# anenbergb/Co-DETR-TensorRT

Hardware: AMD Instinct MI355X
Metric: images/sec, Co-DINO Swin-L 1920x1280 fp16 (p50 ms/image alongside) (higher is better)
Workload: dtype f16

## Files before the change

co-detr-tensorrt_amd/codetr/_cabi.py:

```python
import ctypes
import os

import torch

_HERE = os.path.dirname(os.path.abspath(__file__))
LIB_PATH = os.path.join(_HERE, "libcodetr_hip.so")
ABI_VERSION = 54

_i64, _i32, _vp, _cp = ctypes.c_int64, ctypes.c_int, ctypes.c_void_p, ctypes.c_char_p

_MSDA_ARGS = [_vp, _vp, _vp, _vp, _vp, _vp, _i64, _i64, _i32, _i32, _i32, _i64, _i32, _i64, _vp]
SIGNATURES = {
    "codetr_hip_abi_version": (_i32, []),
    "codetr_hip_strerror": (_cp, [_i32]),
    "codetr_msda_forward_f16": (_i32, _MSDA_ARGS),
    "codetr_msda_forward_bf16": (_i32, _MSDA_ARGS),
    "codetr_msda_forward_f32": (_i32, _MSDA_ARGS),
    "codetr_msda_forward_f64": (_i32, _MSDA_ARGS),
    "codetr_msda_backward_f16": (_i32, [_vp, _vp, _vp, _vp, _vp, _vp, _vp, _i64, _i64, _i32, _i32, _i32, _i64, _i32, _i64,
                                        _vp, _vp, _vp]),
    "codetr_msda_backward_f32": (_i32, [_vp, _vp, _vp, _vp, _vp, _vp, _vp, _i64, _i64, _i32, _i32, _i32, _i64, _i32, _i64,
                                        _vp, _vp, _vp]),
    "codetr_msda_backward_f64": (_i32, [_vp, _vp, _vp, _vp, _vp, _vp, _vp, _i64, _i64, _i32, _i32, _i32, _i64, _i32, _i64,
                                        _vp, _vp, _vp]),
    "codetr_msda_variant": (_cp, [_i32, _i32, _i32, _i32, _i32]),
    "codetr_msda_fused_forward_f16": (_i32, [_vp, _vp, _vp, _vp, _vp, _i64, _vp, _i64, _vp, _i32, _i32, _i64, _i64,
                                             _i32, _i32, _i32, _i64, _i32, _vp]),
    "codetr_msda_fused_forward_bf16": (_i32, [_vp, _vp, _vp, _vp, _vp, _i64, _vp, _i64, _vp, _i32, _i32, _i64, _i64,
                                              _i32, _i32, _i32, _i64, _i32, _vp]),
    "codetr_msda_fused_forward_ref32_f16": (_i32, [_vp, _vp, _vp, _vp, _vp, _i64, _vp, _i64, _vp, _i32, _i32, _i64, _i64,
                                                   _i32, _i32, _i32, _i64, _i32, _vp]),
    "codetr_msda_fused_forward_ref32_bf16": (_i32, [_vp, _vp, _vp, _vp, _vp, _i64, _vp, _i64, _vp, _i32, _i32, _i64, _i64,
                                                    _i32, _i32, _i32, _i64, _i32, _vp]),
    "codetr_msda_encoder_forward_packed_f16": (_i32, [_vp, _vp, _vp, _vp, _i64, _vp, _i64, _i64, _i32, _i32, _i32, _i32,
                                                      _vp, _i32, _i32, _i32, _i32, _vp]),
    "codetr_msda_encoder_forward_packed_bf16": (_i32, [_vp, _vp, _vp, _vp, _i64, _vp, _i64, _i64, _i32, _i32, _i32, _i32,
                                                       _vp, _i32, _i32, _i32, _i32, _vp]),
    "codetr_linear_bf16_f16out": (_i32, [_vp, _vp, _vp, _vp, _vp, _vp, _i64, _i64, _i64, _i64, _i32]),
    "codetr_encoder_projections_f16": (_i32, [_vp, _vp, _vp, _vp, _vp, _vp, _vp, _vp, _i64, _i64, _i64, _i64, _i64, _i32]),
    "codetr_encoder_projections_bf16": (_i32, [_vp, _vp, _vp, _vp, _vp, _vp, _vp, _vp, _i64, _i64, _i64, _i64, _i64, _i32]),
    "codetr_encoder_projections_posgen_f16": (_i32, [_vp, _vp] + [_vp] * 10 + [_vp, _i32, _vp, ctypes.c_float, ctypes.c_float, ctypes.c_float,
                                                              ctypes.c_float, _i32, _vp, _vp, _vp, _vp, _vp, _i64, _i64, _i64, _i64, _i64, _i64, _i32]),
    "codetr_encoder_projections_posgen_bf16": (_i32, [_vp, _vp] + [_vp] * 10 + [_vp, _i32, _vp, ctypes.c_float, ctypes.c_float, ctypes.c_float,
                                                              ctypes.c_float, _i32, _vp, _vp, _vp, _vp, _vp, _i64, _i64, _i64, _i64, _i64, _i64, _i32]),
    "codetr_msda_encoder_packed_lds_bytes": (_i64, [_vp, _i32, _i32, _i32, _vp, _i32, _i32, _i32]),
    "codetr_msda_pack_projection_index": (_i32, [_i32, _i32, _i32, _vp]),
    "codetr_mx_scale_bytes": (_i64, [_i64, _i64]),
    "codetr_linear_fp8mx": (_i32, [_vp, _vp, _vp, _vp, _vp, _vp, _vp, _vp, _vp, _i64, _i64, _i64, _i32]),
    "codetr_cast_fp8mx_f16": (_i32, [_vp, _vp, _vp, _vp, _i64, _i64]),
    "codetr_layernorm_fp8mx_f16": (_i32, [_vp, _vp, _vp, _vp, _vp, _vp, _i64, _i64, ctypes.c_float]),
    "codetr_window_attention_fp8mx_f16": (_i32, [_vp, _vp, _vp, _vp, _vp, _vp, _i64, _i64, _i64, _i32, _i32, _i32, _i32]),
    "codetr_mha_attention_f16": (_i32, [_vp, _vp, _vp, _vp, _vp, _i64, _i64, _i64, _i32, _i32, _i64, _i64, _i64, _i64]),
    "codetr_mha_attention_bf16": (_i32, [_vp, _vp, _vp, _vp, _vp, _i64, _i64, _i64, _i32, _i32, _i64, _i64, _i64, _i64]),
    "codetr_linear_ln_f16": (_i32, [_vp, _vp, _vp, _vp, ctypes.c_float, _vp, _vp, _vp, _i64, _i64, _i64, _i32]),
    "codetr_linear_ln_bf16": (_i32, [_vp, _vp, _vp, _vp, ctypes.c_float, _vp, _vp, _vp, _i64, _i64, _i64, _i32]),
    "codetr_linear_xadd_f16": (_i32, [_vp, _vp, _vp, _vp, _vp, _vp, _i64, _i64, _i64]),
    "codetr_linear_xadd_bf16": (_i32, [_vp, _vp, _vp, _vp, _vp, _vp, _i64, _i64, _i64]),
    "codetr_im2col_tokens_b16": (_i32, [_vp, _vp, _i64, _i64, _i64, _i64, _i32, _i32, _i32, _vp]),
    "codetr_conv_tokens_f16": (_i32, [_vp, _vp, _vp, _vp, _vp, _vp, _i64, _i64, _i64, _i64, _i64, _i32, _i32, _i32, _i32]),
    "codetr_conv_tokens_bf16": (_i32, [_vp, _vp, _vp, _vp, _vp, _vp, _i64, _i64, _i64, _i64, _i64, _i32, _i32, _i32, _i32]),
    "codetr_conv_im2col_nchw_b16": (_i32, [_vp, _vp, _i64, _i32, _i64, _i64, _i32, _i32, _i32, _i32, _vp]),
    "codetr_maxpool_tokens_b16": (_i32, [_vp, _vp, _i64, _i64, _i64, _i64, _i32, _i32, _i32, _i32, _vp]),
    "codetr_topk_chunks": (_i64, [_i64, _i32, _i64, _vp]),
    "codetr_topk_chunked_f16": (_i32, [_vp, _vp, _i64, _i64, _i32, _i32, _vp, _vp, _vp, _i64]),
    "codetr_topk_chunked_bf16": (_i32, [_vp, _vp, _i64, _i64, _i32, _i32, _vp, _vp, _vp, _i64]),
    "codetr_topk_f16": (_i32, [_vp, _vp, _i64, _i64, _i32, _vp, _vp]),
    "codetr_topk_bf16": (_i32, [_vp, _vp, _i64, _i64, _i32, _vp, _vp]),
    "codetr_patch_im2col_b16": (_i32, [_vp, _vp, _i64, _i32, _i64, _i64, _i32, _i32, _vp]),
    "codetr_linear_variant": (_cp, [_i64, _i64, _i64, _i32, _i32, _i32]),
    "codetr_add_f16": (_i32, [_vp, _vp, _vp, _vp, _i64, _i64]),
    "codetr_add_bf16": (_i32, [_vp, _vp, _vp, _vp, _i64, _i64]),
    "codetr_sigmoid_f16": (_i32, [_vp, _vp, _vp, _i64]),
    "codetr_sigmoid_bf16": (_i32, [_vp, _vp, _vp, _i64]),
    "codetr_gather_rows_b16": (_i32, [_vp, _vp, _vp, _vp, _i64, _i64, _i64, _i64]),
    "codetr_decode_boxes_f16": (_i32, [_vp, _vp, _vp, _vp, _vp, _i64, _i64, _i64, _i32, ctypes.c_float, ctypes.c_float]),
    "codetr_decode_boxes_bf16": (_i32, [_vp, _vp, _vp, _vp, _vp, _i64, _i64, _i64, _i32, ctypes.c_float, ctypes.c_float]),
    "codetr_valid_ratios_f16": (_i32, [_vp, _vp, _vp, _vp, _vp, _i64, _i32]),
    "codetr_valid_ratios_bf16": (_i32, [_vp, _vp, _vp, _vp, _vp, _i64, _i32]),
    "codetr_linear_fp8": (_i32, [_vp, _vp, _vp, _vp, ctypes.c_float, _vp, _vp, _vp, _i32, ctypes.c_float, _i64, _i64, _i64,
                                 _i32]),
    "codetr_cast_fp8_f16": (_i32, [_vp, _vp, _vp, _i64, ctypes.c_float]),
    "codetr_layernorm_fp8_f16": (_i32, [_vp, _vp, _vp, _vp, _vp, _i64, _i64, ctypes.c_float, ctypes.c_float]),
    "codetr_linear_f16": (_i32, [_vp, _vp, _vp, _vp, _vp, _vp, _vp, _i64, _i64, _i64, _i32, _i64, _i32]),
    "codetr_linear_bf16": (_i32, [_vp, _vp, _vp, _vp, _vp, _vp, _vp, _i64, _i64, _i64, _i32, _i64, _i32]),
    "codetr_query_sine_embed_f16": (_i32, [_vp, _vp, _vp, _vp, _i64, _i64, _i32, _i32, _i32, ctypes.c_float, _i32, _vp, _vp,
                                           _vp]),
    "codetr_query_sine_embed_bf16": (_i32, [_vp, _vp, _vp, _vp, _i64, _i64, _i32, _i32, _i32, ctypes.c_float, _i32, _vp, _vp,
                                           _vp]),
    "codetr_encoder_geometry_f16": (_i32, [_vp, _vp, _vp, _i64, _i32, _vp, _vp, _vp, _vp, _vp]),
    "codetr_encoder_geometry_bf16": (_i32, [_vp, _vp, _vp, _i64, _i32, _vp, _vp, _vp, _vp, _vp]),
    "codetr_row_max_f16": (_i32, [_vp, _vp, _vp, _i64, _i64]),
    "codetr_row_max_bf16": (_i32, [_vp, _vp, _vp, _i64, _i64]),
    "codetr_preprocess_u8_f16": (_i32, [_vp, _vp, _i64, _i64, _i64, _i64, _i64, _i64, _vp, _vp, _vp, _vp, _vp]),
    "codetr_preprocess_u8_f32": (_i32, [_vp, _vp, _i64, _i64, _i64, _i64, _i64, _i64, _vp, _vp, _vp, _vp, _vp]),
    "codetr_batched_nms_f32": (_i32, [_vp, _vp, _vp, _i64, ctypes.c_float, _vp]),
    "codetr_preprocess_batch_u8_f16": (_i32, [_vp, _vp, _i64, _i64, _vp, _i64, _i64, _vp, _vp, _vp, ctypes.c_float, _vp, _vp]),
    "codetr_preprocess_batch_u8_bf16": (_i32, [_vp, _vp, _i64, _i64, _vp, _i64, _i64, _vp, _vp, _vp, ctypes.c_float, _vp, _vp]),
    "codetr_preprocess_batch_u8_f32": (_i32, [_vp, _vp, _i64, _i64, _vp, _i64, _i64, _vp, _vp, _vp, ctypes.c_float, _vp, _vp]),
    "codetr_postprocess_detections_f16": (_i32, [_vp, _vp, _vp, _vp, _vp, _i64, _i64, _i32, ctypes.c_float, _i32,
                                                 ctypes.c_float, _vp, _vp, _vp, _vp]),
    "codetr_postprocess_detections_bf16": (_i32, [_vp, _vp, _vp, _vp, _vp, _i64, _i64, _i32, ctypes.c_float, _i32,
                                                  ctypes.c_float, _vp, _vp, _vp, _vp]),
    "codetr_postprocess_detections_f32": (_i32, [_vp, _vp, _vp, _vp, _vp, _i64, _i64, _i32, ctypes.c_float, _i32,
                                                 ctypes.c_float, _vp, _vp, _vp, _vp]),
    "codetr_postprocess_softnms_f16": (_i32, [_vp, _vp, _vp, _vp, _vp, _i64, _i64, _i32, ctypes.c_float, _i32,
                                              ctypes.c_float, ctypes.c_float, _i64, _vp, _vp, _vp, _vp, _vp]),
    "codetr_postprocess_softnms_bf16": (_i32, [_vp, _vp, _vp, _vp, _vp, _i64, _i64, _i32, ctypes.c_float, _i32,
                                               ctypes.c_float, ctypes.c_float, _i64, _vp, _vp, _vp, _vp, _vp]),
    "codetr_postprocess_softnms_f32": (_i32, [_vp, _vp, _vp, _vp, _vp, _i64, _i64, _i32, ctypes.c_float, _i32,
                                              ctypes.c_float, ctypes.c_float, _i64, _vp, _vp, _vp, _vp, _vp]),
    "codetr_preprocess_views_u8_f16": (_i32, [_vp, _vp, _i64, _i64, _vp, _i64, _i64, _vp, _vp, _vp, ctypes.c_float, _vp, _vp]),
    "codetr_preprocess_views_u8_bf16": (_i32, [_vp, _vp, _i64, _i64, _vp, _i64, _i64, _vp, _vp, _vp, ctypes.c_float, _vp, _vp]),
    "codetr_preprocess_views_u8_f32": (_i32, [_vp, _vp, _i64, _i64, _vp, _i64, _i64, _vp, _vp, _vp, ctypes.c_float, _vp, _vp]),
    "codetr_tta_merge_f16": (_i32, [_vp, _vp, _vp, _vp, _vp, _i64, _i64, _i64, ctypes.c_uint32, _vp, _i32, ctypes.c_float,
                                    ctypes.c_float, _i64, _vp, _vp, _vp, _vp, _vp]),
    "codetr_tta_merge_bf16": (_i32, [_vp, _vp, _vp, _vp, _vp, _i64, _i64, _i64, ctypes.c_uint32, _vp, _i32, ctypes.c_float,
                                     ctypes.c_float, _i64, _vp, _vp, _vp, _vp, _vp]),
    "codetr_tta_merge_f32": (_i32, [_vp, _vp, _vp, _vp, _vp, _i64, _i64, _i64, ctypes.c_uint32, _vp, _i32, ctypes.c_float,
                                    ctypes.c_float, _i64, _vp, _vp, _vp, _vp, _vp]),
    "codetr_patch_merge_layernorm_f16": (_i32, [_vp, _vp, _vp, _vp, _vp, _i64, _i64, _i64, _i64, ctypes.c_float]),
    "codetr_patch_merge_layernorm_bf16": (_i32, [_vp, _vp, _vp, _vp, _vp, _i64, _i64, _i64, _i64, ctypes.c_float]),
    "codetr_mask_pyramid": (_i32, [_vp, _vp, _i64, _i64, _i64, _i32, _vp, _vp, _vp, _vp, _vp, _i32]),
    "codetr_linear_splitk_plan": (_i32, [_i64, _i64, _i64, _vp]),
    "codetr_linear_splitk_f16": (_i32, [_vp, _vp, _vp, _vp, _vp, _vp, _vp, _i64, _i64, _i64, _i32, _i32, _vp, _i64]),
    "codetr_linear_splitk_bf16": (_i32, [_vp, _vp, _vp, _vp, _vp, _vp, _vp, _i64, _i64, _i64, _i32, _i32, _vp, _i64]),
    "codetr_linear_sk_workspace_bytes": (_i64, []),
    "codetr_linear_sk_supported": (_i32, [_i64, _i64, _i64]),
    "codetr_linear_sk_preferred": (_i32, [_i64, _i64, _i64, _i32, _i32]),
    "codetr_linear_sk_f16": (_i32, [_vp, _vp, _vp, _vp, _vp, _vp, _i64, _i64, _i64, _i32, _vp, _i64, _i32]),
    "codetr_msda_op4_supported": (_i32, [_i32, _i64, _i64, _i32, _i32, _i32, _i64, _i32]),
    "codetr_msda_op4_forward_f16": (_i32, [_vp, _vp, _vp, _vp, _vp, _vp, _i64, _i64, _i32, _i32, _i32, _i64, _i32, _vp]),
    "codetr_msda_op4_forward_bf16": (_i32, [_vp, _vp, _vp, _vp, _vp, _vp, _i64, _i64, _i32, _i32, _i32, _i64, _i32, _vp]),
    "codetr_swin_mlp_supported": (_i32, [_i64, _i64, _i64]),
    "codetr_swin_mlp_f16": (_i32, [_vp, _vp, _vp, _vp, ctypes.c_float, _vp, _vp, _vp, _vp, _vp, _i64, _i64]),
    "codetr_swin_mlp_bf16": (_i32, [_vp, _vp, _vp, _vp, ctypes.c_float, _vp, _vp, _vp, _vp, _vp, _i64, _i64]),
    "codetr_linear_pp_supported": (_i32, [_i64, _i64, _i64]),
    "codetr_linear_pp_preferred": (_i32, [_i64, _i64, _i64, _i32, _i32]),
    "codetr_linear_pp_f16": (_i32, [_vp, _vp, _vp, _vp, _vp, _vp, _i64, _i64, _i64, _i32, _i32]),
    "codetr_linear_pp_bf16": (_i32, [_vp, _vp, _vp, _vp, _vp, _vp, _i64, _i64, _i64, _i32, _i32]),
    "codetr_linear_sk_bf16": (_i32, [_vp, _vp, _vp, _vp, _vp, _vp, _i64, _i64, _i64, _i32, _vp, _i64, _i32]),
    "codetr_decoder_layer_supported": (_i32, [_i32] * 7),
    "codetr_decoder_layer_blob_halfs": (_i64, [_i32] * 4),
    "codetr_decoder_layer_f16": (_i32, [_vp] * 18 + [_i64, _i64, _i64, _i32, _i32, _i32, ctypes.c_float, ctypes.c_float]),
    "codetr_decoder_layer_bf16": (_i32, [_vp] * 18 + [_i64, _i64, _i64, _i32, _i32, _i32, ctypes.c_float, ctypes.c_float]),
    "codetr_layernorm_f16": (_i32, [_vp, _vp, _vp, _vp, _vp, _i64, _i64, ctypes.c_float]),
    "codetr_layernorm_bf16": (_i32, [_vp, _vp, _vp, _vp, _vp, _i64, _i64, ctypes.c_float]),
    "codetr_groupnorm_tokens_workspace_bytes": (_i64, [_i64, _i64, _i64]),
    "codetr_groupnorm_tokens_f16": (_i32, [_vp, _vp, _vp, _vp, _vp, _i64, _vp, _i64, _i64, _i64, _i32,
                                           ctypes.c_float]),
    "codetr_groupnorm_tokens_bf16": (_i32, [_vp, _vp, _vp, _vp, _vp, _i64, _vp, _i64, _i64, _i64, _i32,
                                           ctypes.c_float]),
    "codetr_sine_pos_tokens_f16": (_i32, [_vp, _vp, _vp, _vp, _vp, _i64, _i64, _i64, _i64, _i32, ctypes.c_float,
                                          ctypes.c_float, ctypes.c_float, ctypes.c_float, _i32]),
    "codetr_sine_pos_tokens_bf16": (_i32, [_vp, _vp, _vp, _vp, _vp, _i64, _i64, _i64, _i64, _i32, ctypes.c_float,
                                          ctypes.c_float, ctypes.c_float, ctypes.c_float, _i32]),
    "codetr_ffn_relu_f16": (_i32, [_vp, _vp, _vp, _vp, _vp, _vp, _vp, _i64, _i64, _i64]),
    "codetr_ffn_relu_ln_f16": (_i32, [_vp, _vp, _vp, _vp, _vp, _vp, _vp, _i64, _i64, _i64, _vp, _vp, ctypes.c_float,
                                      _vp, _vp]),
    "codetr_ffn_relu_ln2_f16": (_i32, [_vp, _vp, _vp, _vp, _vp, _vp, _vp, _i64, _i64, _i64, _vp, _vp, ctypes.c_float,
                                       _vp, _vp, ctypes.c_float, _vp, _vp]),
    "codetr_ffn_relu_ln2_bf16": (_i32, [_vp, _vp, _vp, _vp, _vp, _vp, _vp, _i64, _i64, _i64, _vp, _vp, ctypes.c_float,
                                       _vp, _vp, ctypes.c_float, _vp, _vp]),
    "codetr_ffn_pack_w2_f16": (_i32, [_vp, _vp, _vp, _i64, _i64]),
    "codetr_ffn_oproj_relu_ln2_f16": (_i32, [_vp, _vp, _vp, _vp, _vp, _vp, _vp, _vp, _vp, _vp, _i64, _i64, _i64, _vp, _vp,
                                             ctypes.c_float, _vp, _vp, ctypes.c_float, _vp, _vp]),
    "codetr_ffn_oproj_relu_ln2_bf16": (_i32, [_vp, _vp, _vp, _vp, _vp, _vp, _vp, _vp, _vp, _vp, _i64, _i64, _i64, _vp, _vp,
                                              ctypes.c_float, _vp, _vp, ctypes.c_float, _vp, _vp]),
    "codetr_ffn_oproj_w1_index": (_i32, [_i64, _vp]),
    "codetr_ffn_fp8": (_i32, [_vp, _vp, _vp, _vp, _vp, _vp, _vp, _vp, _vp, _i64, _i64, _i64, ctypes.c_float, ctypes.c_float,
                              _vp, _vp, ctypes.c_float, _vp, _vp, ctypes.c_float, _vp, _vp]),
    "codetr_window_attention_f16": (_i32, [_vp, _vp, _vp, _vp, _vp, _i64, _i64, _i64, _i32, _i32, _i32, _i32]),
    "codetr_window_attention_bf16": (_i32, [_vp, _vp, _vp, _vp, _vp, _i64, _i64, _i64, _i32, _i32, _i32, _i32]),
    "codetr_window_attention_ex": (_i32, [_vp, _vp, _vp, _vp, _vp, _vp, ctypes.c_float, _i64, _i64, _i64, _i32, _i32, _i32, _i32,
                                          _i32, _i32, _i32]),
    "codetr_window_attention_bias_index": (_i32, [_i32, _vp]),
    "codetr_window_attention_fp8out_f16": (_i32, [_vp, _vp, _vp, _vp, _vp, ctypes.c_float, _i64, _i64, _i64, _i32, _i32,
                                                  _i32, _i32]),
}

_lib = None

CALLS = {"encoder_projections_posgen": 0, "msda": 0, "msda_fused": 0, "linear": 0, "layernorm": 0, "window_attention": 0, "groupnorm_tokens": 0,
         "sine_pos_tokens": 0, "ffn_fused": 0, "ffn_oproj_fused": 0, "linear_splitk": 0, "linear_sk": 0, "mask_pyramid": 0,
         "query_sine_embed": 0, "encoder_geometry": 0, "row_max": 0, "preprocess": 0, "batched_nms": 0,
         "preprocess_batch": 0, "postprocess_detections": 0, "postprocess_softnms": 0,
         "preprocess_views": 0, "tta_merge": 0,
         "msda_backward": 0, "patch_merge_layernorm": 0, "msda_encoder": 0, "msda_encoder_packed": 0, "patch_im2col": 0, "mha_attention": 0, "topk": 0,
         "linear_pp": 0, "swin_mlp": 0, "linear_tile128": 0, "linear_tile256": 0, "linear_xs": 0, "linear_ln": 0, "linear_xadd": 0, "encoder_projections": 0,
         "linear_fp8": 0, "cast_fp8": 0, "layernorm_fp8": 0, "small_ops": 0, "ffn_fp8": 0, "decoder_layer": 0,
         "conv_tokens": 0, "conv_im2col_nchw": 0, "maxpool_tokens": 0}


RECORDER = None
_QUERIES = {"codetr_hip_abi_version", "codetr_hip_strerror", "codetr_msda_variant", "codetr_linear_variant",
            "codetr_topk_chunks", "codetr_linear_splitk_plan", "codetr_groupnorm_tokens_workspace_bytes",
            "codetr_linear_sk_workspace_bytes", "codetr_linear_sk_supported", "codetr_linear_sk_preferred",
            "codetr_linear_pp_supported", "codetr_linear_pp_preferred", "codetr_msda_op4_supported", "codetr_swin_mlp_supported",
            "codetr_msda_encoder_packed_lds_bytes", "codetr_msda_pack_projection_index", "codetr_window_attention_bias_index",
            "codetr_mx_scale_bytes", "codetr_decoder_layer_supported",
            "codetr_decoder_layer_blob_halfs"}


class _RecordingLib:
    def __init__(self, lib):
        self._lib = lib

    def __getattr__(self, name):
        fn = getattr(self._lib, name)
        if name in _QUERIES or name not in SIGNATURES:
            return fn

        def launch(*args):
            rc = fn(*args)
            if RECORDER is not None and rc == 0:
                RECORDER.append((name, args))
            return rc

        return launch


_rec_lib = None


def load():
    global _lib, _rec_lib
    if _lib is not None:
        if RECORDER is None:
            return _lib
        if _rec_lib is None:
            _rec_lib = _RecordingLib(_lib)
        return _rec_lib
    if not os.path.isfile(LIB_PATH):
        raise ImportError(
            f"HIP extension not found at {LIB_PATH}; build it with "
            "`python -c 'import __graft_entry__ as g; g.build()'` or `make -C co-detr-tensorrt_amd/csrc`"
        )
    lib = ctypes.CDLL(LIB_PATH)
    for name, (res, args) in SIGNATURES.items():
        try:
            fn = getattr(lib, name)
        except AttributeError as e:
            raise ImportError(f"{LIB_PATH} does not export {name}; rebuild the extension") from e
        fn.restype = res
        fn.argtypes = args
    ver = lib.codetr_hip_abi_version()
    if ver != ABI_VERSION:
        raise ImportError(f"{LIB_PATH} has ABI version {ver}, host expects {ABI_VERSION}; rebuild the extension")
    _lib = lib
    return lib


def strerror(code: int) -> str:
    return load().codetr_hip_strerror(code).decode()


def check(code: int, what: str):
    if code != 0:
        raise RuntimeError(f"{what} failed: {strerror(code)} (code {code})")


def current_stream_ptr(device) -> int:
    return torch.cuda.current_stream(device).cuda_stream


_MSDA_BY_DTYPE = {
    torch.float16: ("codetr_msda_forward_f16", 2),
    torch.bfloat16: ("codetr_msda_forward_bf16", 2),
    torch.float32: ("codetr_msda_forward_f32", 4),
    torch.float64: ("codetr_msda_forward_f64", 8),
}


def msda_variant(dtype, M, D, L, P) -> str:
    return load().codetr_msda_variant(_MSDA_BY_DTYPE[dtype][1], M, D, L, P).decode()


def msda_forward(value, spatial_shapes, level_start_index, sampling_loc, attn_weight, im2col_step, out):
    lib = load()
    CALLS["msda"] += 1
    name, _ = _MSDA_BY_DTYPE[value.dtype]
    B, S, M, D = value.shape
    Nq, L, P = sampling_loc.shape[1], sampling_loc.shape[3], sampling_loc.shape[4]
    rc = getattr(lib, name)(
        current_stream_ptr(value.device),
        value.data_ptr(), spatial_shapes.data_ptr(), level_start_index.data_ptr(),
        sampling_loc.data_ptr(), attn_weight.data_ptr(),
        B, S, M, D, L, Nq, P, int(im2col_step), out.data_ptr(),
    )
    if rc == -2:
        raise RuntimeError(f"batch({B}) must divide im2col_step({min(B, int(im2col_step))})")
    check(rc, name)
    return out


_ACT = {None: 0, "relu": 1, "gelu": 2, "relu_res": 3}
_LINEAR_BY_DTYPE = {torch.float16: "codetr_linear_f16", torch.bfloat16: "codetr_linear_bf16"}


def linear_supported(x, weight) -> bool:
    return x.dtype in _LINEAR_BY_DTYPE and weight.dtype == x.dtype and weight.shape[1] % 64 == 0


_VARIANTS = {}


def linear_variant(M, N, K, act=None, has_residual=False, hm_head_dim=0) -> str:
    key = (M, N, K, act, bool(has_residual), hm_head_dim)
    v = _VARIANTS.get(key)
    if v is None:
        v = _VARIANTS[key] = load().codetr_linear_variant(M, N, K, _ACT[act], 1 if has_residual else 0,
                                                          hm_head_dim).decode()
    return v


def linear(x2d, weight, bias, residual2d, act, out2d, row_mask=None, hm_rows=0, hm_head_dim=0):
    lib = load()
    CALLS["linear"] += 1
    M, K = x2d.shape
    N = weight.shape[0]
    variant = linear_variant(M, N, K, act, residual2d is not None, hm_head_dim)
    if variant != "unsupported":
        CALLS["linear_" + variant] += 1
    rc = getattr(lib, _LINEAR_BY_DTYPE[x2d.dtype])(
        current_stream_ptr(x2d.device), x2d.data_ptr(), weight.data_ptr(),
        bias.data_ptr() if bias is not None else None,
        residual2d.data_ptr() if residual2d is not None else None,
        row_mask.data_ptr() if row_mask is not None else None,
        out2d.data_ptr(), M, N, K, _ACT[act], hm_rows, hm_head_dim)
    check(rc, "codetr_linear")
    return out2d


_SK_PREFERRED = {}


def linear_sk_preferred(M, N, K, act=None, has_residual=False) -> bool:
    key = (M, N, K, act, bool(has_residual))
    v = _SK_PREFERRED.get(key)
    if v is None:
        v = _SK_PREFERRED[key] = bool(load().codetr_linear_sk_preferred(M, N, K, _ACT[act], 1 if has_residual else 0))
    return v


_SK_WORKSPACE = {}


def linear_sk_workspace(device):
    key = (device.index, torch.cuda.current_stream(device).cuda_stream)
    ws = _SK_WORKSPACE.get(key)
    if ws is None:
        with torch.cuda.device(device):
            ws = _SK_WORKSPACE[key] = torch.zeros(load().codetr_linear_sk_workspace_bytes(), dtype=torch.uint8, device=device)
    return ws


def linear_sk(x2d, weight, bias, residual2d, act, out2d, flags=0):
    lib = load()
    CALLS["linear"] += 1
    CALLS["linear_sk"] += 1
    M, K = x2d.shape
    N = weight.shape[0]
    ws = linear_sk_workspace(x2d.device) if flags & 0x40 else None
    fn = lib.codetr_linear_sk_f16 if x2d.dtype == torch.float16 else lib.codetr_linear_sk_bf16
    rc = fn(current_stream_ptr(x2d.device), x2d.data_ptr(), weight.data_ptr(),
            bias.data_ptr() if bias is not None else None,
            residual2d.data_ptr() if residual2d is not None else None, out2d.data_ptr(), M, N, K, _ACT[act],
            ws.data_ptr() if ws is not None else None, ws.numel() if ws is not None else 0, flags)
    check(rc, "codetr_linear_sk")
    return out2d


def swin_mlp(x2d, ln_w, ln_b, eps, w1, b1, w2_packed, b2, out2d):
    CALLS["swin_mlp"] += 1
    lib = load()
    fn = lib.codetr_swin_mlp_bf16 if x2d.dtype == torch.bfloat16 else lib.codetr_swin_mlp_f16
    rc = fn(current_stream_ptr(x2d.device), x2d.data_ptr(), ln_w.data_ptr(), ln_b.data_ptr(), float(eps), w1.data_ptr(),
            b1.data_ptr(), w2_packed.data_ptr(), b2.data_ptr(), out2d.data_ptr(), x2d.shape[0], x2d.shape[1])
    check(rc, "codetr_swin_mlp")
    return out2d


_PP_PREFERRED = {}


def linear_pp_preferred(M, N, K, act=None, has_residual=False) -> bool:
    key = (M, N, K, act, bool(has_residual))
    v = _PP_PREFERRED.get(key)
    if v is None:
        v = _PP_PREFERRED[key] = bool(load().codetr_linear_pp_preferred(M, N, K, _ACT[act], 1 if has_residual else 0))
    return v


def linear_pp(x2d, weight, bias, residual2d, act, out2d, flags=0):
    lib = load()
    CALLS["linear"] += 1
    CALLS["linear_pp"] += 1
    M, K = x2d.shape
    N = weight.shape[0]
    fn = lib.codetr_linear_pp_f16 if x2d.dtype == torch.float16 else lib.codetr_linear_pp_bf16
    rc = fn(current_stream_ptr(x2d.device), x2d.data_ptr(), weight.data_ptr(),
            bias.data_ptr() if bias is not None else None,
            residual2d.data_ptr() if residual2d is not None else None, out2d.data_ptr(), M, N, K, _ACT[act], flags)
    check(rc, "codetr_linear_pp")
    return out2d


def query_sine_embed(ref, valid_ratios, pos_feat, temperature=10000.0, apply_sigmoid=True, valid_ratios32=None):
    CALLS["query_sine_embed"] += 1
    B, Nq, d = ref.shape
    L = valid_ratios.shape[1]
    ref_in = torch.empty((B, Nq, L, d), dtype=ref.dtype, device=ref.device)
    ref_in32 = torch.empty((B, Nq, L, d), dtype=torch.float32, device=ref.device) if valid_ratios32 is not None else None
    embed = torch.empty((B, Nq, d * pos_feat), dtype=ref.dtype, device=ref.device)
    fn = load().codetr_query_sine_embed_bf16 if ref.dtype == torch.bfloat16 else load().codetr_query_sine_embed_f16
    rc = fn(current_stream_ptr(ref.device), ref.data_ptr(), valid_ratios.data_ptr(),
                                            valid_ratios32.data_ptr() if valid_ratios32 is not None else None, B, Nq,
                                            d, L, pos_feat, float(temperature), 1 if apply_sigmoid else 0,
                                            ref_in.data_ptr(), ref_in32.data_ptr() if ref_in32 is not None else None,
                                            embed.data_ptr())
    check(rc, "codetr_query_sine_embed_f16")
    return ref_in, embed, ref_in32


_MSDA_BWD = {torch.float16: "codetr_msda_backward_f16", torch.float32: "codetr_msda_backward_f32",
             torch.float64: "codetr_msda_backward_f64"}


def msda_backward(value, spatial_shapes, level_start_index, sampling_loc, attn_weight, grad_output, grad_value,
                  grad_sampling_loc, grad_attn_weight, im2col_step):
    if value.dtype not in _MSDA_BWD:
        raise RuntimeError(f"multi_scale_deformable_attention_backward: unsupported dtype {value.dtype} (f16 / f32 / f64)")
    CALLS["msda_backward"] += 1
    B, S, M, D = value.shape
    Nq, L, P = sampling_loc.shape[1], sampling_loc.shape[3], sampling_loc.shape[4]
    rc = getattr(load(), _MSDA_BWD[value.dtype])(
        current_stream_ptr(value.device), value.data_ptr(), spatial_shapes.data_ptr(), level_start_index.data_ptr(),
        sampling_loc.data_ptr(), attn_weight.data_ptr(), grad_output.data_ptr(), B, S, M, D, L, Nq, P, int(im2col_step),
        grad_value.data_ptr(), grad_sampling_loc.data_ptr(), grad_attn_weight.data_ptr())
    if rc == -2:
        step = min(B, int(im2col_step))
        raise RuntimeError(f"batch({B}) must divide im2col_step({step})")
    check(rc, "codetr_msda_backward")


def encoder_geometry(valid_ratios, mask_flat, shapes):
    CALLS["encoder_geometry"] += 1
    B, S = mask_flat.shape
    L = len(shapes)
    dev = mask_flat.device
    dt = valid_ratios.dtype
    ref = torch.empty((B, S, 2), dtype=dt, device=dev)
    ref_lvl = torch.empty((B, S, L, 2), dtype=dt, device=dev)
    prop = torch.empty((B, S, 4), dtype=dt, device=dev)
    state = torch.empty((B, S), dtype=torch.uint8, device=dev)
    hw = (ctypes.c_int64 * (2 * L))(*[int(v) for s in shapes for v in s])
    fn = load().codetr_encoder_geometry_bf16 if valid_ratios.dtype == torch.bfloat16 else load().codetr_encoder_geometry_f16
    rc = fn(current_stream_ptr(dev), valid_ratios.data_ptr(), mask_flat.data_ptr(), B, L, hw,
                                            ref.data_ptr(), ref_lvl.data_ptr(), prop.data_ptr(), state.data_ptr())
    check(rc, "codetr_encoder_geometry_f16")
    return ref, ref_lvl, prop, state


def row_max(x2d):
    CALLS["row_max"] += 1
    rows, C = x2d.shape
    out = torch.empty((rows,), dtype=x2d.dtype, device=x2d.device)
    fn = load().codetr_row_max_bf16 if x2d.dtype == torch.bfloat16 else load().codetr_row_max_f16
    rc = fn(current_stream_ptr(x2d.device), x2d.data_ptr(), out.data_ptr(), rows, C)
    check(rc, "codetr_row_max_f16")
    return out


def preprocess_u8(src, resized_hw, pad_hw, mean, std, pad_value, dtype, with_mask=True):
    CALLS["preprocess"] += 1
    if dtype not in (torch.float16, torch.float32):
        raise RuntimeError("preprocess_u8 writes f16 or f32")
    Hs, Ws, _ = src.shape
    (Hr, Wr), (Hp, Wp) = resized_hw, pad_hw
    dst = torch.empty((3, Hp, Wp), dtype=dtype, device=src.device)
    mask = torch.empty((Hp, Wp), dtype=dtype, device=src.device) if with_mask else None
    f3 = ctypes.c_float * 3
    fn = load().codetr_preprocess_u8_f16 if dtype == torch.float16 else load().codetr_preprocess_u8_f32
    rc = fn(current_stream_ptr(src.device), src.data_ptr(), Hs, Ws, Hr, Wr, Hp, Wp, f3(*[float(v) for v in mean]),
            f3(*[float(v) for v in std]), (ctypes.c_int * 3)(*[int(v) for v in pad_value]), dst.data_ptr(),
            mask.data_ptr() if mask is not None else None)
    check(rc, "codetr_preprocess_u8")
    return dst, mask


def batched_nms_sorted(boxes_sorted, labels_sorted, iou_threshold):
    CALLS["batched_nms"] += 1
    N = boxes_sorted.shape[0]
    keep = torch.empty((N,), dtype=torch.bool, device=boxes_sorted.device)
    rc = load().codetr_batched_nms_f32(current_stream_ptr(boxes_sorted.device), boxes_sorted.data_ptr(),
                                       labels_sorted.data_ptr(), N, float(iou_threshold), keep.data_ptr())
    check(rc, "codetr_batched_nms_f32")
    return keep


PREPROCESS_BATCH_MAX = 32
POSTPROCESS_MAX_Q = 1024
_PRE_BATCH_BY_DTYPE = {torch.float16: "codetr_preprocess_batch_u8_f16", torch.bfloat16: "codetr_preprocess_batch_u8_bf16",
                       torch.float32: "codetr_preprocess_batch_u8_f32"}
_POST_BY_DTYPE = {torch.float16: "codetr_postprocess_detections_f16", torch.bfloat16: "codetr_postprocess_detections_bf16",
                  torch.float32: "codetr_postprocess_detections_f32"}


def preprocess_batch_u8(src, images, batch_hw, mean, std, pad_value, pad_fill, dst, mask):
    CALLS["preprocess_batch"] += 1
    N = len(images)
    H, W = batch_hw
    table = (ctypes.c_int64 * (7 * N))(*[int(v) for row in images for v in row])
    f3 = ctypes.c_float * 3
    rc = getattr(load(), _PRE_BATCH_BY_DTYPE[dst.dtype])(
        current_stream_ptr(src.device), src.data_ptr(), src.numel(), N, table, H, W, f3(*[float(v) for v in mean]),
        f3(*[float(v) for v in std]), (ctypes.c_int * 3)(*[int(v) for v in pad_value]), float(pad_fill), dst.data_ptr(),
        mask.data_ptr() if mask is not None else None)
    check(rc, "codetr_preprocess_batch_u8")


def postprocess_detections(boxes, scores, labels, divisors, score_threshold, iou_threshold, boxes_out, scores_out,
                           labels_out, count):
    CALLS["postprocess_detections"] += 1
    N, Q = scores.shape
    rc = getattr(load(), _POST_BY_DTYPE[scores.dtype])(
        current_stream_ptr(scores.device), boxes.data_ptr(), scores.data_ptr(), labels.data_ptr(), divisors.data_ptr(),
        N, Q, 0 if score_threshold is None else 1, 0.0 if score_threshold is None else float(score_threshold),
        0 if iou_threshold is None else 1, 0.0 if iou_threshold is None else float(iou_threshold), boxes_out.data_ptr(),
        scores_out.data_ptr(), labels_out.data_ptr(), count.data_ptr())
    check(rc, "codetr_postprocess_detections")


_SOFTNMS_BY_DTYPE = {torch.float16: "codetr_postprocess_softnms_f16", torch.bfloat16: "codetr_postprocess_softnms_bf16",
                     torch.float32: "codetr_postprocess_softnms_f32"}
SOFTNMS_METHODS = {"naive": 0, "linear": 1}


def postprocess_softnms(boxes, scores, labels, divisors, score_threshold, method, iou_threshold, min_score, max_keep,
                        boxes_out, scores_out, labels_out, index_out, count):
    CALLS["postprocess_softnms"] += 1
    N, Q = scores.shape
    rc = getattr(load(), _SOFTNMS_BY_DTYPE[scores.dtype])(
        current_stream_ptr(scores.device), boxes.data_ptr(), scores.data_ptr(), labels.data_ptr(), divisors.data_ptr(),
        N, Q, 0 if score_threshold is None else 1, 0.0 if score_threshold is None else float(score_threshold),
        int(method), float(iou_threshold), float(min_score), int(max_keep), boxes_out.data_ptr(), scores_out.data_ptr(),
        labels_out.data_ptr(), index_out.data_ptr(), count.data_ptr())
    check(rc, "codetr_postprocess_softnms")


TTA_MAX_VIEWS = 16
TTA_MAX_CANDIDATES = 4096
TTA_NMS_MODES = {"nms": 0, "naive": 1, "linear": 2}
_PRE_VIEWS_BY_DTYPE = {torch.float16: "codetr_preprocess_views_u8_f16", torch.bfloat16: "codetr_preprocess_views_u8_bf16",
                       torch.float32: "codetr_preprocess_views_u8_f32"}
_TTA_MERGE_BY_DTYPE = {torch.float16: "codetr_tta_merge_f16", torch.bfloat16: "codetr_tta_merge_bf16",
                       torch.float32: "codetr_tta_merge_f32"}


def preprocess_views_u8(src, rows, batch_hw, mean, std, pad_value, pad_fill, dst, mask):
    CALLS["preprocess_views"] += 1
    N = len(rows)
    H, W = batch_hw
    table = (ctypes.c_int64 * (8 * N))(*[int(v) for row in rows for v in row])
    f3 = ctypes.c_float * 3
    rc = getattr(load(), _PRE_VIEWS_BY_DTYPE[dst.dtype])(
        current_stream_ptr(src.device), src.data_ptr(), src.numel(), N, table, H, W, f3(*[float(v) for v in mean]),
        f3(*[float(v) for v in std]), (ctypes.c_int * 3)(*[int(v) for v in pad_value]), float(pad_fill), dst.data_ptr(),
        mask.data_ptr() if mask is not None else None)
    check(rc, "codetr_preprocess_views_u8")


def tta_merge(boxes, scores, labels, count, flip_mask, width, mode, iou_threshold, min_score, max_keep, boxes_out,
              scores_out, labels_out, index_out, count_out):
    CALLS["tta_merge"] += 1
    V, N, Q = scores.shape
    rc = getattr(load(), _TTA_MERGE_BY_DTYPE[scores.dtype])(
        current_stream_ptr(scores.device), boxes.data_ptr(), scores.data_ptr(), labels.data_ptr(), count.data_ptr(),
        V, N, Q, int(flip_mask), width.data_ptr(), int(mode), float(iou_threshold), float(min_score), int(max_keep),
        boxes_out.data_ptr(), scores_out.data_ptr(), labels_out.data_ptr(), index_out.data_ptr(), count_out.data_ptr())
    check(rc, "codetr_tta_merge")


def mask_pyramid(img_masks, shapes):
    CALLS["mask_pyramid"] += 1
    B, Hi, Wi = img_masks.shape
    L = len(shapes)
    S = sum(int(h) * int(w) for h, w in shapes)
    dev = img_masks.device
    mask_flat = torch.empty((B, S), dtype=torch.bool, device=dev)
    cums = torch.empty((2, B * S), dtype=torch.float32, device=dev)
    counts = torch.empty((B, L, 2), dtype=torch.float32, device=dev)
    hw = (ctypes.c_int64 * (2 * L))(*[int(v) for s in shapes for v in s])
    rc = load().codetr_mask_pyramid(current_stream_ptr(dev), img_masks.data_ptr(), B, Hi, Wi, L, hw,
                                    mask_flat.data_ptr(), cums[0].data_ptr(), cums[1].data_ptr(), counts.data_ptr(),
                                    img_masks.element_size())
    check(rc, "codetr_mask_pyramid")
    return mask_flat, cums[0], cums[1], counts


_SPLITK_PLANS = {}


def linear_splitk_plan(M, N, K):
    key = (M, N, K)
    if key not in _SPLITK_PLANS:
        nbytes = ctypes.c_int64(0)
        splits = load().codetr_linear_splitk_plan(M, N, K, ctypes.byref(nbytes))
        _SPLITK_PLANS[key] = (int(splits), int(nbytes.value))
    return _SPLITK_PLANS[key]


def linear_splitk(x2d, weight, bias, residual2d, act, out2d, splits, workspace, row_mask=None):
    lib = load()
    CALLS["linear"] += 1
    CALLS["linear_splitk"] += 1
    M, K = x2d.shape
    N = weight.shape[0]
    fn = lib.codetr_linear_splitk_f16 if x2d.dtype == torch.float16 else lib.codetr_linear_splitk_bf16
    rc = fn(current_stream_ptr(x2d.device), x2d.data_ptr(), weight.data_ptr(),
            bias.data_ptr() if bias is not None else None,
            residual2d.data_ptr() if residual2d is not None else None,
            row_mask.data_ptr() if row_mask is not None else None,
            out2d.data_ptr(), M, N, K, _ACT[act], splits, workspace.data_ptr(), workspace.numel())
# ... 586 lines not shown
```

co-detr-tensorrt_amd/codetr/_kernel_names.py:

```python
KERNEL_NAMES = (
    "add_kernel",
    "batched_nms_kernel",
    "cast_fp8_kernel",
    "cast_fp8mx_kernel",
    "conv_im2col_nchw_kernel",
    "conv_tokens_kernel",
    "decode_boxes_kernel",
    "decoder_layer_kernel",
    "encoder_geometry_kernel",
    "ffn_fp8_kernel",
    "ffn_fused_kernel",
    "gather_rows_kernel",
    "gn_apply_kernel",
    "gn_finalize_kernel",
    "gn_partial_kernel",
    "im2col_tokens_kernel",
    "layernorm_fp8_kernel",
    "layernorm_fp8mx_kernel",
    "layernorm_kernel",
    "level_cums_kernel",
    "level_mask_kernel",
    "linear_256_fp8_kernel",
    "linear_256_kernel",
    "linear_kernel",
    "linear_pp_kernel",
    "linear_sk_kernel",
    "linear_xs_kernel",
    "maxpool_tokens_kernel",
    "mha_attention_kernel",
    "msda_backward_generic_kernel",
    "msda_backward_kernel",
    "msda_encoder_v4_kernel",
    "msda_fused_headmajor_kernel",
    "msda_op4_kernel",
    "msda_scalar_kernel",
    "msda_tiled_kernel",
    "pack_w2_kernel",
    "patch_im2col_k4_kernel",
    "postprocess_kernel",
    "postprocess_softnms_kernel",
    "preprocess_batch_kernel",
    "preprocess_kernel",
    "preprocess_views_kernel",
    "query_sine_embed_kernel",
    "row_max_kernel",
    "sigmoid_kernel",
    "sine_pos_kernel",
    "splitk_reduce_kernel",
    "swin_mlp_kernel",
    "topk_kernel",
    "topk_reg_kernel",
    "tta_merge_kernel",
    "valid_ratios_kernel",
    "window_attention_kernel",
)
```

co-detr-tensorrt_amd/codetr/hip_ops.py:

```python

import collections

import torch
import torch.nn.functional as F

from . import _cabi

NATIVE = {"msda", "linear(f16/bf16, K%64==0)", "layer_norm(f16/bf16)", "swin_window_attention(f16, head_dim 32)",
          "msda_fused(softmax + sampling locations in-kernel)", "groupnorm_tokens(f16, 8 ch/group)",
          "sine_pos_tokens(f16, + level_embed)", "ffn_fused(f16, 256 -> hidden -> 256, ReLU, + identity)",
          "mask_pyramid(level masks + running valid counts + valid ratios)",
          "query_sine_embed(f16: sigmoid x valid ratios + sine embedding of the decoder reference boxes)",
          "encoder_geometry(f16: reference points, proposals, keep/drop state)", "row_max(f16)",
          "preprocess_image(u8 -> f16/f32, cv2-exact resize + pad + normalise + mask)", "batched_nms(f32)",
          "preprocess_batch(u8 -> f16/bf16/f32, <= 32 images of any size per launch, stacked + padded)",
          "postprocess_detections(f16/bf16/f32: threshold + sort + per-class NMS + rescale, one workgroup per image)",
          "postprocess_detections_soft(f16/bf16/f32: threshold + per-class soft-NMS (linear / naive) + max_per_img + rescale)",
          "patch_merge_layernorm(f16: Swin 2x2 gather + LayerNorm)",
          "msda_encoder_packed(f16/bf16: LDS-staged gather for the encoder's self-attention, csrc/msda_encoder4.hip)",
          "patch_embed(f16/bf16: 4x4 patch gather + GEMM)",
          "mha_attention(f16/bf16: dense softmax attention, head_dim 32, <= 1024 keys)",
          "topk(f16/bf16 rows, k <= 1024: radix select + bitonic sort)",
          "im2col_tokens(16-bit token-major maps)",
          "resnet50(f16/bf16: implicit-GEMM conv_tokens, stem window gather + GEMM, maxpool_tokens, BN folded)",
          "small_ops(f16: add, sigmoid, gather_rows, decode_boxes, valid_ratios)",
          "linear_fp8(e4m3 x e4m3, K%128==0) + layer_norm_fp8 + cast_fp8", "ffn_fp8(fused FFN, both products e4m3)"}


LINEAR_PROFILE = None
KERNEL_PROFILE = None


def _timed(name, meta, launch, device):
    if KERNEL_PROFILE is None:
        return launch()
    st = torch.cuda.current_stream(device)
    e0, e1 = torch.cuda.Event(enable_timing=True), torch.cuda.Event(enable_timing=True)
    e0.record(st)
    r = launch()
    e1.record(st)
    KERNEL_PROFILE.setdefault(name, []).append((e0, e1, meta))
    return r


def _gpu(x, what):
    if not x.is_cuda:
        raise RuntimeError(
            f"codetr.hip_ops.{what}: got a {x.device.type} tensor; this package computes on MI355X only "
            "(the CPU formulation is the oracle in oracle/, not a fallback)"
        )


LINEAR_PP = True


def _persistent_ok(mk, head_major, out, x2, w, r2, bias):
    return (mk is None and not head_major and out.data_ptr() % 16 == 0 and x2.data_ptr() % 16 == 0
            and w.data_ptr() % 16 == 0 and (r2 is None or r2.data_ptr() % 16 == 0)
            and (bias is None or bias.data_ptr() % 16 == 0))


def linear(x, weight, bias=None, act=None, residual=None, row_mask=None, head_major=None):
    _gpu(x, "linear")
    if _cabi.linear_supported(x, weight):
        K = x.shape[-1]
        N = weight.shape[0]
        x2 = x.reshape(-1, K)
        if not x2.is_contiguous():
            x2 = x2.contiguous()
        w = weight if weight.is_contiguous() else weight.contiguous()
        r2 = None
        if residual is not None:
            r2 = residual.reshape(-1, N)
            if not r2.is_contiguous():
                r2 = r2.contiguous()
        mk = None
        if row_mask is not None:
            mk = row_mask.reshape(-1)
            if mk.dtype != torch.bool and mk.dtype != torch.uint8:
                mk = mk != 0
            mk = mk.contiguous()
        hm_rows = hm_hd = 0
        if head_major:
            if x.dim() != 3 or residual is not None:
                raise ValueError("head_major needs a [B, S, K] input and no residual")
            hm_rows, hm_hd = x.shape[1], int(head_major)
        out = torch.empty((x2.shape[0], N), dtype=x.dtype, device=x.device)
        if x2.shape[0] > 0:
            with torch.cuda.device(x.device):
                res_act = act == "relu_res"
                splits, ws_bytes = (1, 0) if (head_major or res_act) else _cabi.linear_splitk_plan(x2.shape[0], N, K)
                if res_act:
                    launch = lambda: _cabi.linear(x2, w, bias, r2, act, out, mk, hm_rows, hm_hd)
                elif splits > 1:
                    ws = torch.empty(ws_bytes, dtype=torch.uint8, device=x.device)
                    launch = lambda: _cabi.linear_splitk(x2, w, bias, r2, act, out, splits, ws, mk)
                elif (LINEAR_PP and _persistent_ok(mk, head_major, out, x2, w, r2, bias)
                      and _cabi.linear_pp_preferred(x2.shape[0], N, K, act, r2 is not None)):
                    launch = lambda: _cabi.linear_pp(x2, w, bias, r2, act, out)
                elif (_persistent_ok(mk, head_major, out, x2, w, r2, bias)
                      and _cabi.linear_sk_preferred(x2.shape[0], N, K, act, r2 is not None)):
                    launch = lambda: _cabi.linear_sk(x2, w, bias, r2, act, out)
                else:
                    launch = lambda: _cabi.linear(x2, w, bias, r2, act, out, mk, hm_rows, hm_hd)
                if LINEAR_PROFILE is None:
                    launch()
                else:
                    st = torch.cuda.current_stream(x.device)
                    e0, e1 = torch.cuda.Event(enable_timing=True), torch.cuda.Event(enable_timing=True)
                    e0.record(st)
                    launch()
                    e1.record(st)
                    LINEAR_PROFILE.append((e0, e1, 2.0 * x2.shape[0] * N * K, x2.shape[0], N, K))
        if head_major:
            return out.view(x.shape[0], N // hm_hd, hm_rows, hm_hd)
        return out.view(*x.shape[:-1], N)
    if head_major:
        raise RuntimeError("head_major output exists only on the native linear (f16/bf16, K % 64 == 0)")
    y = F.linear(x, weight, bias)
    if act == "relu_res":
        if row_mask is not None:
            y = y.masked_fill(row_mask[..., None], 0.0)
        return F.relu(y + residual if residual is not None else y)
    if act == "relu":
        y = F.relu(y, inplace=True)
    elif act == "gelu":
        y = F.gelu(y)
    elif act is not None:
        raise ValueError(act)
    if row_mask is not None:
        y = y.masked_fill(row_mask[..., None], 0.0)
    if residual is not None:
        y = y + residual
    return y


LN_GEMM = True


def linear_ln_supported(x, norm_weight, weight):
    return (LN_GEMM and x.is_cuda and norm_weight is not None and norm_weight.dtype == x.dtype and weight.dtype == x.dtype
            and not torch.is_grad_enabled() and norm_weight.shape[0] == x.shape[-1]
            and _cabi.linear_xadd_supported(x.numel() // max(x.shape[-1], 1), weight.shape[0], x.shape[-1], x.dtype))


def linear_ln(x, norm_weight, norm_bias, eps, weight, bias=None, act=None):
    _gpu(x, "linear_ln")
    if linear_ln_supported(x, norm_weight, weight):
        K, N = x.shape[-1], weight.shape[0]
        x2 = x.reshape(-1, K)
        x2 = x2 if x2.is_contiguous() else x2.contiguous()
        w = weight if weight.is_contiguous() else weight.contiguous()
        out = torch.empty((x2.shape[0], N), dtype=x.dtype, device=x.device)
        ok = [False]

        def launch():
            ok[0] = _cabi.linear_ln(x2, norm_weight, norm_bias, eps, w, bias, act, out)

        with torch.cuda.device(x.device):
            if LINEAR_PROFILE is None:
                launch()
            else:
                st = torch.cuda.current_stream(x.device)
                e0, e1 = torch.cuda.Event(enable_timing=True), torch.cuda.Event(enable_timing=True)
                e0.record(st)
                launch()
# ... 94 lines not shown
        x2 = x2.contiguous()
    out = torch.empty_like(x2)
    w1c = w1 if w1.is_contiguous() else w1.contiguous()
    with torch.cuda.device(x.device):
        w2p = _packed_w2(w2)
        _timed("swin_mlp", {"M": x2.shape[0], "C": C},
               lambda: _cabi.swin_mlp(x2, ln_weight, ln_bias, eps, w1c, b1, w2p, b2, out), x.device)
    return out.view(x.shape)


def ffn_fused(x, w1, b1, w2, b2, ln=None, pos=None, ln_in=None):
    _gpu(x, "ffn_fused")
    x2 = x.reshape(-1, x.shape[-1])
    if not x2.is_contiguous():
        x2 = x2.contiguous()
    out = torch.empty_like(x2)
    p2 = out2 = None
    if pos is not None:
        p2 = pos.reshape(-1, pos.shape[-1])
        if p2.shape != x2.shape or p2.dtype != x2.dtype:
            raise ValueError("pos must match x in shape and dtype")
        if not p2.is_contiguous():
            p2 = p2.contiguous()
        out2 = torch.empty_like(x2)
    if x2.shape[0] > 0:
        with torch.cuda.device(x.device):
            _timed("ffn_fused", {"M": x2.shape[0], "C": x2.shape[1], "hidden": w1.shape[0]},
                   lambda: _cabi.ffn_fused(x2, w1.contiguous(), b1, _packed_w2(w2), b2, out, ln, p2, out2, ln_in), x.device)
    if pos is not None:
        return out.view(x.shape), out2.view(x.shape)
    return out.view(x.shape)


FFN_OPROJ = True


def ffn_oproj_fused(attn, wo, bo, identity, w1, b1, w2, b2, ln, pos=None, ln_in=None):
    _gpu(attn, "ffn_oproj_fused")
    C = attn.shape[-1]
    a2, i2 = attn.reshape(-1, C), identity.reshape(-1, C)
    a2 = a2 if a2.is_contiguous() else a2.contiguous()
    i2 = i2 if i2.is_contiguous() else i2.contiguous()
    if i2.shape != a2.shape or i2.dtype != a2.dtype:
        raise ValueError("identity must match the attention output in shape and dtype")
    out = torch.empty_like(a2)
    p2 = out2 = None
    if pos is not None:
        p2 = pos.reshape(-1, C)
        if p2.shape != a2.shape or p2.dtype != a2.dtype:
            raise ValueError("pos must match x in shape and dtype")
        p2 = p2 if p2.is_contiguous() else p2.contiguous()
        out2 = torch.empty_like(a2)
    w1p = derived((w1,), "_codetr_w1_oproj", lambda: w1.detach()[:, torch.tensor(
        _cabi.ffn_oproj_w1_index(C), dtype=torch.long, device=w1.device)].contiguous())
    woc = wo if wo.is_contiguous() else wo.contiguous()
    if a2.shape[0] > 0:
        with torch.cuda.device(attn.device):
            _timed("ffn_fused", {"M": a2.shape[0], "C": C, "hidden": w1.shape[0], "oproj": True},
                   lambda: _cabi.ffn_oproj_fused(a2, woc, bo, i2, w1p, b1, _packed_w2(w2), b2, out, ln_in, ln, p2, out2),
                   attn.device)
    if pos is not None:
        return out.view(attn.shape), out2.view(attn.shape)
    return out.view(attn.shape)


def layer_norm(x, weight, bias, eps=1e-5):
    _gpu(x, "layer_norm")
    if _cabi.layernorm_supported(x, weight):
        C = x.shape[-1]
        x2 = x.reshape(-1, C)
        if not x2.is_contiguous():
            x2 = x2.contiguous()
        out = torch.empty_like(x2)
        if x2.shape[0] > 0:
            with torch.cuda.device(x.device):
                _cabi.layernorm(x2, weight, bias, eps, out)
        return out.view(x.shape)
    return F.layer_norm(x, (x.shape[-1],), weight, bias, eps)


MERGE_LN = True


def patch_merge_layernorm_supported(x, C):
    return (x.is_cuda and x.dtype in (torch.float16, torch.bfloat16) and C % 8 == 0 and 4 * C <= 4096
            and MERGE_LN)


def patch_merge_layernorm(x, hw, weight_kkc, bias_kkc, eps=1e-5):
    _gpu(x, "patch_merge_layernorm")
    B, L, C = x.shape
    H, W = hw
    x4 = x.view(B, H, W, C)
    if not x4.is_contiguous():
        x4 = x4.contiguous()
    with torch.cuda.device(x.device):
        return _cabi.patch_merge_layernorm(x4, weight_kkc, bias_kkc, eps)


def group_norm(x, groups, weight, bias, eps=1e-5):
    _gpu(x, "group_norm")
    return F.group_norm(x, groups, weight, bias, eps)


def groupnorm_tokens_supported(x, groups):
    return x.is_cuda and _cabi.groupnorm_tokens_supported(x, groups)


def groupnorm_tokens_into(x, gamma, beta, groups, eps, dest, row_start):
    _gpu(x, "groupnorm_tokens_into")
    B, HW, C = x.shape
    if not x.is_contiguous():
        x = x.contiguous()
    if not dest.is_contiguous() or dest.shape[0] != B or dest.shape[2] != C:
        raise AssertionError("destination must be a contiguous [B, S, C] tensor")
    with torch.cuda.device(x.device):
        _cabi.groupnorm_tokens(x, gamma, beta, groups, eps, dest[0, row_start:], dest.shape[1] * C)
    return dest


def query_sine_embed_supported(ref, valid_ratios, pos_feat):
    return (ref.is_cuda and ref.dtype in (torch.float16, torch.bfloat16) and valid_ratios.dtype == ref.dtype
            and ref.shape[-1] in (2, 4) and pos_feat % 8 == 0 and valid_ratios.shape[1] <= ref.shape[-1] * pos_feat // 8)


def query_sine_embed(ref, valid_ratios, pos_feat, temperature=10000.0):
    _gpu(ref, "query_sine_embed")
    vr32 = getattr(valid_ratios, "_codetr_f32", None) if MSDA_FP32_REF else None
    with torch.cuda.device(ref.device):
        ref_in, embed, ref32 = _cabi.query_sine_embed(ref.contiguous(), valid_ratios.contiguous(), pos_feat, temperature,
                                                      valid_ratios32=vr32)
    if ref32 is not None:
        ref_in._codetr_ref32 = ref32
    return ref_in, embed


def encoder_geometry(valid_ratios, mask_flat, shapes):
    _gpu(mask_flat, "encoder_geometry")
    if valid_ratios.dtype not in (torch.float16, torch.bfloat16):
        raise RuntimeError("encoder_geometry is the 16-bit inference path; fp32 parity runs use the ATen formulation")
    with torch.cuda.device(mask_flat.device):
        return _cabi.encoder_geometry(valid_ratios.contiguous(), mask_flat.contiguous(),
                                      [tuple(int(v) for v in s) for s in shapes])


def row_max(x):
    _gpu(x, "row_max")
    if x.dtype not in (torch.float16, torch.bfloat16) or not x.is_contiguous():
        return x.max(-1)[0]
    with torch.cuda.device(x.device):
        return _cabi.row_max(x.view(-1, x.shape[-1])).view(x.shape[:-1])


def preprocess_image(src_u8, resized_hw, pad_hw, mean, std, pad_value=(0, 0, 0), dtype=torch.float16):
    _gpu(src_u8, "preprocess_image")
    if src_u8.dtype != torch.uint8 or src_u8.dim() != 3 or src_u8.shape[2] != 3:
        raise ValueError("expected a uint8 [H, W, 3] image")
    with torch.cuda.device(src_u8.device):
        return _cabi.preprocess_u8(src_u8.contiguous(), resized_hw, pad_hw, mean, std, pad_value, dtype)


def batched_nms(boxes, scores, labels, iou_threshold):
    _gpu(boxes, "batched_nms")
    if boxes.shape[0] == 0:
        return torch.empty((0,), dtype=torch.int64, device=boxes.device)
    order = torch.sort(scores.float(), descending=True, stable=True)[1]
    with torch.cuda.device(boxes.device):
        keep = _cabi.batched_nms_sorted(boxes.float()[order].contiguous(), labels.to(torch.int64)[order].contiguous(),
                                        iou_threshold)
    return order[keep]


PREPROCESS_BATCH_MAX = _cabi.PREPROCESS_BATCH_MAX


def preprocess_batch(src_u8, images, batch_hw, mean, std, pad_val=(0, 0, 0), pad_value=0.0, dtype=torch.float16,
                     with_mask=True):
    _gpu(src_u8, "preprocess_batch")
    if src_u8.dtype != torch.uint8 or src_u8.dim() != 1 or not src_u8.is_contiguous():
        raise ValueError("expected one contiguous flat uint8 buffer")
    if dtype not in (torch.float16, torch.bfloat16, torch.float32):
        raise ValueError(f"preprocess_batch writes f16, bf16 or f32, not {dtype}")
    N = len(images)
    H, W = (int(v) for v in batch_hw)
    x = torch.empty((N, 3, H, W), dtype=dtype, device=src_u8.device)
    m = torch.empty((N, H, W), dtype=dtype, device=src_u8.device) if with_mask else None
    with torch.cuda.device(src_u8.device):
        for i in range(0, N, PREPROCESS_BATCH_MAX):
            j = min(N, i + PREPROCESS_BATCH_MAX)
            _cabi.preprocess_batch_u8(src_u8, images[i:j], (H, W), mean, std, pad_val, pad_value, x[i:j],
                                      m[i:j] if m is not None else None)
    return x, m


Detections = collections.namedtuple("Detections", "boxes scores labels count packed")


def _detection_views(packed, N, Q, dtype):
    es = torch.empty((), dtype=dtype).element_size()
    o1 = N * Q * 8
    o2 = o1 + N * 4
    o3 = o2 + N * Q * 4 * es
    o4 = o3 + N * Q * es
    return Detections(packed[o2:o3].view(dtype).view(N, Q, 4), packed[o3:o4].view(dtype).view(N, Q),
                      packed[:o1].view(torch.int64).view(N, Q), packed[o1:o2].view(torch.int32), packed)


def postprocess_detections(boxes, scores, labels, divisors, score_threshold=None, iou_threshold=None):
    _gpu(scores, "postprocess_detections")
    dtype = scores.dtype
    if dtype not in (torch.float16, torch.bfloat16, torch.float32) or boxes.dtype != dtype or divisors.dtype != dtype:
        raise ValueError("postprocess_detections: boxes, scores and divisors in one dtype of f16 / bf16 / f32")
    N, Q = scores.shape
    if tuple(boxes.shape) != (N, Q, 4) or tuple(labels.shape) != (N, Q) or tuple(divisors.shape) != (N, 4):
        raise ValueError("postprocess_detections: boxes [N,Q,4], scores [N,Q], labels [N,Q], divisors [N,4]")
    nbytes = N * Q * 8 + N * 4 + N * Q * 5 * scores.element_size()
    if N == 0 or Q == 0:
        return _detection_views(torch.zeros((nbytes,), dtype=torch.uint8, device=scores.device), N, Q, dtype)
    out = _detection_views(torch.empty((nbytes,), dtype=torch.uint8, device=scores.device), N, Q, dtype)
    with torch.cuda.device(scores.device):
        _cabi.postprocess_detections(boxes.contiguous(), scores.contiguous(), labels.to(torch.int64).contiguous(),
                                     divisors.contiguous(), score_threshold, iou_threshold, out.boxes, out.scores,
                                     out.labels, out.count)
    return out


def detections_to_host(dets):
    N, Q = dets.scores.shape
    views = _soft_detection_views if isinstance(dets, SoftDetections) else _detection_views
    return views(dets.packed.cpu(), N, Q, dets.scores.dtype)


SoftDetections = collections.namedtuple("SoftDetections", "boxes scores labels count index packed")


def _soft_detection_views(packed, N, Q, dtype):
    es = torch.empty((), dtype=dtype).element_size()
    o1 = N * Q * 8
    o2 = o1 + N * 4
    o3 = o2 + N * Q * 4
    o4 = o3 + N * Q * 4 * es
    o5 = o4 + N * Q * es
    return SoftDetections(packed[o3:o4].view(dtype).view(N, Q, 4), packed[o4:o5].view(dtype).view(N, Q),
                          packed[:o1].view(torch.int64).view(N, Q), packed[o1:o2].view(torch.int32),
                          packed[o2:o3].view(torch.int32).view(N, Q), packed)


def _soft_method(method):
    if method == "gaussian":
        raise NotImplementedError("soft-NMS method 'gaussian' is not provided (exp() cannot be held bit-exact against "
                                  "the CPU reference and no shipped config uses it): 'linear' or 'naive'")
    if method not in _cabi.SOFTNMS_METHODS:
        raise ValueError(f"soft-NMS method must be 'linear' or 'naive', got {method!r}")
    return _cabi.SOFTNMS_METHODS[method]


def postprocess_detections_soft(boxes, scores, labels, divisors, score_threshold=None, iou_threshold=0.3,
                                method="linear", min_score=1e-3, max_per_img=None):
    _gpu(scores, "postprocess_detections_soft")
    m = _soft_method(method)
    dtype = scores.dtype
    if dtype not in (torch.float16, torch.bfloat16, torch.float32) or boxes.dtype != dtype or divisors.dtype != dtype:
        raise ValueError("postprocess_detections_soft: boxes, scores and divisors in one dtype of f16 / bf16 / f32")
    if scores.dim() != 2:
        raise ValueError("postprocess_detections_soft: boxes [N,Q,4], scores [N,Q], labels [N,Q], divisors [N,4]")
    N, Q = scores.shape
    if tuple(boxes.shape) != (N, Q, 4) or tuple(labels.shape) != (N, Q) or tuple(divisors.shape) != (N, 4):
        raise ValueError("postprocess_detections_soft: boxes [N,Q,4], scores [N,Q], labels [N,Q], divisors [N,4]")
    nbytes = N * Q * 12 + N * 4 + N * Q * 5 * scores.element_size()
    if N == 0 or Q == 0:
        return _soft_detection_views(torch.zeros((nbytes,), dtype=torch.uint8, device=scores.device), N, Q, dtype)
    out = _soft_detection_views(torch.empty((nbytes,), dtype=torch.uint8, device=scores.device), N, Q, dtype)
    with torch.cuda.device(scores.device):
        _cabi.postprocess_softnms(boxes.contiguous(), scores.contiguous(), labels.to(torch.int64).contiguous(),
                                  divisors.contiguous(), score_threshold, m, iou_threshold, min_score,
                                  0 if max_per_img is None else int(max_per_img), out.boxes, out.scores, out.labels,
                                  out.index, out.count)
    return out


def soft_nms(boxes, scores, labels, iou_threshold, method="linear", min_score=1e-3):
    _gpu(boxes, "soft_nms")
    _soft_method(method)
    n = boxes.shape[0]
    if n == 0:
        return scores.new_empty((0,)), torch.empty((0,), dtype=torch.int64, device=boxes.device)
    if n > _cabi.POSTPROCESS_MAX_Q:
        raise ValueError(f"soft_nms: at most {_cabi.POSTPROCESS_MAX_Q} boxes per call, got {n}")
    dtype = scores.dtype if scores.dtype in (torch.float16, torch.bfloat16, torch.float32) else torch.float32
    dets = postprocess_detections_soft(boxes.to(dtype)[None], scores.to(dtype)[None], labels[None],
                                       torch.ones((1, 4), dtype=dtype, device=boxes.device), None, iou_threshold, method,
                                       min_score, None)
    c = int(dets.count[0])
    return dets.scores[0, :c].to(scores.dtype), dets.index[0, :c].to(torch.int64)


TTA_MAX_VIEWS = _cabi.TTA_MAX_VIEWS
TTA_MAX_CANDIDATES = _cabi.TTA_MAX_CANDIDATES


def preprocess_views(src_u8, rows8, batch_hw, mean, std, pad_val=(0, 0, 0), pad_value=0.0, dtype=torch.float16,
                     with_mask=True):
    _gpu(src_u8, "preprocess_views")
    if src_u8.dtype != torch.uint8 or src_u8.dim() != 1 or not src_u8.is_contiguous():
        raise ValueError("expected one contiguous flat uint8 buffer")
    if dtype not in (torch.float16, torch.bfloat16, torch.float32):
# ... 157 lines not shown
                                    "out_bytes": out.element_size()},
               lambda: _cabi.window_attention(qkv, qkv_bias, rel_bias if lane is None else lane, out, B, H, W, num_heads,
                                              window_size, shift, out_scale, scales, 0 if lane is None else 1), qkv.device)
    return (out, scales) if out_mx else out


def mha_self_attention(q, k, v, num_heads):
    _gpu(q, "mha_self_attention")
    B, N, C = q.shape
    if _cabi.mha_attention_supported(q, k, v, num_heads):
        out = torch.empty((B, N, C), dtype=q.dtype, device=q.device)
        with torch.cuda.device(q.device):
            _cabi.mha_attention(q, k, v, num_heads, out)
        return out
    hd = C // num_heads
    sp = lambda t: t.reshape(B, -1, num_heads, hd).transpose(1, 2)
    o = F.scaled_dot_product_attention(sp(q), sp(k), sp(v))
    return o.transpose(1, 2).reshape(B, N, C)


def msda_fused_supported(value_dtype, head_dim, num_levels, num_points):
    return _cabi.msda_fused_supported(value_dtype, head_dim, num_levels, num_points)


def msda_head_major_supported(value_dtype, head_dim, num_levels, num_points):
    return _cabi.msda_head_major_supported(value_dtype, head_dim, num_levels, num_points)


def msda_fused(value, spatial_shapes, level_start_index, proj, off_col, logit_col, reference_points, num_levels,
               num_points, head_major=False):
    _gpu(value, "msda_fused")
    if head_major:
        B, M, S, D = value.shape
    else:
        B, S, M, D = value.shape
    out = torch.empty((B, proj.shape[1], M * D), dtype=value.dtype, device=value.device)
    ref32 = getattr(reference_points, "_codetr_ref32", None) if MSDA_FP32_REF else None
    ref = ref32 if ref32 is not None else reference_points.to(value.dtype).contiguous()
    if out.numel():
        with torch.cuda.device(value.device):
            _timed("msda_fused", {"B": B, "S": S, "Nq": proj.shape[1], "M": M, "D": D, "L": num_levels, "P": num_points},
                   lambda: _cabi.msda_fused(value.contiguous(), spatial_shapes, level_start_index, proj.contiguous(),
                                            off_col, logit_col, ref, num_levels, num_points, out,
                                            head_major=head_major), value.device)
    return out


def patch_embed_supported(x, weight, stride):
    kh, kw = weight.shape[-2:]
    return (x.is_cuda and x.dtype in (torch.float16, torch.bfloat16) and weight.dtype == x.dtype
            and kh == kw == 4 and tuple(stride) == (4, 4) and x.shape[1] * 16 <= 64 and not torch.is_grad_enabled())


def patch_embed(x, weight, bias):
    _gpu(x, "patch_embed")
    B, C, H, W = x.shape
    E = weight.shape[0]
    Hp, Wp = -(-H // 4), -(-W // 4)
    cache = getattr(weight, "_codetr_w64", None)
    if cache is None or cache[0] != weight._version or cache[1].device != weight.device:
        w64 = torch.zeros((E, 64), dtype=weight.dtype, device=weight.device)
        w64[:, :C * 16] = weight.detach().reshape(E, C * 16)
        cache = weight._codetr_w64 = (weight._version, w64)
    cols = torch.empty((B * Hp * Wp, 64), dtype=x.dtype, device=x.device)
    with torch.cuda.device(x.device):
        _cabi.patch_im2col(x.contiguous(), 4, 64, cols)
    return linear(cols, cache[1], bias).view(B, Hp * Wp, E), (Hp, Wp)


def im2col_tokens(x4d, k, stride, pad):
    _gpu(x4d, "im2col_tokens")
    B, H, W, C = x4d.shape
    Ho, Wo = (H + 2 * pad - k) // stride + 1, (W + 2 * pad - k) // stride + 1
    if x4d.dtype in (torch.float16, torch.bfloat16) and C % 8 == 0:
        out = torch.empty((B, Ho * Wo, k * k * C), dtype=x4d.dtype, device=x4d.device)
        with torch.cuda.device(x4d.device):
            _cabi.im2col_tokens(x4d.contiguous(), k, stride, pad, out)
        return out
    xp = F.pad(x4d, (0, 0, pad, pad, pad, pad))
    return torch.cat([xp[:, ky:ky + stride * (Ho - 1) + 1:stride, kx:kx + stride * (Wo - 1) + 1:stride, :]
                      for ky in range(k) for kx in range(k)], dim=-1).reshape(B, Ho * Wo, -1)


R50_NATIVE = True
R50_CONV_IM2COL = False


def conv_tokens(x4d, weight_kkc, bias, k, stride, pad, act=None, residual=None):
    _gpu(x4d, "conv_tokens")
    B, H, W, C = x4d.shape
    Cout = weight_kkc.shape[0]
    Ho, Wo = (H + 2 * pad - k) // stride + 1, (W + 2 * pad - k) // stride + 1
    if not _cabi.conv_tokens_supported(x4d, weight_kkc, k, stride, pad):
        raise RuntimeError(f"conv_tokens: no native kernel for x {tuple(x4d.shape)} {x4d.dtype}, k={k}, stride={stride}, "
                           f"pad={pad}, Cout={Cout} (C % 64 == 0, Cout % 8 == 0, k in (1, 3), stride in (1, 2))")
    if R50_CONV_IM2COL:
        cols = im2col_tokens(x4d, k, stride, pad)
        r = residual.reshape(B, Ho * Wo, Cout) if residual is not None else None
        return linear(cols, weight_kkc, bias, act=act, residual=r).view(B, Ho, Wo, Cout)
    x4d = x4d if x4d.is_contiguous() else x4d.contiguous()
    if residual is not None and not residual.is_contiguous():
        residual = residual.contiguous()
    out = torch.empty((B, Ho, Wo, Cout), dtype=x4d.dtype, device=x4d.device)
    with torch.cuda.device(x4d.device):
        _timed("conv_tokens", {"M": B * Ho * Wo, "N": Cout, "K": k * k * C},
               lambda: _cabi.conv_tokens(x4d, weight_kkc, bias, residual, k, stride, pad, act, out), x4d.device)
    return out


def stem_conv_tokens(x, weight_pad, bias, k, stride, pad):
    _gpu(x, "stem_conv_tokens")
    B, C, H, W = x.shape
    Cout, kpad = weight_pad.shape
    Ho, Wo = (H + 2 * pad - k) // stride + 1, (W + 2 * pad - k) // stride + 1
    cols = torch.empty((B * Ho * Wo, kpad), dtype=x.dtype, device=x.device)
    with torch.cuda.device(x.device):
        _cabi.conv_im2col_nchw(x if x.is_contiguous() else x.contiguous(), k, stride, pad, kpad, cols)
    return linear(cols, weight_pad, bias, act="relu").view(B, Ho, Wo, Cout)


def maxpool_tokens(x4d):
    _gpu(x4d, "maxpool_tokens")
    B, H, W, C = x4d.shape
    out = torch.empty((B, (H - 1) // 2 + 1, (W - 1) // 2 + 1, C), dtype=x4d.dtype, device=x4d.device)
    with torch.cuda.device(x4d.device):
        _cabi.maxpool_tokens(x4d if x4d.is_contiguous() else x4d.contiguous(), out)
    return out




def topk(x, k, want_values=True):
    _gpu(x, "topk")
    x2 = x.reshape(-1, x.shape[-1])
    if not torch.is_grad_enabled():
        x2 = x2 if x2.is_contiguous() else x2.contiguous()
        if _cabi.topk_supported(x2, k):
            idx = torch.empty((x2.shape[0], k), dtype=torch.int64, device=x.device)
            val = torch.empty((x2.shape[0], k), dtype=x.dtype, device=x.device) if want_values else None
            with torch.cuda.device(x.device):
                _cabi.topk(x2, k, val, idx)
            shape = (*x.shape[:-1], k)
            return (val.view(shape) if val is not None else None), idx.view(shape)
    v, i = torch.topk(x, k, dim=-1)
    return v, i


MSDA_ENCODER = True
MSDA_FP32_REF = True


_SWITCH_DEFAULTS = {"ENC_POSGEN": True, "WINDOW_BIAS_LANE": True, "LINEAR_PP": True, "SWIN_MLP": True, "SWIN_MLP_MIN_ROWS": 32768, "LN_GEMM": True, "XADD": True, "XADD_MIN_ROWS": 0, "MERGE_LN": True, "MSDA_ENCODER": True,
                    "MSDA_FP32_REF": True, "FP8_MIN_TILES": 96,
                    "R50_NATIVE": True, "R50_CONV_IM2COL": False}


def nondefault_switches():
    import sys

    from . import multi_scale_deformable_attention as msda_mod
    from . import transformer as tr_mod

    me = sys.modules[__name__]
    out = [k for k, v in _SWITCH_DEFAULTS.items() if getattr(me, k) != v]
    if msda_mod.HEAD_MAJOR_VALUE:
        out.append("HEAD_MAJOR_VALUE")
    out += [k for k in ("DEC_FUSED", "DEC_VPROJ") if not getattr(tr_mod, k)]
    return sorted(out)


MSDA_V4 = True
MSDA_V4_THREADS = 512
MSDA_V4_REGION = (16, 16)
MSDA_V4_LDS_BUDGET = 64 * 1024
MSDA_V4_MARGIN_CAP = 40.0
MSDA_V4_HEAD_MAJOR = True
ENC_PROJ_FUSED = True
_SWITCH_DEFAULTS.update({"MSDA_V4": True, "MSDA_V4_THREADS": 512, "MSDA_V4_REGION": (16, 16),
                         "MSDA_V4_LDS_BUDGET": 64 * 1024, "MSDA_V4_MARGIN_CAP": 40.0,
                         "MSDA_V4_HEAD_MAJOR": True, "ENC_PROJ_FUSED": True, "FFN_OPROJ": True})


def msda_encoder_packed_supported(dtype, head_dim, num_levels, num_points):
    return (MSDA_V4 and MSDA_ENCODER and dtype in (torch.float16, torch.bfloat16) and head_dim == 32 and num_levels == 5
            and num_points == 4)


def value_projection_f16(x, weight, bias, row_mask, head_dim):
    _gpu(x, "value_projection_f16")
    if not (x.dtype == torch.bfloat16 and weight.dtype == torch.bfloat16 and x.dim() == 3):
        return None
    B, S, K = x.shape
    N = weight.shape[0]
    x2 = x.reshape(-1, K)
    x2 = x2 if x2.is_contiguous() else x2.contiguous()
    w = weight if weight.is_contiguous() else weight.contiguous()
    mk = None
    if row_mask is not None:
        mk = row_mask.reshape(-1)
        if mk.dtype != torch.bool and mk.dtype != torch.uint8:
            mk = mk != 0
        mk = mk.contiguous()
    out = torch.empty((B * S, N), dtype=torch.float16, device=x.device)
    with torch.cuda.device(x.device):
        ok = _cabi.linear_bf16_f16out(x2, w, bias, out, mk, S, int(head_dim))
    return out.view(B, N // head_dim, S, head_dim) if ok else None


ENC_POSGEN = True


def encoder_projections(x, pos, w_cat, b_cat, row_mask, n_value, head_dim):
    _gpu(x, "encoder_projections")
    if not (ENC_PROJ_FUSED and x.dim() == 3 and x.dtype in (torch.float16, torch.bfloat16) and pos is not None
            and pos.shape == x.shape and pos.dtype == x.dtype and w_cat.dtype == x.dtype and not torch.is_grad_enabled()):
        return None
    B, S, K = x.shape
    n_packed = w_cat.shape[0] - n_value
    x2, p2 = x.reshape(-1, K), pos.reshape(-1, K)
    x2 = x2 if x2.is_contiguous() else x2.contiguous()
    p2 = p2 if p2.is_contiguous() else p2.contiguous()
    mk = None
    if row_mask is not None:
        mk = row_mask.reshape(-1)
        if mk.dtype != torch.bool and mk.dtype != torch.uint8:
            mk = mk != 0
        mk = mk.contiguous()
    value = torch.empty((B * S, n_value), dtype=torch.float16, device=x.device)
    packed = torch.empty((B * S, n_packed), dtype=x.dtype, device=x.device)
    ok = [False]
    gen = getattr(pos, "_codetr_posgen", None) if ENC_POSGEN else None

    def launch():
        if gen is not None and gen["S"] == S and gen["B"] == B:
            ok[0] = _cabi.encoder_projections_posgen(x2, S, gen["cums"], gen["shapes"], gen["level_embed"], gen["temperature"],
                                                     gen["scale"], gen["eps"], gen["offset"], gen["normalize"], w_cat, b_cat,
                                                     mk, value, packed, S, int(head_dim))
            if ok[0]:
                return
        ok[0] = _cabi.encoder_projections(x2, p2, w_cat, b_cat, mk, value, packed, S, int(head_dim))

    with torch.cuda.device(x.device):
        if LINEAR_PROFILE is None:
            launch()
        else:
            st = torch.cuda.current_stream(x.device)
            e0, e1 = torch.cuda.Event(enable_timing=True), torch.cuda.Event(enable_timing=True)
            e0.record(st)
            launch()
            e1.record(st)
            if ok[0]:
                LINEAR_PROFILE.append((e0, e1, 2.0 * B * S * (n_value + n_packed) * K, B * S, n_value + n_packed, K))
    if not ok[0]:
        return None
    return value.view(B, n_value // head_dim, S, head_dim), packed.view(B, S, n_packed)


def msda_packed_projection(w_off, b_off, w_aw, b_aw, num_heads, num_levels, num_points):
    idx = _cabi.msda_pack_projection_index(num_heads, num_levels, num_points)
    if idx is None:
        return None
    ii = torch.tensor(idx, dtype=torch.long, device=w_off.device)
    wcat = torch.cat((w_off, w_aw), 0)
    bcat = torch.cat((b_off, b_aw), 0)
    pad = ii < 0
    wp = wcat[ii.clamp_min(0)].clone()
    bp = bcat[ii.clamp_min(0)].clone()
    wp[pad] = 0
    bp[pad] = 0
    return wp.contiguous(), bp.contiguous()


def msda_encoder_windows_packed(bias, level_shapes, num_heads, num_levels, num_points):
    import math

    b = bias.detach().float().cpu().view(num_heads, num_levels, num_points, 2)
    b = torch.round(b * 1024) / 1024
    lo, hi = b.amin(2).tolist(), b.amax(2).tolist()
    groups = [[0], [1, 2], [3, 4]]
    steps = int(2 * MSDA_V4_MARGIN_CAP)

    def window(m, l, mg):
        return (max(-127, math.floor(lo[m][l][0] - mg)), min(127, math.ceil(hi[m][l][0] + mg)),
                max(-127, math.floor(lo[m][l][1] - mg)), min(127, math.ceil(hi[m][l][1] + mg)))

    def need(trial):
        return _cabi.msda_encoder_packed_lds_bytes(level_shapes, num_heads, num_points, [trial] * num_heads,
                                                   MSDA_V4_REGION, MSDA_V4_THREADS)

    out = []
    for m in range(num_heads):
        win = [window(m, l, 0.0) for l in range(num_levels)]
        for grp in groups:
            a, z = 0, steps
            while a < z:
                mid = (a + z + 1) // 2
                trial = list(win)
                for l in grp:
                    trial[l] = window(m, l, 0.5 * mid)
                n = need(trial)
                if 0 < n <= MSDA_V4_LDS_BUDGET:
                    a = mid
                else:
                    z = mid - 1
            for l in grp:
                win[l] = window(m, l, 0.5 * a)
        out.append(win)
# ... 264 lines not shown
```

co-detr-tensorrt_amd/codetr/transformer.py:

```python
import math

import torch
import torch.nn as nn

from . import hip_ops
from .multi_scale_deformable_attention import MultiScaleDeformableAttention
from .transformer_layers import BaseTransformerLayer, DetrTransformerDecoderLayer, build_norm


DEC_FUSED = True
DEC_VPROJ = True


class DetrTransformerEncoder(nn.Module):
    def __init__(self, post_norm_cfg=dict(type="LN"), with_cp=-1, transformerlayers=None, num_layers=None,
                 init_cfg=None):
        super().__init__()
        if not isinstance(transformerlayers, dict):
            raise AssertionError("transformerlayers must be a dict")
        layer_cfg = dict(transformerlayers)
        if layer_cfg.pop("type") != "BaseTransformerLayer":
            raise AssertionError("encoder layers must be BaseTransformerLayer")
        self.num_layers = num_layers
        self.layers = nn.ModuleList(BaseTransformerLayer(**layer_cfg) for _ in range(num_layers))
# ... 306 lines not shown
def get_reference_points(mlvl_feats, valid_ratios, device):
    out = []
    for lvl, feat in enumerate(mlvl_feats):
        if isinstance(feat, tuple):
            (H, W), B, dt = feat, valid_ratios.shape[0], valid_ratios.dtype
        else:
            (B, _, H, W), dt = feat.shape, feat.dtype
        ys, xs = _pixel_centres(H, W, dt, device)
        y = ys / (valid_ratios[:, lvl, 1].reshape(B, 1) * H)
        x = xs / (valid_ratios[:, lvl, 0].reshape(B, 1) * W)
        out.append(torch.stack((x, y), -1))
    return torch.cat(out, 1)


_LVL_REPEATED = {}


def get_lvl_repeated(mlvl_masks, dtype=torch.float32):
    key = (tuple(m.shape[-2] * m.shape[-1] for m in mlvl_masks), dtype, str(mlvl_masks[0].device))
    hit = _LVL_REPEATED.get(key)
    if hit is None:
        hit = _LVL_REPEATED[key] = torch.cat([torch.full((n,), float(lvl), dtype=dtype, device=mlvl_masks[0].device)
                                              for lvl, n in enumerate(key[0])], 0)
    return hit


def make_encoder_output_proposals_export(reference_points, mlvl_masks):
    B, S = reference_points.shape[:2]
    wh = (0.05 * (2.0 ** get_lvl_repeated(mlvl_masks, dtype=reference_points.dtype))).expand(B, S).reshape(B, S, 1)
    prop = torch.cat((reference_points, wh, wh), dim=-1)
    return torch.log(prop / (1 - prop))


def make_encoder_output_proposals(reference_points, level_counts):
    B, S = reference_points.shape[:2]
    lvl = torch.repeat_interleave(
        torch.arange(level_counts.shape[0], dtype=reference_points.dtype, device=reference_points.device), level_counts)
    wh = (0.05 * (2.0 ** lvl)).expand(B, S).reshape(B, S, 1)
    prop = torch.cat((reference_points, wh, wh), dim=-1)
    return torch.log(prop / (1 - prop))


def apply_mask_to_proposal_and_memory(output_proposals, memory, memory_padding_mask):
    dt = output_proposals.dtype
    inside = ((output_proposals > -4.6) & (output_proposals < 4.6)).to(dt).prod(-1, keepdim=True)
    keep = inside * (~memory_padding_mask).to(dt).unsqueeze(-1)
    output_proposals = output_proposals * keep + (1.0 - keep) * torch.finfo(dt).max
    return output_proposals, memory * keep + (1.0 - keep) * 0.0


_SHAPE_TENSORS = {}
_LEVEL_WH = {}


def _level_wh(shapes, dtype, device):
    key = (tuple(tuple(s) for s in shapes), dtype, str(device))
    hit = _LEVEL_WH.get(key)
    if hit is None:
        hit = _LEVEL_WH[key] = torch.tensor([[float(w), float(h)] for h, w in shapes], dtype=dtype, device=device)
    return hit


def _shape_tensors(shapes, device):
    key = (tuple(shapes), str(device))
    hit = _SHAPE_TENSORS.get(key)
    if hit is None:
        ss = torch.as_tensor(shapes, dtype=torch.long, device=device)
        counts = ss.prod(1)
        ss._codetr_host = tuple((int(h), int(w)) for h, w in shapes)
        hit = (ss, torch.cat((ss.new_zeros((1,)), counts.cumsum(0)[:-1])))
        _SHAPE_TENSORS[key] = hit
    return hit


class CoDinoTransformer(nn.Module):
    def __init__(self, with_pos_coord=True, with_coord_feat=True, num_co_heads=1, as_two_stage=False,
                 num_feature_levels=4, two_stage_num_proposals=300, encoder=None, decoder=None, init_cfg=None):
        super().__init__()
        enc, dec = dict(encoder), dict(decoder)
        if enc.pop("type") != "DetrTransformerEncoder":
            raise AssertionError("encoder must be DetrTransformerEncoder")
        if dec.pop("type") != "DinoTransformerDecoder":
            raise AssertionError("decoder must be DinoTransformerDecoder")
        self.encoder = DetrTransformerEncoder(**enc)
        self.decoder = DinoTransformerDecoder(**dec)
        self.embed_dims = self.encoder.embed_dims
        self.with_pos_coord, self.with_coord_feat, self.num_co_heads = with_pos_coord, with_coord_feat, num_co_heads
        self.as_two_stage = as_two_stage
        self.num_feature_levels = num_feature_levels
        self.two_stage_num_proposals = two_stage_num_proposals
        self.init_layers()

    def init_layers(self):
        C = self.embed_dims
        self.level_embeds = nn.Parameter(torch.zeros(self.num_feature_levels, C))
        self.enc_output = nn.Linear(C, C)
        self.enc_output_norm = nn.LayerNorm(C)
        self.query_embed = nn.Embedding(self.two_stage_num_proposals, C)
        if self.with_pos_coord and self.num_co_heads > 0:
            self.aux_pos_trans = nn.ModuleList(nn.Linear(C * 2, C) for _ in range(self.num_co_heads))
            self.aux_pos_trans_norm = nn.ModuleList(nn.LayerNorm(C) for _ in range(self.num_co_heads))
            self.pos_feats_trans = nn.ModuleList()
            self.pos_feats_norm = nn.ModuleList()
            if self.with_coord_feat:
                self.pos_feats_trans.extend(nn.Linear(C, C) for _ in range(self.num_co_heads))
                self.pos_feats_norm.extend(nn.LayerNorm(C) for _ in range(self.num_co_heads))

    def init_weights(self):
        for p in self.parameters():
            if p.dim() > 1:
                nn.init.xavier_uniform_(p)
        for m in self.modules():
            if isinstance(m, MultiScaleDeformableAttention):
                m.init_weights()
        nn.init.normal_(self.level_embeds)
        nn.init.normal_(self.query_embed.weight)

    def forward(self, mlvl_feats, mlvl_masks, mlvl_pos_embeds, reg_branches=None, cls_branches=None,
                forced_topk_indices=None, capture=None, **kwargs):
        shapes = [tuple(f.shape[-2:]) for f in mlvl_feats]
        feat = torch.cat([f.flatten(2).transpose(1, 2) for f in mlvl_feats], 1)
        pos_tokens = [p.flatten(2).transpose(1, 2) for p in mlvl_pos_embeds]
        return self.forward_flat(feat, shapes, mlvl_masks, pos_tokens, reg_branches, cls_branches, forced_topk_indices,
                                 capture)

    def forward_flat(self, feat, shapes, mlvl_masks, mlvl_pos_tokens, reg_branches=None, cls_branches=None,
                     forced_topk_indices=None, capture=None, lvl_pos_embed_flat=None, mask_flat=None,
                     valid_counts=None):
        if not self.as_two_stage:
            raise AssertionError("as_two_stage must be True for DINO")
        dev = feat.device
        mask = mask_flat if mask_flat is not None else torch.cat([m.flatten(1) for m in mlvl_masks], 1)
        if lvl_pos_embed_flat is not None:
            pos = lvl_pos_embed_flat
        else:
            pos = torch.cat([p + self.level_embeds[l].view(1, 1, -1) for l, p in enumerate(mlvl_pos_tokens)], 1)
        spatial_shapes, level_start_index = _shape_tensors(shapes, dev)
        if valid_counts is not None:
            valid_ratios = hip_ops.valid_ratios(valid_counts, _level_wh(shapes, feat.dtype, dev))
        else:
            valid_ratios = torch.stack([get_valid_ratio(m, dtype=feat.dtype) for m in mlvl_masks], 1)
        native_geom = feat.is_cuda and feat.dtype in (torch.float16, torch.bfloat16) and mask.dtype == torch.bool
        if native_geom:
            reference_points, ref_by_level, proposals, row_state = hip_ops.encoder_geometry(valid_ratios, mask, shapes)
            if valid_counts is not None:
                ref_by_level._codetr_valid_counts = valid_counts
        else:
            reference_points = get_reference_points([tuple(s) for s in shapes], valid_ratios, device=dev)
            ref_by_level = reference_points[:, :, None] * valid_ratios[:, None]

        memory = self.encoder.forward_bf(feat, pos, mask, reference_points=ref_by_level, spatial_shapes=spatial_shapes,
                                         level_start_index=level_start_index)
        B = memory.shape[0]
        if native_geom:
            out_mem = hip_ops.linear(memory, self.enc_output.weight, self.enc_output.bias, row_mask=row_state)
        else:
            proposals = make_encoder_output_proposals_export(reference_points, mlvl_masks)
            proposals, out_mem = apply_mask_to_proposal_and_memory(proposals, memory, mask)
            out_mem = hip_ops.linear(out_mem, self.enc_output.weight, self.enc_output.bias)
        out_mem = hip_ops.layer_norm(out_mem, self.enc_output_norm.weight, self.enc_output_norm.bias,
                                     self.enc_output_norm.eps)
        last = self.decoder.num_layers
        cls_head = cls_branches[last]
        enc_cls = hip_ops.linear(out_mem, cls_head.weight, cls_head.bias)
        if forced_topk_indices is None:
            topk = hip_ops.topk(hip_ops.row_max(enc_cls), self.two_stage_num_proposals, want_values=False)[1]
        else:
            topk = forced_topk_indices
        sel = hip_ops.gather_rows(out_mem, topk)
        topk_coords = run_mlp(reg_branches[last], sel, residual=hip_ops.gather_rows(proposals, topk))
        qw = self.query_embed.weight
        if B == 1 or not qw.is_cuda or torch.is_grad_enabled():
            query = qw[None].expand(B, -1, -1)
        else:
            query = hip_ops.derived((qw,), f"_codetr_query_b{B}", lambda: qw.detach()[None].expand(B, -1, -1).contiguous())
        if capture is not None:
            enc_coord = run_mlp(reg_branches[last], out_mem) + proposals
            capture["topk_coords_unact"] = topk_coords
            capture.update(memory=memory, enc_outputs_class=enc_cls, enc_outputs_coord_unact=enc_coord,
                           topk_indices=topk, spatial_shapes=spatial_shapes, level_start_index=level_start_index,
                           valid_ratios=valid_ratios)
        return self.decoder.forward_bf(query, memory, mask, topk_coords, valid_ratios, reg_branches,
                                       spatial_shapes=spatial_shapes, level_start_index=level_start_index)
```

include/codetr_hip.h:

```cpp
#ifndef CODETR_HIP_H_
#define CODETR_HIP_H_

#include <stdint.h>

#ifdef __cplusplus
extern "C" {
#endif

#define CODETR_E_BADARG (-1)
#define CODETR_E_IM2COL_STEP (-2)
#define CODETR_E_TOO_LARGE (-3)
#define CODETR_E_UNSUPPORTED (-4)

#define CODETR_HIP_ABI_VERSION 54
int codetr_hip_abi_version(void);
const char *codetr_hip_strerror(int code);

int codetr_msda_forward_f16(void *stream, const void *value_dev, const int64_t *spatial_shapes_dev,
                            const int64_t *level_start_dev, const void *loc_dev, const void *weight_dev,
                            int64_t B, int64_t S, int M, int D, int L, int64_t Nq, int P, int64_t im2col_step,
                            void *out_dev);
int codetr_msda_forward_bf16(void *stream, const void *value_dev, const int64_t *spatial_shapes_dev,
                             const int64_t *level_start_dev, const void *loc_dev, const void *weight_dev,
                             int64_t B, int64_t S, int M, int D, int L, int64_t Nq, int P, int64_t im2col_step,
// ... 70 lines not shown
                              int stride, int pad, int is_bf16, void *y_dev);

int codetr_topk_f16(void *stream, const void *x_dev, int64_t rows, int64_t n, int k, void *values_dev,
                    int64_t *indices_dev);
int codetr_topk_bf16(void *stream, const void *x_dev, int64_t rows, int64_t n, int k, void *values_dev,
                     int64_t *indices_dev);

int64_t codetr_topk_chunks(int64_t n, int k, int64_t rows, int64_t *workspace_bytes);
int codetr_topk_chunked_f16(void *stream, const void *x_dev, int64_t rows, int64_t n, int k, int chunks,
                            void *values_dev, int64_t *indices_dev, void *workspace_dev, int64_t workspace_bytes);
int codetr_topk_chunked_bf16(void *stream, const void *x_dev, int64_t rows, int64_t n, int k, int chunks,
                             void *values_dev, int64_t *indices_dev, void *workspace_dev, int64_t workspace_bytes);

const char *codetr_msda_variant(int elem_bytes, int M, int D, int L, int P);

int codetr_linear_f16(void *stream, const void *x_dev, const void *w_dev, const void *bias_dev,
                      const void *residual_dev, const void *row_mask_dev, void *y_dev, int64_t M, int64_t N,
                      int64_t K, int act, int64_t hm_rows, int hm_head_dim);
int codetr_linear_bf16(void *stream, const void *x_dev, const void *w_dev, const void *bias_dev,
                       const void *residual_dev, const void *row_mask_dev, void *y_dev, int64_t M, int64_t N,
                       int64_t K, int act, int64_t hm_rows, int hm_head_dim);
int codetr_linear_bf16_f16out(void *stream, const void *x_dev, const void *w_dev, const void *bias_dev,
                              const void *row_mask_dev, void *y_dev, int64_t M, int64_t N, int64_t K,
                              int64_t hm_rows, int hm_head_dim);
int codetr_encoder_projections_f16(void *stream, const void *x_dev, const void *pos_dev, const void *w_dev,
                                   const void *bias_dev, const void *row_mask_dev, void *value_dev, void *packed_dev,
                                   int64_t M, int64_t N_value, int64_t N_packed, int64_t K, int64_t hm_rows,
                                   int hm_head_dim);
int codetr_encoder_projections_bf16(void *stream, const void *x_dev, const void *pos_dev, const void *w_dev,
                                    const void *bias_dev, const void *row_mask_dev, void *value_f16_dev,
                                    void *packed_dev, int64_t M, int64_t N_value, int64_t N_packed, int64_t K,
                                    int64_t hm_rows, int hm_head_dim);
int codetr_encoder_projections_posgen_f16(void *stream, const void *x_dev, const float *ycum0, const float *ycum1,
                                          const float *ycum2, const float *ycum3, const float *ycum4, const float *xcum0,
                                          const float *xcum1, const float *xcum2, const float *xcum3, const float *xcum4,
                                          const int64_t *level_shapes_host, int num_levels, const void *level_embed_dev,
                                          float temperature, float scale, float eps, float offset, int normalize,
                                          const void *w_dev, const void *bias_dev, const void *row_mask_dev, void *value_dev,
                                          void *packed_dev, int64_t M, int64_t S, int64_t N_value, int64_t N_packed, int64_t K,
                                          int64_t hm_rows, int hm_head_dim);
int codetr_encoder_projections_posgen_bf16(void *stream, const void *x_dev, const float *ycum0, const float *ycum1,
                                           const float *ycum2, const float *ycum3, const float *ycum4, const float *xcum0,
                                           const float *xcum1, const float *xcum2, const float *xcum3, const float *xcum4,
                                           const int64_t *level_shapes_host, int num_levels, const void *level_embed_dev,
                                           float temperature, float scale, float eps, float offset, int normalize,
                                           const void *w_dev, const void *bias_dev, const void *row_mask_dev,
                                           void *value_f16_dev, void *packed_dev, int64_t M, int64_t S, int64_t N_value,
                                           int64_t N_packed, int64_t K, int64_t hm_rows, int hm_head_dim);

const char *codetr_linear_variant(int64_t M, int64_t N, int64_t K, int act, int has_residual, int hm_head_dim);

int codetr_linear_xadd_f16(void *stream, const void *x_dev, const void *x_add_dev, const void *w_dev,
                           const void *bias_dev, void *y_dev, int64_t M, int64_t N, int64_t K);
int codetr_linear_xadd_bf16(void *stream, const void *x_dev, const void *x_add_dev, const void *w_dev,
                            const void *bias_dev, void *y_dev, int64_t M, int64_t N, int64_t K);

int codetr_linear_ln_f16(void *stream, const void *x_dev, const void *ln_gamma_dev, const void *ln_beta_dev,
                         float ln_eps, const void *w_dev, const void *bias_dev, void *y_dev, int64_t M, int64_t N,
                         int64_t K, int act);
int codetr_linear_ln_bf16(void *stream, const void *x_dev, const void *ln_gamma_dev, const void *ln_beta_dev,
                          float ln_eps, const void *w_dev, const void *bias_dev, void *y_dev, int64_t M, int64_t N,
                          int64_t K, int act);

int codetr_linear_fp8(void *stream, const void *x8_dev, const void *w8_dev, const float *w_scale_dev, float x_scale,
                      const void *bias_f16_dev, const void *residual_f16_dev, void *y_dev, int out_is_fp8,
                      float out_scale, int64_t M, int64_t N, int64_t K, int act);
int codetr_cast_fp8_f16(void *stream, const void *x_f16_dev, void *y8_dev, int64_t n, float scale);
int codetr_layernorm_fp8_f16(void *stream, const void *x_f16_dev, const void *gamma_f16_dev, const void *beta_f16_dev,
                             void *y8_dev, int64_t rows, int64_t C, float eps, float scale);

int64_t codetr_mx_scale_bytes(int64_t M, int64_t K);
int codetr_linear_fp8mx(void *stream, const void *x8_dev, const void *x_scales_dev, const void *w8_dev,
                        const float *w_scale_dev, const void *bias_f16_dev, const void *residual_f16_dev, void *y_dev,
                        void *y_scales_dev, int64_t M, int64_t N, int64_t K, int act);
int codetr_cast_fp8mx_f16(void *stream, const void *x_f16_dev, void *y8_dev, void *y_scales_dev, int64_t rows, int64_t C);
int codetr_layernorm_fp8mx_f16(void *stream, const void *x_f16_dev, const void *gamma_f16_dev, const void *beta_f16_dev,
                               void *y8_dev, void *y_scales_dev, int64_t rows, int64_t C, float eps);
int codetr_window_attention_fp8mx_f16(void *stream, const void *qkv_dev, const void *qkv_bias_dev,
                                      const void *rel_bias_dev, void *out8_dev, void *out_scales_dev, int64_t B, int64_t H,
                                      int64_t W, int num_heads, int head_dim, int window_size, int shift);

int codetr_add_f16(void *stream, const void *a_dev, const void *b_dev, void *out_dev, int64_t n, int64_t a_period);
int codetr_add_bf16(void *stream, const void *a_dev, const void *b_dev, void *out_dev, int64_t n, int64_t a_period);
int codetr_sigmoid_f16(void *stream, const void *x_dev, void *out_dev, int64_t n);
int codetr_sigmoid_bf16(void *stream, const void *x_dev, void *out_dev, int64_t n);
int codetr_gather_rows_b16(void *stream, const void *src_dev, const int64_t *idx_dev, void *out_dev, int64_t B, int64_t S,
                           int64_t K, int64_t C);
int codetr_decode_boxes_f16(void *stream, const void *coords_unact_dev, const int64_t *idx_dev, void *boxes_dev,
                            int64_t *labels_dev, int64_t B, int64_t Nq, int64_t K, int num_classes, float img_w,
                            float img_h);
int codetr_decode_boxes_bf16(void *stream, const void *coords_unact_dev, const int64_t *idx_dev, void *boxes_dev,
                            int64_t *labels_dev, int64_t B, int64_t Nq, int64_t K, int num_classes, float img_w,
                            float img_h);
int codetr_valid_ratios_f16(void *stream, const float *counts_dev, const void *level_wh_f16_dev, void *out_dev,
                            float *out32_dev, int64_t B, int L);
int codetr_valid_ratios_bf16(void *stream, const float *counts_dev, const void *level_wh_bf16_dev, void *out_dev,
                            float *out32_dev, int64_t B, int L);

int codetr_linear_splitk_plan(int64_t M, int64_t N, int64_t K, int64_t *workspace_bytes);
int codetr_linear_splitk_f16(void *stream, const void *x_dev, const void *w_dev, const void *bias_dev,
                             const void *residual_dev, const void *row_mask_dev, void *y_dev, int64_t M, int64_t N,
                             int64_t K, int act, int splits, void *workspace_dev, int64_t workspace_bytes);
int codetr_linear_splitk_bf16(void *stream, const void *x_dev, const void *w_dev, const void *bias_dev,
                              const void *residual_dev, const void *row_mask_dev, void *y_dev, int64_t M, int64_t N,
                              int64_t K, int act, int splits, void *workspace_dev, int64_t workspace_bytes);

int64_t codetr_linear_sk_workspace_bytes(void);
int codetr_linear_sk_supported(int64_t M, int64_t N, int64_t K);
int codetr_linear_sk_preferred(int64_t M, int64_t N, int64_t K, int act, int has_residual);
int codetr_linear_sk_f16(void *stream, const void *x_dev, const void *w_dev, const void *bias_dev,
                         const void *residual_dev, void *y_dev, int64_t M, int64_t N, int64_t K, int act,
                         void *workspace_dev, int64_t workspace_bytes, int flags);
int codetr_linear_sk_bf16(void *stream, const void *x_dev, const void *w_dev, const void *bias_dev,
                          const void *residual_dev, void *y_dev, int64_t M, int64_t N, int64_t K, int act,
                          void *workspace_dev, int64_t workspace_bytes, int flags);

int codetr_swin_mlp_supported(int64_t M, int64_t C, int64_t hidden);
int codetr_swin_mlp_f16(void *stream, const void *x_dev, const void *ln_gamma_dev, const void *ln_beta_dev, float ln_eps,
                        const void *w1_dev, const void *b1_dev, const void *w2_packed_dev, const void *b2_dev, void *y_dev,
                        int64_t M, int64_t C);
int codetr_swin_mlp_bf16(void *stream, const void *x_dev, const void *ln_gamma_dev, const void *ln_beta_dev, float ln_eps,
                         const void *w1_dev, const void *b1_dev, const void *w2_packed_dev, const void *b2_dev, void *y_dev,
                         int64_t M, int64_t C);

int codetr_linear_pp_supported(int64_t M, int64_t N, int64_t K);
int codetr_linear_pp_preferred(int64_t M, int64_t N, int64_t K, int act, int has_residual);
int codetr_linear_pp_f16(void *stream, const void *x_dev, const void *w_dev, const void *bias_dev,
                         const void *residual_dev, void *y_dev, int64_t M, int64_t N, int64_t K, int act, int flags);
int codetr_linear_pp_bf16(void *stream, const void *x_dev, const void *w_dev, const void *bias_dev,
                          const void *residual_dev, void *y_dev, int64_t M, int64_t N, int64_t K, int act, int flags);

int codetr_mask_pyramid(void *stream, const void *img_mask_dev, int64_t B, int64_t H_img, int64_t W_img,
                        int num_levels, const int64_t *level_shapes_host, void *mask_flat_dev, float *ycum_dev,
                        float *xcum_dev, float *valid_counts_dev, int mask_elem_bytes);

int codetr_query_sine_embed_f16(void *stream, const void *ref_dev, const void *valid_ratios_dev,
                                const float *valid_ratios32_dev, int64_t B, int64_t Nq, int ref_dim, int num_levels,
                                int pos_feat, float temperature, int apply_sigmoid, void *ref_in_dev,
                                float *ref_in32_dev, void *embed_dev);
int codetr_query_sine_embed_bf16(void *stream, const void *ref_dev, const void *valid_ratios_dev,
                                const float *valid_ratios32_dev, int64_t B, int64_t Nq, int ref_dim, int num_levels,
                                int pos_feat, float temperature, int apply_sigmoid, void *ref_in_dev,
                                float *ref_in32_dev, void *embed_dev);

int codetr_encoder_geometry_f16(void *stream, const void *valid_ratios_dev, const void *mask_flat_dev, int64_t B,
                                int num_levels, const int64_t *level_shapes_host, void *reference_points_dev,
                                void *reference_by_level_dev, void *proposals_dev, void *row_state_dev);
int codetr_encoder_geometry_bf16(void *stream, const void *valid_ratios_dev, const void *mask_flat_dev, int64_t B,
                                int num_levels, const int64_t *level_shapes_host, void *reference_points_dev,
                                void *reference_by_level_dev, void *proposals_dev, void *row_state_dev);

int codetr_row_max_f16(void *stream, const void *x_dev, void *out_dev, int64_t rows, int64_t C);
int codetr_row_max_bf16(void *stream, const void *x_dev, void *out_dev, int64_t rows, int64_t C);

int codetr_preprocess_u8_f16(void *stream, const void *src_dev, int64_t H_src, int64_t W_src, int64_t H_resized,
                             int64_t W_resized, int64_t H_pad, int64_t W_pad, const float *mean_host,
                             const float *std_host, const int *pad_value_host, void *dst_dev, void *mask_dev);
int codetr_preprocess_u8_f32(void *stream, const void *src_dev, int64_t H_src, int64_t W_src, int64_t H_resized,
                             int64_t W_resized, int64_t H_pad, int64_t W_pad, const float *mean_host,
                             const float *std_host, const int *pad_value_host, void *dst_dev, void *mask_dev);
int codetr_batched_nms_f32(void *stream, const float *boxes_sorted_dev, const int64_t *labels_sorted_dev, int64_t N,
                           float iou_threshold, void *keep_dev);

#define CODETR_PREPROCESS_BATCH_MAX 32
#define CODETR_POSTPROCESS_MAX_Q 1024
int codetr_preprocess_batch_u8_f16(void *stream, const void *src_dev, int64_t src_bytes, int64_t N,
                                   const int64_t *images_host, int64_t H, int64_t W, const float *mean_host,
                                   const float *std_host, const int *pad_value_host, float pad_fill, void *dst_dev,
                                   void *mask_dev);
int codetr_preprocess_batch_u8_bf16(void *stream, const void *src_dev, int64_t src_bytes, int64_t N,
                                    const int64_t *images_host, int64_t H, int64_t W, const float *mean_host,
                                    const float *std_host, const int *pad_value_host, float pad_fill, void *dst_dev,
                                    void *mask_dev);
int codetr_preprocess_batch_u8_f32(void *stream, const void *src_dev, int64_t src_bytes, int64_t N,
                                   const int64_t *images_host, int64_t H, int64_t W, const float *mean_host,
                                   const float *std_host, const int *pad_value_host, float pad_fill, void *dst_dev,
                                   void *mask_dev);
int codetr_postprocess_detections_f16(void *stream, const void *boxes_dev, const void *scores_dev,
                                      const int64_t *labels_dev, const void *divisor_dev, int64_t N, int64_t Q,
                                      int apply_threshold, float score_threshold, int apply_nms, float iou_threshold,
                                      void *boxes_out_dev, void *scores_out_dev, int64_t *labels_out_dev,
                                      int *count_dev);
int codetr_postprocess_detections_bf16(void *stream, const void *boxes_dev, const void *scores_dev,
                                       const int64_t *labels_dev, const void *divisor_dev, int64_t N, int64_t Q,
                                       int apply_threshold, float score_threshold, int apply_nms, float iou_threshold,
                                       void *boxes_out_dev, void *scores_out_dev, int64_t *labels_out_dev,
                                       int *count_dev);
int codetr_postprocess_detections_f32(void *stream, const void *boxes_dev, const void *scores_dev,
                                      const int64_t *labels_dev, const void *divisor_dev, int64_t N, int64_t Q,
                                      int apply_threshold, float score_threshold, int apply_nms, float iou_threshold,
                                      void *boxes_out_dev, void *scores_out_dev, int64_t *labels_out_dev,
                                      int *count_dev);
#define CODETR_SOFTNMS_NAIVE 0
#define CODETR_SOFTNMS_LINEAR 1
int codetr_postprocess_softnms_f16(void *stream, const void *boxes_dev, const void *scores_dev,
                                   const int64_t *labels_dev, const void *divisor_dev, int64_t N, int64_t Q,
                                   int apply_threshold, float score_threshold, int method, float iou_threshold,
                                   float min_score, int64_t max_keep, void *boxes_out_dev, void *scores_out_dev,
                                   int64_t *labels_out_dev, int *index_out_dev, int *count_dev);
int codetr_postprocess_softnms_bf16(void *stream, const void *boxes_dev, const void *scores_dev,
                                    const int64_t *labels_dev, const void *divisor_dev, int64_t N, int64_t Q,
                                    int apply_threshold, float score_threshold, int method, float iou_threshold,
                                    float min_score, int64_t max_keep, void *boxes_out_dev, void *scores_out_dev,
                                    int64_t *labels_out_dev, int *index_out_dev, int *count_dev);
int codetr_postprocess_softnms_f32(void *stream, const void *boxes_dev, const void *scores_dev,
                                   const int64_t *labels_dev, const void *divisor_dev, int64_t N, int64_t Q,
                                   int apply_threshold, float score_threshold, int method, float iou_threshold,
                                   float min_score, int64_t max_keep, void *boxes_out_dev, void *scores_out_dev,
                                   int64_t *labels_out_dev, int *index_out_dev, int *count_dev);

#define CODETR_TTA_MAX_VIEWS 16
#define CODETR_TTA_MAX_CANDIDATES 4096
#define CODETR_TTA_NMS_HARD 0
#define CODETR_TTA_NMS_SOFT_NAIVE 1
#define CODETR_TTA_NMS_SOFT_LINEAR 2
int codetr_preprocess_views_u8_f16(void *stream, const void *src_dev, int64_t src_bytes, int64_t N,
                                   const int64_t *images_host, int64_t H, int64_t W, const float *mean_host,
                                   const float *std_host, const int *pad_value_host, float pad_fill, void *dst_dev,
                                   void *mask_dev);
int codetr_preprocess_views_u8_bf16(void *stream, const void *src_dev, int64_t src_bytes, int64_t N,
                                    const int64_t *images_host, int64_t H, int64_t W, const float *mean_host,
                                    const float *std_host, const int *pad_value_host, float pad_fill, void *dst_dev,
                                    void *mask_dev);
int codetr_preprocess_views_u8_f32(void *stream, const void *src_dev, int64_t src_bytes, int64_t N,
                                   const int64_t *images_host, int64_t H, int64_t W, const float *mean_host,
                                   const float *std_host, const int *pad_value_host, float pad_fill, void *dst_dev,
                                   void *mask_dev);
int codetr_tta_merge_f16(void *stream, const void *boxes_dev, const void *scores_dev, const int64_t *labels_dev,
                         const int *count_dev, int64_t V, int64_t N, int64_t Q, uint32_t flip_mask,
                         const float *width_dev, int mode, float iou_threshold, float min_score, int64_t max_keep,
                         void *boxes_out_dev, void *scores_out_dev, int64_t *labels_out_dev, int *index_out_dev,
                         int *count_out_dev);
int codetr_tta_merge_bf16(void *stream, const void *boxes_dev, const void *scores_dev, const int64_t *labels_dev,
                          const int *count_dev, int64_t V, int64_t N, int64_t Q, uint32_t flip_mask,
                          const float *width_dev, int mode, float iou_threshold, float min_score, int64_t max_keep,
                          void *boxes_out_dev, void *scores_out_dev, int64_t *labels_out_dev, int *index_out_dev,
                          int *count_out_dev);
int codetr_tta_merge_f32(void *stream, const void *boxes_dev, const void *scores_dev, const int64_t *labels_dev,
                         const int *count_dev, int64_t V, int64_t N, int64_t Q, uint32_t flip_mask,
                         const float *width_dev, int mode, float iou_threshold, float min_score, int64_t max_keep,
                         void *boxes_out_dev, void *scores_out_dev, int64_t *labels_out_dev, int *index_out_dev,
                         int *count_out_dev);

int codetr_msda_backward_f16(void *stream, const void *value_dev, const int64_t *spatial_shapes_dev,
                             const int64_t *level_start_dev, const void *sampling_loc_dev, const void *attn_weight_dev,
                             const void *grad_output_dev, int64_t B, int64_t S, int M, int D, int L, int64_t Nq, int P,
                             int64_t im2col_step, void *grad_value_dev, void *grad_sampling_loc_dev,
                             void *grad_attn_weight_dev);
int codetr_msda_backward_f32(void *stream, const void *value_dev, const int64_t *spatial_shapes_dev,
                             const int64_t *level_start_dev, const void *sampling_loc_dev, const void *attn_weight_dev,
                             const void *grad_output_dev, int64_t B, int64_t S, int M, int D, int L, int64_t Nq, int P,
                             int64_t im2col_step, void *grad_value_dev, void *grad_sampling_loc_dev,
                             void *grad_attn_weight_dev);
int codetr_msda_backward_f64(void *stream, const void *value_dev, const int64_t *spatial_shapes_dev,
                             const int64_t *level_start_dev, const void *sampling_loc_dev, const void *attn_weight_dev,
                             const void *grad_output_dev, int64_t B, int64_t S, int M, int D, int L, int64_t Nq, int P,
                             int64_t im2col_step, void *grad_value_dev, void *grad_sampling_loc_dev,
                             void *grad_attn_weight_dev);

int codetr_layernorm_f16(void *stream, const void *x_dev, const void *gamma_dev, const void *beta_dev, void *y_dev,
                         int64_t rows, int64_t C, float eps);
int codetr_layernorm_bf16(void *stream, const void *x_dev, const void *gamma_dev, const void *beta_dev, void *y_dev,
                          int64_t rows, int64_t C, float eps);

int codetr_patch_merge_layernorm_f16(void *stream, const void *x_dev, const void *gamma_dev, const void *beta_dev,
                                     void *y_dev, int64_t B, int64_t H, int64_t W, int64_t C, float eps);
int codetr_patch_merge_layernorm_bf16(void *stream, const void *x_dev, const void *gamma_dev, const void *beta_dev,
                                     void *y_dev, int64_t B, int64_t H, int64_t W, int64_t C, float eps);

int codetr_window_attention_f16(void *stream, const void *qkv_dev, const void *qkv_bias_dev,
                                const void *rel_bias_dev, void *out_dev, int64_t B, int64_t H, int64_t W,
                                int num_heads, int head_dim, int window_size, int shift);
int codetr_window_attention_bf16(void *stream, const void *qkv_dev, const void *qkv_bias_dev,
                                 const void *rel_bias_dev, void *out_dev, int64_t B, int64_t H, int64_t W,
                                 int num_heads, int head_dim, int window_size, int shift);
int codetr_window_attention_fp8out_f16(void *stream, const void *qkv_dev, const void *qkv_bias_dev,
                                       const void *rel_bias_dev, void *out8_dev, float out_scale, int64_t B,
                                       int64_t H, int64_t W, int num_heads, int head_dim, int window_size, int shift);
int codetr_window_attention_ex(void *stream, const void *qkv_dev, const void *qkv_bias_dev, const void *rel_bias_dev,
                               void *out_dev, void *out_scales_dev, float out_scale, int64_t B, int64_t H, int64_t W,
                               int num_heads, int head_dim, int window_size, int shift, int elem, int out_mode,
                               int bias_layout);
int codetr_window_attention_bias_index(int window_size, int32_t *idx_host);

int codetr_mha_attention_f16(void *stream, const void *q_dev, const void *k_dev, const void *v_dev, void *out_dev,
                             int64_t B, int64_t Nq, int64_t Nk, int num_heads, int head_dim, int64_t q_row_stride,
                             int64_t k_row_stride, int64_t v_row_stride, int64_t out_row_stride);
int codetr_mha_attention_bf16(void *stream, const void *q_dev, const void *k_dev, const void *v_dev, void *out_dev,
                              int64_t B, int64_t Nq, int64_t Nk, int num_heads, int head_dim, int64_t q_row_stride,
                              int64_t k_row_stride, int64_t v_row_stride, int64_t out_row_stride);

int codetr_decoder_layer_supported(int embed_dims, int num_heads, int num_levels, int num_points, int hidden, int ref_dim,
                                   int pos_feat);
int64_t codetr_decoder_layer_blob_halfs(int which, int num_levels, int num_points, int hidden);
int codetr_decoder_layer_f16(void *stream, const void *x_dev, const void *attn_dev, const void *qpos_dev,
                             const void *ref_dev, const float *valid_ratios32_dev, const void *value_dev,
                             const int64_t *spatial_shapes_dev, const int64_t *level_start_dev, const void *tail_w_dev,
                             const void *pos_w_dev, const void *head_w_dev, const void *final_norm_dev, void *x_out_dev,
                             void *ref_out_dev, void *qpos_out_dev, void *qk_out_dev, void *v_out_dev, int64_t B,
                             int64_t Nq, int64_t S, int num_levels, int num_points, int hidden, float ln_eps,
                             float temperature);
int codetr_decoder_layer_bf16(void *stream, const void *x_dev, const void *attn_dev, const void *qpos_dev,
                             const void *ref_dev, const float *valid_ratios32_dev, const void *value_dev,
                             const int64_t *spatial_shapes_dev, const int64_t *level_start_dev, const void *tail_w_dev,
                             const void *pos_w_dev, const void *head_w_dev, const void *final_norm_dev, void *x_out_dev,
                             void *ref_out_dev, void *qpos_out_dev, void *qk_out_dev, void *v_out_dev, int64_t B,
// ... 64 lines not shown
```

runner/dispatch_gen.inc:

```
static const int kPlanAbi = 54;
static int call_codetr_msda_forward_f16(void* fn, const Arg* a) { typedef int (*F)(const void*, const void*, const void*, const void*, const void*, const void*, long long, long long, int, int, int, long long, int, long long, const void*); return ((F)fn)((const void*)a[0].p, (const void*)a[1].p, (const void*)a[2].p, (const void*)a[3].p, (const void*)a[4].p, (const void*)a[5].p, (long long)a[6].i, (long long)a[7].i, (int)a[8].i, (int)a[9].i, (int)a[10].i, (long long)a[11].i, (int)a[12].i, (long long)a[13].i, (const void*)a[14].p); }
static int call_codetr_msda_forward_bf16(void* fn, const Arg* a) { typedef int (*F)(const void*, const void*, const void*, const void*, const void*, const void*, long long, long long, int, int, int, long long, int, long long, const void*); return ((F)fn)((const void*)a[0].p, (const void*)a[1].p, (const void*)a[2].p, (const void*)a[3].p, (const void*)a[4].p, (const void*)a[5].p, (long long)a[6].i, (long long)a[7].i, (int)a[8].i, (int)a[9].i, (int)a[10].i, (long long)a[11].i, (int)a[12].i, (long long)a[13].i, (const void*)a[14].p); }
static int call_codetr_msda_forward_f32(void* fn, const Arg* a) { typedef int (*F)(const void*, const void*, const void*, const void*, const void*, const void*, long long, long long, int, int, int, long long, int, long long, const void*); return ((F)fn)((const void*)a[0].p, (const void*)a[1].p, (const void*)a[2].p, (const void*)a[3].p, (const void*)a[4].p, (const void*)a[5].p, (long long)a[6].i, (long long)a[7].i, (int)a[8].i, (int)a[9].i, (int)a[10].i, (long long)a[11].i, (int)a[12].i, (long long)a[13].i, (const void*)a[14].p); }
static int call_codetr_msda_forward_f64(void* fn, const Arg* a) { typedef int (*F)(const void*, const void*, const void*, const void*, const void*, const void*, long long, long long, int, int, int, long long, int, long long, const void*); return ((F)fn)((const void*)a[0].p, (const void*)a[1].p, (const void*)a[2].p, (const void*)a[3].p, (const void*)a[4].p, (const void*)a[5].p, (long long)a[6].i, (long long)a[7].i, (int)a[8].i, (int)a[9].i, (int)a[10].i, (long long)a[11].i, (int)a[12].i, (long long)a[13].i, (const void*)a[14].p); }
static int call_codetr_msda_backward_f16(void* fn, const Arg* a) { typedef int (*F)(const void*, const void*, const void*, const void*, const void*, const void*, const void*, long long, long long, int, int, int, long long, int, long long, const void*, const void*, const void*); return ((F)fn)((const void*)a[0].p, (const void*)a[1].p, (const void*)a[2].p, (const void*)a[3].p, (const void*)a[4].p, (const void*)a[5].p, (const void*)a[6].p, (long long)a[7].i, (long long)a[8].i, (int)a[9].i, (int)a[10].i, (int)a[11].i, (long long)a[12].i, (int)a[13].i, (long long)a[14].i, (const void*)a[15].p, (const void*)a[16].p, (const void*)a[17].p); }
static int call_codetr_msda_backward_f32(void* fn, const Arg* a) { typedef int (*F)(const void*, const void*, const void*, const void*, const void*, const void*, const void*, long long, long long, int, int, int, long long, int, long long, const void*, const void*, const void*); return ((F)fn)((const void*)a[0].p, (const void*)a[1].p, (const void*)a[2].p, (const void*)a[3].p, (const void*)a[4].p, (const void*)a[5].p, (const void*)a[6].p, (long long)a[7].i, (long long)a[8].i, (int)a[9].i, (int)a[10].i, (int)a[11].i, (long long)a[12].i, (int)a[13].i, (long long)a[14].i, (const void*)a[15].p, (const void*)a[16].p, (const void*)a[17].p); }
static int call_codetr_msda_backward_f64(void* fn, const Arg* a) { typedef int (*F)(const void*, const void*, const void*, const void*, const void*, const void*, const void*, long long, long long, int, int, int, long long, int, long long, const void*, const void*, const void*); return ((F)fn)((const void*)a[0].p, (const void*)a[1].p, (const void*)a[2].p, (const void*)a[3].p, (const void*)a[4].p, (const void*)a[5].p, (const void*)a[6].p, (long long)a[7].i, (long long)a[8].i, (int)a[9].i, (int)a[10].i, (int)a[11].i, (long long)a[12].i, (int)a[13].i, (long long)a[14].i, (const void*)a[15].p, (const void*)a[16].p, (const void*)a[17].p); }
static int call_codetr_msda_fused_forward_f16(void* fn, const Arg* a) { typedef int (*F)(const void*, const void*, const void*, const void*, const void*, long long, const void*, long long, const void*, int, int, long long, long long, int, int, int, long long, int, const void*); return ((F)fn)((const void*)a[0].p, (const void*)a[1].p, (const void*)a[2].p, (const void*)a[3].p, (const void*)a[4].p, (long long)a[5].i, (const void*)a[6].p, (long long)a[7].i, (const void*)a[8].p, (int)a[9].i, (int)a[10].i, (long long)a[11].i, (long long)a[12].i, (int)a[13].i, (int)a[14].i, (int)a[15].i, (long long)a[16].i, (int)a[17].i, (const void*)a[18].p); }
static int call_codetr_msda_fused_forward_bf16(void* fn, const Arg* a) { typedef int (*F)(const void*, const void*, const void*, const void*, const void*, long long, const void*, long long, const void*, int, int, long long, long long, int, int, int, long long, int, const void*); return ((F)fn)((const void*)a[0].p, (const void*)a[1].p, (const void*)a[2].p, (const void*)a[3].p, (const void*)a[4].p, (long long)a[5].i, (const void*)a[6].p, (long long)a[7].i, (const void*)a[8].p, (int)a[9].i, (int)a[10].i, (long long)a[11].i, (long long)a[12].i, (int)a[13].i, (int)a[14].i, (int)a[15].i, (long long)a[16].i, (int)a[17].i, (const void*)a[18].p); }
static int call_codetr_msda_fused_forward_ref32_f16(void* fn, const Arg* a) { typedef int (*F)(const void*, const void*, const void*, const void*, const void*, long long, const void*, long long, const void*, int, int, long long, long long, int, int, int, long long, int, const void*); return ((F)fn)((const void*)a[0].p, (const void*)a[1].p, (const void*)a[2].p, (const void*)a[3].p, (const void*)a[4].p, (long long)a[5].i, (const void*)a[6].p, (long long)a[7].i, (const void*)a[8].p, (int)a[9].i, (int)a[10].i, (long long)a[11].i, (long long)a[12].i, (int)a[13].i, (int)a[14].i, (int)a[15].i, (long long)a[16].i, (int)a[17].i, (const void*)a[18].p); }
static int call_codetr_msda_fused_forward_ref32_bf16(void* fn, const Arg* a) { typedef int (*F)(const void*, const void*, const void*, const void*, const void*, long long, const void*, long long, const void*, int, int, long long, long long, int, int, int, long long, int, const void*); return ((F)fn)((const void*)a[0].p, (const void*)a[1].p, (const void*)a[2].p, (const void*)a[3].p, (const void*)a[4].p, (long long)a[5].i, (const void*)a[6].p, (long long)a[7].i, (const void*)a[8].p, (int)a[9].i, (int)a[10].i, (long long)a[11].i, (long long)a[12].i, (int)a[13].i, (int)a[14].i, (int)a[15].i, (long long)a[16].i, (int)a[17].i, (const void*)a[18].p); }
static int call_codetr_msda_encoder_forward_packed_f16(void* fn, const Arg* a) { typedef int (*F)(const void*, const void*, const void*, const void*, long long, const void*, long long, long long, int, int, int, int, const void*, int, int, int, int, const void*); return ((F)fn)((const void*)a[0].p, (const void*)a[1].p, (const void*)a[2].p, (const void*)a[3].p, (long long)a[4].i, (const void*)a[5].p, (long long)a[6].i, (long long)a[7].i, (int)a[8].i, (int)a[9].i, (int)a[10].i, (int)a[11].i, (const void*)a[12].p, (int)a[13].i, (int)a[14].i, (int)a[15].i, (int)a[16].i, (const void*)a[17].p); }
static int call_codetr_msda_encoder_forward_packed_bf16(void* fn, const Arg* a) { typedef int (*F)(const void*, const void*, const void*, const void*, long long, const void*, long long, long long, int, int, int, int, const void*, int, int, int, int, const void*); return ((F)fn)((const void*)a[0].p, (const void*)a[1].p, (const void*)a[2].p, (const void*)a[3].p, (long long)a[4].i, (const void*)a[5].p, (long long)a[6].i, (long long)a[7].i, (int)a[8].i, (int)a[9].i, (int)a[10].i, (int)a[11].i, (const void*)a[12].p, (int)a[13].i, (int)a[14].i, (int)a[15].i, (int)a[16].i, (const void*)a[17].p); }
static int call_codetr_linear_bf16_f16out(void* fn, const Arg* a) { typedef int (*F)(const void*, const void*, const void*, const void*, const void*, const void*, long long, long long, long long, long long, int); return ((F)fn)((const void*)a[0].p, (const void*)a[1].p, (const void*)a[2].p, (const void*)a[3].p, (const void*)a[4].p, (const void*)a[5].p, (long long)a[6].i, (long long)a[7].i, (long long)a[8].i, (long long)a[9].i, (int)a[10].i); }
static int call_codetr_encoder_projections_f16(void* fn, const Arg* a) { typedef int (*F)(const void*, const void*, const void*, const void*, const void*, const void*, const void*, const void*, long long, long long, long long, long long, long long, int); return ((F)fn)((const void*)a[0].p, (const void*)a[1].p, (const void*)a[2].p, (const void*)a[3].p, (const void*)a[4].p, (const void*)a[5].p, (const void*)a[6].p, (const void*)a[7].p, (long long)a[8].i, (long long)a[9].i, (long long)a[10].i, (long long)a[11].i, (long long)a[12].i, (int)a[13].i); }
static int call_codetr_encoder_projections_bf16(void* fn, const Arg* a) { typedef int (*F)(const void*, const void*, const void*, const void*, const void*, const void*, const void*, const void*, long long, long long, long long, long long, long long, int); return ((F)fn)((const void*)a[0].p, (const void*)a[1].p, (const void*)a[2].p, (const void*)a[3].p, (const void*)a[4].p, (const void*)a[5].p, (const void*)a[6].p, (const void*)a[7].p, (long long)a[8].i, (long long)a[9].i, (long long)a[10].i, (long long)a[11].i, (long long)a[12].i, (int)a[13].i); }
static int call_codetr_encoder_projections_posgen_f16(void* fn, const Arg* a) { typedef int (*F)(const void*, const void*, const void*, const void*, const void*, const void*, const void*, const void*, const void*, const void*, const void*, const void*, const void*, int, const void*, float, float, float, float, int, const void*, const void*, const void*, const void*, const void*, long long, long long, long long, long long, long long, long long, int); return ((F)fn)((const void*)a[0].p, (const void*)a[1].p, (const void*)a[2].p, (const void*)a[3].p, (const void*)a[4].p, (const void*)a[5].p, (const void*)a[6].p, (const void*)a[7].p, (const void*)a[8].p, (const void*)a[9].p, (const void*)a[10].p, (const void*)a[11].p, (const void*)a[12].p, (int)a[13].i, (const void*)a[14].p, (float)a[15].f, (float)a[16].f, (float)a[17].f, (float)a[18].f, (int)a[19].i, (const void*)a[20].p, (const void*)a[21].p, (const void*)a[22].p, (const void*)a[23].p, (const void*)a[24].p, (long long)a[25].i, (long long)a[26].i, (long long)a[27].i, (long long)a[28].i, (long long)a[29].i, (long long)a[30].i, (int)a[31].i); }
static int call_codetr_encoder_projections_posgen_bf16(void* fn, const Arg* a) { typedef int (*F)(const void*, const void*, const void*, const void*, const void*, const void*, const void*, const void*, const void*, const void*, const void*, const void*, const void*, int, const void*, float, float, float, float, int, const void*, const void*, const void*, const void*, const void*, long long, long long, long long, long long, long long, long long, int); return ((F)fn)((const void*)a[0].p, (const void*)a[1].p, (const void*)a[2].p, (const void*)a[3].p, (const void*)a[4].p, (const void*)a[5].p, (const void*)a[6].p, (const void*)a[7].p, (const void*)a[8].p, (const void*)a[9].p, (const void*)a[10].p, (const void*)a[11].p, (const void*)a[12].p, (int)a[13].i, (const void*)a[14].p, (float)a[15].f, (float)a[16].f, (float)a[17].f, (float)a[18].f, (int)a[19].i, (const void*)a[20].p, (const void*)a[21].p, (const void*)a[22].p, (const void*)a[23].p, (const void*)a[24].p, (long long)a[25].i, (long long)a[26].i, (long long)a[27].i, (long long)a[28].i, (long long)a[29].i, (long long)a[30].i, (int)a[31].i); }
static int call_codetr_linear_fp8mx(void* fn, const Arg* a) { typedef int (*F)(const void*, const void*, const void*, const void*, const void*, const void*, const void*, const void*, const void*, long long, long long, long long, int); return ((F)fn)((const void*)a[0].p, (const void*)a[1].p, (const void*)a[2].p, (const void*)a[3].p, (const void*)a[4].p, (const void*)a[5].p, (const void*)a[6].p, (const void*)a[7].p, (const void*)a[8].p, (long long)a[9].i, (long long)a[10].i, (long long)a[11].i, (int)a[12].i); }
static int call_codetr_cast_fp8mx_f16(void* fn, const Arg* a) { typedef int (*F)(const void*, const void*, const void*, const void*, long long, long long); return ((F)fn)((const void*)a[0].p, (const void*)a[1].p, (const void*)a[2].p, (const void*)a[3].p, (long long)a[4].i, (long long)a[5].i); }
static int call_codetr_layernorm_fp8mx_f16(void* fn, const Arg* a) { typedef int (*F)(const void*, const void*, const void*, const void*, const void*, const void*, long long, long long, float); return ((F)fn)((const void*)a[0].p, (const void*)a[1].p, (const void*)a[2].p, (const void*)a[3].p, (const void*)a[4].p, (const void*)a[5].p, (long long)a[6].i, (long long)a[7].i, (float)a[8].f); }
static int call_codetr_window_attention_fp8mx_f16(void* fn, const Arg* a) { typedef int (*F)(const void*, const void*, const void*, const void*, const void*, const void*, long long, long long, long long, int, int, int, int); return ((F)fn)((const void*)a[0].p, (const void*)a[1].p, (const void*)a[2].p, (const void*)a[3].p, (const void*)a[4].p, (const void*)a[5].p, (long long)a[6].i, (long long)a[7].i, (long long)a[8].i, (int)a[9].i, (int)a[10].i, (int)a[11].i, (int)a[12].i); }
static int call_codetr_mha_attention_f16(void* fn, const Arg* a) { typedef int (*F)(const void*, const void*, const void*, const void*, const void*, long long, long long, long long, int, int, long long, long long, long long, long long); return ((F)fn)((const void*)a[0].p, (const void*)a[1].p, (const void*)a[2].p, (const void*)a[3].p, (const void*)a[4].p, (long long)a[5].i, (long long)a[6].i, (long long)a[7].i, (int)a[8].i, (int)a[9].i, (long long)a[10].i, (long long)a[11].i, (long long)a[12].i, (long long)a[13].i); }
static int call_codetr_mha_attention_bf16(void* fn, const Arg* a) { typedef int (*F)(const void*, const void*, const void*, const void*, const void*, long long, long long, long long, int, int, long long, long long, long long, long long); return ((F)fn)((const void*)a[0].p, (const void*)a[1].p, (const void*)a[2].p, (const void*)a[3].p, (const void*)a[4].p, (long long)a[5].i, (long long)a[6].i, (long long)a[7].i, (int)a[8].i, (int)a[9].i, (long long)a[10].i, (long long)a[11].i, (long long)a[12].i, (long long)a[13].i); }
static int call_codetr_linear_ln_f16(void* fn, const Arg* a) { typedef int (*F)(const void*, const void*, const void*, const void*, float, const void*, const void*, const void*, long long, long long, long long, int); return ((F)fn)((const void*)a[0].p, (const void*)a[1].p, (const void*)a[2].p, (const void*)a[3].p, (float)a[4].f, (const void*)a[5].p, (const void*)a[6].p, (const void*)a[7].p, (long long)a[8].i, (long long)a[9].i, (long long)a[10].i, (int)a[11].i); }
static int call_codetr_linear_ln_bf16(void* fn, const Arg* a) { typedef int (*F)(const void*, const void*, const void*, const void*, float, const void*, const void*, const void*, long long, long long, long long, int); return ((F)fn)((const void*)a[0].p, (const void*)a[1].p, (const void*)a[2].p, (const void*)a[3].p, (float)a[4].f, (const void*)a[5].p, (const void*)a[6].p, (const void*)a[7].p, (long long)a[8].i, (long long)a[9].i, (long long)a[10].i, (int)a[11].i); }
static int call_codetr_linear_xadd_f16(void* fn, const Arg* a) { typedef int (*F)(const void*, const void*, const void*, const void*, const void*, const void*, long long, long long, long long); return ((F)fn)((const void*)a[0].p, (const void*)a[1].p, (const void*)a[2].p, (const void*)a[3].p, (const void*)a[4].p, (const void*)a[5].p, (long long)a[6].i, (long long)a[7].i, (long long)a[8].i); }
static int call_codetr_linear_xadd_bf16(void* fn, const Arg* a) { typedef int (*F)(const void*, const void*, const void*, const void*, const void*, const void*, long long, long long, long long); return ((F)fn)((const void*)a[0].p, (const void*)a[1].p, (const void*)a[2].p, (const void*)a[3].p, (const void*)a[4].p, (const void*)a[5].p, (long long)a[6].i, (long long)a[7].i, (long long)a[8].i); }
static int call_codetr_im2col_tokens_b16(void* fn, const Arg* a) { typedef int (*F)(const void*, const void*, long long, long long, long long, long long, int, int, int, const void*); return ((F)fn)((const void*)a[0].p, (const void*)a[1].p, (long long)a[2].i, (long long)a[3].i, (long long)a[4].i, (long long)a[5].i, (int)a[6].i, (int)a[7].i, (int)a[8].i, (const void*)a[9].p); }
static int call_codetr_conv_tokens_f16(void* fn, const Arg* a) { typedef int (*F)(const void*, const void*, const void*, const void*, const void*, const void*, long long, long long, long long, long long, long long, int, int, int, int); return ((F)fn)((const void*)a[0].p, (const void*)a[1].p, (const void*)a[2].p, (const void*)a[3].p, (const void*)a[4].p, (const void*)a[5].p, (long long)a[6].i, (long long)a[7].i, (long long)a[8].i, (long long)a[9].i, (long long)a[10].i, (int)a[11].i, (int)a[12].i, (int)a[13].i, (int)a[14].i); }
static int call_codetr_conv_tokens_bf16(void* fn, const Arg* a) { typedef int (*F)(const void*, const void*, const void*, const void*, const void*, const void*, long long, long long, long long, long long, long long, int, int, int, int); return ((F)fn)((const void*)a[0].p, (const void*)a[1].p, (const void*)a[2].p, (const void*)a[3].p, (const void*)a[4].p, (const void*)a[5].p, (long long)a[6].i, (long long)a[7].i, (long long)a[8].i, (long long)a[9].i, (long long)a[10].i, (int)a[11].i, (int)a[12].i, (int)a[13].i, (int)a[14].i); }
static int call_codetr_conv_im2col_nchw_b16(void* fn, const Arg* a) { typedef int (*F)(const void*, const void*, long long, int, long long, long long, int, int, int, int, const void*); return ((F)fn)((const void*)a[0].p, (const void*)a[1].p, (long long)a[2].i, (int)a[3].i, (long long)a[4].i, (long long)a[5].i, (int)a[6].i, (int)a[7].i, (int)a[8].i, (int)a[9].i, (const void*)a[10].p); }
static int call_codetr_maxpool_tokens_b16(void* fn, const Arg* a) { typedef int (*F)(const void*, const void*, long long, long long, long long, long long, int, int, int, int, const void*); return ((F)fn)((const void*)a[0].p, (const void*)a[1].p, (long long)a[2].i, (long long)a[3].i, (long long)a[4].i, (long long)a[5].i, (int)a[6].i, (int)a[7].i, (int)a[8].i, (int)a[9].i, (const void*)a[10].p); }
static int call_codetr_topk_chunked_f16(void* fn, const Arg* a) { typedef int (*F)(const void*, const void*, long long, long long, int, int, const void*, const void*, const void*, long long); return ((F)fn)((const void*)a[0].p, (const void*)a[1].p, (long long)a[2].i, (long long)a[3].i, (int)a[4].i, (int)a[5].i, (const void*)a[6].p, (const void*)a[7].p, (const void*)a[8].p, (long long)a[9].i); }
static int call_codetr_topk_chunked_bf16(void* fn, const Arg* a) { typedef int (*F)(const void*, const void*, long long, long long, int, int, const void*, const void*, const void*, long long); return ((F)fn)((const void*)a[0].p, (const void*)a[1].p, (long long)a[2].i, (long long)a[3].i, (int)a[4].i, (int)a[5].i, (const void*)a[6].p, (const void*)a[7].p, (const void*)a[8].p, (long long)a[9].i); }
static int call_codetr_topk_f16(void* fn, const Arg* a) { typedef int (*F)(const void*, const void*, long long, long long, int, const void*, const void*); return ((F)fn)((const void*)a[0].p, (const void*)a[1].p, (long long)a[2].i, (long long)a[3].i, (int)a[4].i, (const void*)a[5].p, (const void*)a[6].p); }
static int call_codetr_topk_bf16(void* fn, const Arg* a) { typedef int (*F)(const void*, const void*, long long, long long, int, const void*, const void*); return ((F)fn)((const void*)a[0].p, (const void*)a[1].p, (long long)a[2].i, (long long)a[3].i, (int)a[4].i, (const void*)a[5].p, (const void*)a[6].p); }
static int call_codetr_patch_im2col_b16(void* fn, const Arg* a) { typedef int (*F)(const void*, const void*, long long, int, long long, long long, int, int, const void*); return ((F)fn)((const void*)a[0].p, (const void*)a[1].p, (long long)a[2].i, (int)a[3].i, (long long)a[4].i, (long long)a[5].i, (int)a[6].i, (int)a[7].i, (const void*)a[8].p); }
static int call_codetr_add_f16(void* fn, const Arg* a) { typedef int (*F)(const void*, const void*, const void*, const void*, long long, long long); return ((F)fn)((const void*)a[0].p, (const void*)a[1].p, (const void*)a[2].p, (const void*)a[3].p, (long long)a[4].i, (long long)a[5].i); }
static int call_codetr_add_bf16(void* fn, const Arg* a) { typedef int (*F)(const void*, const void*, const void*, const void*, long long, long long); return ((F)fn)((const void*)a[0].p, (const void*)a[1].p, (const void*)a[2].p, (const void*)a[3].p, (long long)a[4].i, (long long)a[5].i); }
static int call_codetr_sigmoid_f16(void* fn, const Arg* a) { typedef int (*F)(const void*, const void*, const void*, long long); return ((F)fn)((const void*)a[0].p, (const void*)a[1].p, (const void*)a[2].p, (long long)a[3].i); }
static int call_codetr_sigmoid_bf16(void* fn, const Arg* a) { typedef int (*F)(const void*, const void*, const void*, long long); return ((F)fn)((const void*)a[0].p, (const void*)a[1].p, (const void*)a[2].p, (long long)a[3].i); }
static int call_codetr_gather_rows_b16(void* fn, const Arg* a) { typedef int (*F)(const void*, const void*, const void*, const void*, long long, long long, long long, long long); return ((F)fn)((const void*)a[0].p, (const void*)a[1].p, (const void*)a[2].p, (const void*)a[3].p, (long long)a[4].i, (long long)a[5].i, (long long)a[6].i, (long long)a[7].i); }
static int call_codetr_decode_boxes_f16(void* fn, const Arg* a) { typedef int (*F)(const void*, const void*, const void*, const void*, const void*, long long, long long, long long, int, float, float); return ((F)fn)((const void*)a[0].p, (const void*)a[1].p, (const void*)a[2].p, (const void*)a[3].p, (const void*)a[4].p, (long long)a[5].i, (long long)a[6].i, (long long)a[7].i, (int)a[8].i, (float)a[9].f, (float)a[10].f); }
static int call_codetr_decode_boxes_bf16(void* fn, const Arg* a) { typedef int (*F)(const void*, const void*, const void*, const void*, const void*, long long, long long, long long, int, float, float); return ((F)fn)((const void*)a[0].p, (const void*)a[1].p, (const void*)a[2].p, (const void*)a[3].p, (const void*)a[4].p, (long long)a[5].i, (long long)a[6].i, (long long)a[7].i, (int)a[8].i, (float)a[9].f, (float)a[10].f); }
static int call_codetr_valid_ratios_f16(void* fn, const Arg* a) { typedef int (*F)(const void*, const void*, const void*, const void*, const void*, long long, int); return ((F)fn)((const void*)a[0].p, (const void*)a[1].p, (const void*)a[2].p, (const void*)a[3].p, (const void*)a[4].p, (long long)a[5].i, (int)a[6].i); }
static int call_codetr_valid_ratios_bf16(void* fn, const Arg* a) { typedef int (*F)(const void*, const void*, const void*, const void*, const void*, long long, int); return ((F)fn)((const void*)a[0].p, (const void*)a[1].p, (const void*)a[2].p, (const void*)a[3].p, (const void*)a[4].p, (long long)a[5].i, (int)a[6].i); }
static int call_codetr_linear_fp8(void* fn, const Arg* a) { typedef int (*F)(const void*, const void*, const void*, const void*, float, const void*, const void*, const void*, int, float, long long, long long, long long, int); return ((F)fn)((const void*)a[0].p, (const void*)a[1].p, (const void*)a[2].p, (const void*)a[3].p, (float)a[4].f, (const void*)a[5].p, (const void*)a[6].p, (const void*)a[7].p, (int)a[8].i, (float)a[9].f, (long long)a[10].i, (long long)a[11].i, (long long)a[12].i, (int)a[13].i); }
static int call_codetr_cast_fp8_f16(void* fn, const Arg* a) { typedef int (*F)(const void*, const void*, const void*, long long, float); return ((F)fn)((const void*)a[0].p, (const void*)a[1].p, (const void*)a[2].p, (long long)a[3].i, (float)a[4].f); }
static int call_codetr_layernorm_fp8_f16(void* fn, const Arg* a) { typedef int (*F)(const void*, const void*, const void*, const void*, const void*, long long, long long, float, float); return ((F)fn)((const void*)a[0].p, (const void*)a[1].p, (const void*)a[2].p, (const void*)a[3].p, (const void*)a[4].p, (long long)a[5].i, (long long)a[6].i, (float)a[7].f, (float)a[8].f); }
static int call_codetr_linear_f16(void* fn, const Arg* a) { typedef int (*F)(const void*, const void*, const void*, const void*, const void*, const void*, const void*, long long, long long, long long, int, long long, int); return ((F)fn)((const void*)a[0].p, (const void*)a[1].p, (const void*)a[2].p, (const void*)a[3].p, (const void*)a[4].p, (const void*)a[5].p, (const void*)a[6].p, (long long)a[7].i, (long long)a[8].i, (long long)a[9].i, (int)a[10].i, (long long)a[11].i, (int)a[12].i); }
static int call_codetr_linear_bf16(void* fn, const Arg* a) { typedef int (*F)(const void*, const void*, const void*, const void*, const void*, const void*, const void*, long long, long long, long long, int, long long, int); return ((F)fn)((const void*)a[0].p, (const void*)a[1].p, (const void*)a[2].p, (const void*)a[3].p, (const void*)a[4].p, (const void*)a[5].p, (const void*)a[6].p, (long long)a[7].i, (long long)a[8].i, (long long)a[9].i, (int)a[10].i, (long long)a[11].i, (int)a[12].i); }
static int call_codetr_query_sine_embed_f16(void* fn, const Arg* a) { typedef int (*F)(const void*, const void*, const void*, const void*, long long, long long, int, int, int, float, int, const void*, const void*, const void*); return ((F)fn)((const void*)a[0].p, (const void*)a[1].p, (const void*)a[2].p, (const void*)a[3].p, (long long)a[4].i, (long long)a[5].i, (int)a[6].i, (int)a[7].i, (int)a[8].i, (float)a[9].f, (int)a[10].i, (const void*)a[11].p, (const void*)a[12].p, (const void*)a[13].p); }
static int call_codetr_query_sine_embed_bf16(void* fn, const Arg* a) { typedef int (*F)(const void*, const void*, const void*, const void*, long long, long long, int, int, int, float, int, const void*, const void*, const void*); return ((F)fn)((const void*)a[0].p, (const void*)a[1].p, (const void*)a[2].p, (const void*)a[3].p, (long long)a[4].i, (long long)a[5].i, (int)a[6].i, (int)a[7].i, (int)a[8].i, (float)a[9].f, (int)a[10].i, (const void*)a[11].p, (const void*)a[12].p, (const void*)a[13].p); }
static int call_codetr_encoder_geometry_f16(void* fn, const Arg* a) { typedef int (*F)(const void*, const void*, const void*, long long, int, const void*, const void*, const void*, const void*, const void*); return ((F)fn)((const void*)a[0].p, (const void*)a[1].p, (const void*)a[2].p, (long long)a[3].i, (int)a[4].i, (const void*)a[5].p, (const void*)a[6].p, (const void*)a[7].p, (const void*)a[8].p, (const void*)a[9].p); }
static int call_codetr_encoder_geometry_bf16(void* fn, const Arg* a) { typedef int (*F)(const void*, const void*, const void*, long long, int, const void*, const void*, const void*, const void*, const void*); return ((F)fn)((const void*)a[0].p, (const void*)a[1].p, (const void*)a[2].p, (long long)a[3].i, (int)a[4].i, (const void*)a[5].p, (const void*)a[6].p, (const void*)a[7].p, (const void*)a[8].p, (const void*)a[9].p); }
static int call_codetr_row_max_f16(void* fn, const Arg* a) { typedef int (*F)(const void*, const void*, const void*, long long, long long); return ((F)fn)((const void*)a[0].p, (const void*)a[1].p, (const void*)a[2].p, (long long)a[3].i, (long long)a[4].i); }
static int call_codetr_row_max_bf16(void* fn, const Arg* a) { typedef int (*F)(const void*, const void*, const void*, long long, long long); return ((F)fn)((const void*)a[0].p, (const void*)a[1].p, (const void*)a[2].p, (long long)a[3].i, (long long)a[4].i); }
static int call_codetr_preprocess_u8_f16(void* fn, const Arg* a) { typedef int (*F)(const void*, const void*, long long, long long, long long, long long, long long, long long, const void*, const void*, const void*, const void*, const void*); return ((F)fn)((const void*)a[0].p, (const void*)a[1].p, (long long)a[2].i, (long long)a[3].i, (long long)a[4].i, (long long)a[5].i, (long long)a[6].i, (long long)a[7].i, (const void*)a[8].p, (const void*)a[9].p, (const void*)a[10].p, (const void*)a[11].p, (const void*)a[12].p); }
static int call_codetr_preprocess_u8_f32(void* fn, const Arg* a) { typedef int (*F)(const void*, const void*, long long, long long, long long, long long, long long, long long, const void*, const void*, const void*, const void*, const void*); return ((F)fn)((const void*)a[0].p, (const void*)a[1].p, (long long)a[2].i, (long long)a[3].i, (long long)a[4].i, (long long)a[5].i, (long long)a[6].i, (long long)a[7].i, (const void*)a[8].p, (const void*)a[9].p, (const void*)a[10].p, (const void*)a[11].p, (const void*)a[12].p); }
static int call_codetr_batched_nms_f32(void* fn, const Arg* a) { typedef int (*F)(const void*, const void*, const void*, long long, float, const void*); return ((F)fn)((const void*)a[0].p, (const void*)a[1].p, (const void*)a[2].p, (long long)a[3].i, (float)a[4].f, (const void*)a[5].p); }
static int call_codetr_preprocess_batch_u8_f16(void* fn, const Arg* a) { typedef int (*F)(const void*, const void*, long long, long long, const void*, long long, long long, const void*, const void*, const void*, float, const void*, const void*); return ((F)fn)((const void*)a[0].p, (const void*)a[1].p, (long long)a[2].i, (long long)a[3].i, (const void*)a[4].p, (long long)a[5].i, (long long)a[6].i, (const void*)a[7].p, (const void*)a[8].p, (const void*)a[9].p, (float)a[10].f, (const void*)a[11].p, (const void*)a[12].p); }
static int call_codetr_preprocess_batch_u8_bf16(void* fn, const Arg* a) { typedef int (*F)(const void*, const void*, long long, long long, const void*, long long, long long, const void*, const void*, const void*, float, const void*, const void*); return ((F)fn)((const void*)a[0].p, (const void*)a[1].p, (long long)a[2].i, (long long)a[3].i, (const void*)a[4].p, (long long)a[5].i, (long long)a[6].i, (const void*)a[7].p, (const void*)a[8].p, (const void*)a[9].p, (float)a[10].f, (const void*)a[11].p, (const void*)a[12].p); }
static int call_codetr_preprocess_batch_u8_f32(void* fn, const Arg* a) { typedef int (*F)(const void*, const void*, long long, long long, const void*, long long, long long, const void*, const void*, const void*, float, const void*, const void*); return ((F)fn)((const void*)a[0].p, (const void*)a[1].p, (long long)a[2].i, (long long)a[3].i, (const void*)a[4].p, (long long)a[5].i, (long long)a[6].i, (const void*)a[7].p, (const void*)a[8].p, (const void*)a[9].p, (float)a[10].f, (const void*)a[11].p, (const void*)a[12].p); }
static int call_codetr_postprocess_detections_f16(void* fn, const Arg* a) { typedef int (*F)(const void*, const void*, const void*, const void*, const void*, long long, long long, int, float, int, float, const void*, const void*, const void*, const void*); return ((F)fn)((const void*)a[0].p, (const void*)a[1].p, (const void*)a[2].p, (const void*)a[3].p, (const void*)a[4].p, (long long)a[5].i, (long long)a[6].i, (int)a[7].i, (float)a[8].f, (int)a[9].i, (float)a[10].f, (const void*)a[11].p, (const void*)a[12].p, (const void*)a[13].p, (const void*)a[14].p); }
static int call_codetr_postprocess_detections_bf16(void* fn, const Arg* a) { typedef int (*F)(const void*, const void*, const void*, const void*, const void*, long long, long long, int, float, int, float, const void*, const void*, const void*, const void*); return ((F)fn)((const void*)a[0].p, (const void*)a[1].p, (const void*)a[2].p, (const void*)a[3].p, (const void*)a[4].p, (long long)a[5].i, (long long)a[6].i, (int)a[7].i, (float)a[8].f, (int)a[9].i, (float)a[10].f, (const void*)a[11].p, (const void*)a[12].p, (const void*)a[13].p, (const void*)a[14].p); }
static int call_codetr_postprocess_detections_f32(void* fn, const Arg* a) { typedef int (*F)(const void*, const void*, const void*, const void*, const void*, long long, long long, int, float, int, float, const void*, const void*, const void*, const void*); return ((F)fn)((const void*)a[0].p, (const void*)a[1].p, (const void*)a[2].p, (const void*)a[3].p, (const void*)a[4].p, (long long)a[5].i, (long long)a[6].i, (int)a[7].i, (float)a[8].f, (int)a[9].i, (float)a[10].f, (const void*)a[11].p, (const void*)a[12].p, (const void*)a[13].p, (const void*)a[14].p); }
static int call_codetr_postprocess_softnms_f16(void* fn, const Arg* a) { typedef int (*F)(const void*, const void*, const void*, const void*, const void*, long long, long long, int, float, int, float, float, long long, const void*, const void*, const void*, const void*, const void*); return ((F)fn)((const void*)a[0].p, (const void*)a[1].p, (const void*)a[2].p, (const void*)a[3].p, (const void*)a[4].p, (long long)a[5].i, (long long)a[6].i, (int)a[7].i, (float)a[8].f, (int)a[9].i, (float)a[10].f, (float)a[11].f, (long long)a[12].i, (const void*)a[13].p, (const void*)a[14].p, (const void*)a[15].p, (const void*)a[16].p, (const void*)a[17].p); }
static int call_codetr_postprocess_softnms_bf16(void* fn, const Arg* a) { typedef int (*F)(const void*, const void*, const void*, const void*, const void*, long long, long long, int, float, int, float, float, long long, const void*, const void*, const void*, const void*, const void*); return ((F)fn)((const void*)a[0].p, (const void*)a[1].p, (const void*)a[2].p, (const void*)a[3].p, (const void*)a[4].p, (long long)a[5].i, (long long)a[6].i, (int)a[7].i, (float)a[8].f, (int)a[9].i, (float)a[10].f, (float)a[11].f, (long long)a[12].i, (const void*)a[13].p, (const void*)a[14].p, (const void*)a[15].p, (const void*)a[16].p, (const void*)a[17].p); }
static int call_codetr_postprocess_softnms_f32(void* fn, const Arg* a) { typedef int (*F)(const void*, const void*, const void*, const void*, const void*, long long, long long, int, float, int, float, float, long long, const void*, const void*, const void*, const void*, const void*); return ((F)fn)((const void*)a[0].p, (const void*)a[1].p, (const void*)a[2].p, (const void*)a[3].p, (const void*)a[4].p, (long long)a[5].i, (long long)a[6].i, (int)a[7].i, (float)a[8].f, (int)a[9].i, (float)a[10].f, (float)a[11].f, (long long)a[12].i, (const void*)a[13].p, (const void*)a[14].p, (const void*)a[15].p, (const void*)a[16].p, (const void*)a[17].p); }
static int call_codetr_preprocess_views_u8_f16(void* fn, const Arg* a) { typedef int (*F)(const void*, const void*, long long, long long, const void*, long long, long long, const void*, const void*, const void*, float, const void*, const void*); return ((F)fn)((const void*)a[0].p, (const void*)a[1].p, (long long)a[2].i, (long long)a[3].i, (const void*)a[4].p, (long long)a[5].i, (long long)a[6].i, (const void*)a[7].p, (const void*)a[8].p, (const void*)a[9].p, (float)a[10].f, (const void*)a[11].p, (const void*)a[12].p); }
static int call_codetr_preprocess_views_u8_bf16(void* fn, const Arg* a) { typedef int (*F)(const void*, const void*, long long, long long, const void*, long long, long long, const void*, const void*, const void*, float, const void*, const void*); return ((F)fn)((const void*)a[0].p, (const void*)a[1].p, (long long)a[2].i, (long long)a[3].i, (const void*)a[4].p, (long long)a[5].i, (long long)a[6].i, (const void*)a[7].p, (const void*)a[8].p, (const void*)a[9].p, (float)a[10].f, (const void*)a[11].p, (const void*)a[12].p); }
static int call_codetr_preprocess_views_u8_f32(void* fn, const Arg* a) { typedef int (*F)(const void*, const void*, long long, long long, const void*, long long, long long, const void*, const void*, const void*, float, const void*, const void*); return ((F)fn)((const void*)a[0].p, (const void*)a[1].p, (long long)a[2].i, (long long)a[3].i, (const void*)a[4].p, (long long)a[5].i, (long long)a[6].i, (const void*)a[7].p, (const void*)a[8].p, (const void*)a[9].p, (float)a[10].f, (const void*)a[11].p, (const void*)a[12].p); }
static int call_codetr_tta_merge_f16(void* fn, const Arg* a) { typedef int (*F)(const void*, const void*, const void*, const void*, const void*, long long, long long, long long, unsigned, const void*, int, float, float, long long, const void*, const void*, const void*, const void*, const void*); return ((F)fn)((const void*)a[0].p, (const void*)a[1].p, (const void*)a[2].p, (const void*)a[3].p, (const void*)a[4].p, (long long)a[5].i, (long long)a[6].i, (long long)a[7].i, (unsigned)a[8].i, (const void*)a[9].p, (int)a[10].i, (float)a[11].f, (float)a[12].f, (long long)a[13].i, (const void*)a[14].p, (const void*)a[15].p, (const void*)a[16].p, (const void*)a[17].p, (const void*)a[18].p); }
static int call_codetr_tta_merge_bf16(void* fn, const Arg* a) { typedef int (*F)(const void*, const void*, const void*, const void*, const void*, long long, long long, long long, unsigned, const void*, int, float, float, long long, const void*, const void*, const void*, const void*, const void*); return ((F)fn)((const void*)a[0].p, (const void*)a[1].p, (const void*)a[2].p, (const void*)a[3].p, (const void*)a[4].p, (long long)a[5].i, (long long)a[6].i, (long long)a[7].i, (unsigned)a[8].i, (const void*)a[9].p, (int)a[10].i, (float)a[11].f, (float)a[12].f, (long long)a[13].i, (const void*)a[14].p, (const void*)a[15].p, (const void*)a[16].p, (const void*)a[17].p, (const void*)a[18].p); }
static int call_codetr_tta_merge_f32(void* fn, const Arg* a) { typedef int (*F)(const void*, const void*, const void*, const void*, const void*, long long, long long, long long, unsigned, const void*, int, float, float, long long, const void*, const void*, const void*, const void*, const void*); return ((F)fn)((const void*)a[0].p, (const void*)a[1].p, (const void*)a[2].p, (const void*)a[3].p, (const void*)a[4].p, (long long)a[5].i, (long long)a[6].i, (long long)a[7].i, (unsigned)a[8].i, (const void*)a[9].p, (int)a[10].i, (float)a[11].f, (float)a[12].f, (long long)a[13].i, (const void*)a[14].p, (const void*)a[15].p, (const void*)a[16].p, (const void*)a[17].p, (const void*)a[18].p); }
static int call_codetr_patch_merge_layernorm_f16(void* fn, const Arg* a) { typedef int (*F)(const void*, const void*, const void*, const void*, const void*, long long, long long, long long, long long, float); return ((F)fn)((const void*)a[0].p, (const void*)a[1].p, (const void*)a[2].p, (const void*)a[3].p, (const void*)a[4].p, (long long)a[5].i, (long long)a[6].i, (long long)a[7].i, (long long)a[8].i, (float)a[9].f); }
static int call_codetr_patch_merge_layernorm_bf16(void* fn, const Arg* a) { typedef int (*F)(const void*, const void*, const void*, const void*, const void*, long long, long long, long long, long long, float); return ((F)fn)((const void*)a[0].p, (const void*)a[1].p, (const void*)a[2].p, (const void*)a[3].p, (const void*)a[4].p, (long long)a[5].i, (long long)a[6].i, (long long)a[7].i, (long long)a[8].i, (float)a[9].f); }
static int call_codetr_mask_pyramid(void* fn, const Arg* a) { typedef int (*F)(const void*, const void*, long long, long long, long long, int, const void*, const void*, const void*, const void*, const void*, int); return ((F)fn)((const void*)a[0].p, (const void*)a[1].p, (long long)a[2].i, (long long)a[3].i, (long long)a[4].i, (int)a[5].i, (const void*)a[6].p, (const void*)a[7].p, (const void*)a[8].p, (const void*)a[9].p, (const void*)a[10].p, (int)a[11].i); }
static int call_codetr_linear_splitk_f16(void* fn, const Arg* a) { typedef int (*F)(const void*, const void*, const void*, const void*, const void*, const void*, const void*, long long, long long, long long, int, int, const void*, long long); return ((F)fn)((const void*)a[0].p, (const void*)a[1].p, (const void*)a[2].p, (const void*)a[3].p, (const void*)a[4].p, (const void*)a[5].p, (const void*)a[6].p, (long long)a[7].i, (long long)a[8].i, (long long)a[9].i, (int)a[10].i, (int)a[11].i, (const void*)a[12].p, (long long)a[13].i); }
static int call_codetr_linear_splitk_bf16(void* fn, const Arg* a) { typedef int (*F)(const void*, const void*, const void*, const void*, const void*, const void*, const void*, long long, long long, long long, int, int, const void*, long long); return ((F)fn)((const void*)a[0].p, (const void*)a[1].p, (const void*)a[2].p, (const void*)a[3].p, (const void*)a[4].p, (const void*)a[5].p, (const void*)a[6].p, (long long)a[7].i, (long long)a[8].i, (long long)a[9].i, (int)a[10].i, (int)a[11].i, (const void*)a[12].p, (long long)a[13].i); }
static int call_codetr_linear_sk_f16(void* fn, const Arg* a) { typedef int (*F)(const void*, const void*, const void*, const void*, const void*, const void*, long long, long long, long long, int, const void*, long long, int); return ((F)fn)((const void*)a[0].p, (const void*)a[1].p, (const void*)a[2].p, (const void*)a[3].p, (const void*)a[4].p, (const void*)a[5].p, (long long)a[6].i, (long long)a[7].i, (long long)a[8].i, (int)a[9].i, (const void*)a[10].p, (long long)a[11].i, (int)a[12].i); }
static int call_codetr_msda_op4_forward_f16(void* fn, const Arg* a) { typedef int (*F)(const void*, const void*, const void*, const void*, const void*, const void*, long long, long long, int, int, int, long long, int, const void*); return ((F)fn)((const void*)a[0].p, (const void*)a[1].p, (const void*)a[2].p, (const void*)a[3].p, (const void*)a[4].p, (const void*)a[5].p, (long long)a[6].i, (long long)a[7].i, (int)a[8].i, (int)a[9].i, (int)a[10].i, (long long)a[11].i, (int)a[12].i, (const void*)a[13].p); }
static int call_codetr_msda_op4_forward_bf16(void* fn, const Arg* a) { typedef int (*F)(const void*, const void*, const void*, const void*, const void*, const void*, long long, long long, int, int, int, long long, int, const void*); return ((F)fn)((const void*)a[0].p, (const void*)a[1].p, (const void*)a[2].p, (const void*)a[3].p, (const void*)a[4].p, (const void*)a[5].p, (long long)a[6].i, (long long)a[7].i, (int)a[8].i, (int)a[9].i, (int)a[10].i, (long long)a[11].i, (int)a[12].i, (const void*)a[13].p); }
static int call_codetr_swin_mlp_f16(void* fn, const Arg* a) { typedef int (*F)(const void*, const void*, const void*, const void*, float, const void*, const void*, const void*, const void*, const void*, long long, long long); return ((F)fn)((const void*)a[0].p, (const void*)a[1].p, (const void*)a[2].p, (const void*)a[3].p, (float)a[4].f, (const void*)a[5].p, (const void*)a[6].p, (const void*)a[7].p, (const void*)a[8].p, (const void*)a[9].p, (long long)a[10].i, (long long)a[11].i); }
static int call_codetr_swin_mlp_bf16(void* fn, const Arg* a) { typedef int (*F)(const void*, const void*, const void*, const void*, float, const void*, const void*, const void*, const void*, const void*, long long, long long); return ((F)fn)((const void*)a[0].p, (const void*)a[1].p, (const void*)a[2].p, (const void*)a[3].p, (float)a[4].f, (const void*)a[5].p, (const void*)a[6].p, (const void*)a[7].p, (const void*)a[8].p, (const void*)a[9].p, (long long)a[10].i, (long long)a[11].i); }
static int call_codetr_linear_pp_f16(void* fn, const Arg* a) { typedef int (*F)(const void*, const void*, const void*, const void*, const void*, const void*, long long, long long, long long, int, int); return ((F)fn)((const void*)a[0].p, (const void*)a[1].p, (const void*)a[2].p, (const void*)a[3].p, (const void*)a[4].p, (const void*)a[5].p, (long long)a[6].i, (long long)a[7].i, (long long)a[8].i, (int)a[9].i, (int)a[10].i); }
static int call_codetr_linear_pp_bf16(void* fn, const Arg* a) { typedef int (*F)(const void*, const void*, const void*, const void*, const void*, const void*, long long, long long, long long, int, int); return ((F)fn)((const void*)a[0].p, (const void*)a[1].p, (const void*)a[2].p, (const void*)a[3].p, (const void*)a[4].p, (const void*)a[5].p, (long long)a[6].i, (long long)a[7].i, (long long)a[8].i, (int)a[9].i, (int)a[10].i); }
static int call_codetr_linear_sk_bf16(void* fn, const Arg* a) { typedef int (*F)(const void*, const void*, const void*, const void*, const void*, const void*, long long, long long, long long, int, const void*, long long, int); return ((F)fn)((const void*)a[0].p, (const void*)a[1].p, (const void*)a[2].p, (const void*)a[3].p, (const void*)a[4].p, (const void*)a[5].p, (long long)a[6].i, (long long)a[7].i, (long long)a[8].i, (int)a[9].i, (const void*)a[10].p, (long long)a[11].i, (int)a[12].i); }
static int call_codetr_decoder_layer_f16(void* fn, const Arg* a) { typedef int (*F)(const void*, const void*, const void*, const void*, const void*, const void*, const void*, const void*, const void*, const void*, const void*, const void*, const void*, const void*, const void*, const void*, const void*, const void*, long long, long long, long long, int, int, int, float, float); return ((F)fn)((const void*)a[0].p, (const void*)a[1].p, (const void*)a[2].p, (const void*)a[3].p, (const void*)a[4].p, (const void*)a[5].p, (const void*)a[6].p, (const void*)a[7].p, (const void*)a[8].p, (const void*)a[9].p, (const void*)a[10].p, (const void*)a[11].p, (const void*)a[12].p, (const void*)a[13].p, (const void*)a[14].p, (const void*)a[15].p, (const void*)a[16].p, (const void*)a[17].p, (long long)a[18].i, (long long)a[19].i, (long long)a[20].i, (int)a[21].i, (int)a[22].i, (int)a[23].i, (float)a[24].f, (float)a[25].f); }
static int call_codetr_decoder_layer_bf16(void* fn, const Arg* a) { typedef int (*F)(const void*, const void*, const void*, const void*, const void*, const void*, const void*, const void*, const void*, const void*, const void*, const void*, const void*, const void*, const void*, const void*, const void*, const void*, long long, long long, long long, int, int, int, float, float); return ((F)fn)((const void*)a[0].p, (const void*)a[1].p, (const void*)a[2].p, (const void*)a[3].p, (const void*)a[4].p, (const void*)a[5].p, (const void*)a[6].p, (const void*)a[7].p, (const void*)a[8].p, (const void*)a[9].p, (const void*)a[10].p, (const void*)a[11].p, (const void*)a[12].p, (const void*)a[13].p, (const void*)a[14].p, (const void*)a[15].p, (const void*)a[16].p, (const void*)a[17].p, (long long)a[18].i, (long long)a[19].i, (long long)a[20].i, (int)a[21].i, (int)a[22].i, (int)a[23].i, (float)a[24].f, (float)a[25].f); }
static int call_codetr_layernorm_f16(void* fn, const Arg* a) { typedef int (*F)(const void*, const void*, const void*, const void*, const void*, long long, long long, float); return ((F)fn)((const void*)a[0].p, (const void*)a[1].p, (const void*)a[2].p, (const void*)a[3].p, (const void*)a[4].p, (long long)a[5].i, (long long)a[6].i, (float)a[7].f); }
static int call_codetr_layernorm_bf16(void* fn, const Arg* a) { typedef int (*F)(const void*, const void*, const void*, const void*, const void*, long long, long long, float); return ((F)fn)((const void*)a[0].p, (const void*)a[1].p, (const void*)a[2].p, (const void*)a[3].p, (const void*)a[4].p, (long long)a[5].i, (long long)a[6].i, (float)a[7].f); }
static int call_codetr_groupnorm_tokens_f16(void* fn, const Arg* a) { typedef int (*F)(const void*, const void*, const void*, const void*, const void*, long long, const void*, long long, long long, long long, int, float); return ((F)fn)((const void*)a[0].p, (const void*)a[1].p, (const void*)a[2].p, (const void*)a[3].p, (const void*)a[4].p, (long long)a[5].i, (const void*)a[6].p, (long long)a[7].i, (long long)a[8].i, (long long)a[9].i, (int)a[10].i, (float)a[11].f); }
static int call_codetr_groupnorm_tokens_bf16(void* fn, const Arg* a) { typedef int (*F)(const void*, const void*, const void*, const void*, const void*, long long, const void*, long long, long long, long long, int, float); return ((F)fn)((const void*)a[0].p, (const void*)a[1].p, (const void*)a[2].p, (const void*)a[3].p, (const void*)a[4].p, (long long)a[5].i, (const void*)a[6].p, (long long)a[7].i, (long long)a[8].i, (long long)a[9].i, (int)a[10].i, (float)a[11].f); }
static int call_codetr_sine_pos_tokens_f16(void* fn, const Arg* a) { typedef int (*F)(const void*, const void*, const void*, const void*, const void*, long long, long long, long long, long long, int, float, float, float, float, int); return ((F)fn)((const void*)a[0].p, (const void*)a[1].p, (const void*)a[2].p, (const void*)a[3].p, (const void*)a[4].p, (long long)a[5].i, (long long)a[6].i, (long long)a[7].i, (long long)a[8].i, (int)a[9].i, (float)a[10].f, (float)a[11].f, (float)a[12].f, (float)a[13].f, (int)a[14].i); }
static int call_codetr_sine_pos_tokens_bf16(void* fn, const Arg* a) { typedef int (*F)(const void*, const void*, const void*, const void*, const void*, long long, long long, long long, long long, int, float, float, float, float, int); return ((F)fn)((const void*)a[0].p, (const void*)a[1].p, (const void*)a[2].p, (const void*)a[3].p, (const void*)a[4].p, (long long)a[5].i, (long long)a[6].i, (long long)a[7].i, (long long)a[8].i, (int)a[9].i, (float)a[10].f, (float)a[11].f, (float)a[12].f, (float)a[13].f, (int)a[14].i); }
static int call_codetr_ffn_relu_f16(void* fn, const Arg* a) { typedef int (*F)(const void*, const void*, const void*, const void*, const void*, const void*, const void*, long long, long long, long long); return ((F)fn)((const void*)a[0].p, (const void*)a[1].p, (const void*)a[2].p, (const void*)a[3].p, (const void*)a[4].p, (const void*)a[5].p, (const void*)a[6].p, (long long)a[7].i, (long long)a[8].i, (long long)a[9].i); }
static int call_codetr_ffn_relu_ln_f16(void* fn, const Arg* a) { typedef int (*F)(const void*, const void*, const void*, const void*, const void*, const void*, const void*, long long, long long, long long, const void*, const void*, float, const void*, const void*); return ((F)fn)((const void*)a[0].p, (const void*)a[1].p, (const void*)a[2].p, (const void*)a[3].p, (const void*)a[4].p, (const void*)a[5].p, (const void*)a[6].p, (long long)a[7].i, (long long)a[8].i, (long long)a[9].i, (const void*)a[10].p, (const void*)a[11].p, (float)a[12].f, (const void*)a[13].p, (const void*)a[14].p); }
static int call_codetr_ffn_relu_ln2_f16(void* fn, const Arg* a) { typedef int (*F)(const void*, const void*, const void*, const void*, const void*, const void*, const void*, long long, long long, long long, const void*, const void*, float, const void*, const void*, float, const void*, const void*); return ((F)fn)((const void*)a[0].p, (const void*)a[1].p, (const void*)a[2].p, (const void*)a[3].p, (const void*)a[4].p, (const void*)a[5].p, (const void*)a[6].p, (long long)a[7].i, (long long)a[8].i, (long long)a[9].i, (const void*)a[10].p, (const void*)a[11].p, (float)a[12].f, (const void*)a[13].p, (const void*)a[14].p, (float)a[15].f, (const void*)a[16].p, (const void*)a[17].p); }
static int call_codetr_ffn_relu_ln2_bf16(void* fn, const Arg* a) { typedef int (*F)(const void*, const void*, const void*, const void*, const void*, const void*, const void*, long long, long long, long long, const void*, const void*, float, const void*, const void*, float, const void*, const void*); return ((F)fn)((const void*)a[0].p, (const void*)a[1].p, (const void*)a[2].p, (const void*)a[3].p, (const void*)a[4].p, (const void*)a[5].p, (const void*)a[6].p, (long long)a[7].i, (long long)a[8].i, (long long)a[9].i, (const void*)a[10].p, (const void*)a[11].p, (float)a[12].f, (const void*)a[13].p, (const void*)a[14].p, (float)a[15].f, (const void*)a[16].p, (const void*)a[17].p); }
static int call_codetr_ffn_pack_w2_f16(void* fn, const Arg* a) { typedef int (*F)(const void*, const void*, const void*, long long, long long); return ((F)fn)((const void*)a[0].p, (const void*)a[1].p, (const void*)a[2].p, (long long)a[3].i, (long long)a[4].i); }
static int call_codetr_ffn_oproj_relu_ln2_f16(void* fn, const Arg* a) { typedef int (*F)(const void*, const void*, const void*, const void*, const void*, const void*, const void*, const void*, const void*, const void*, long long, long long, long long, const void*, const void*, float, const void*, const void*, float, const void*, const void*); return ((F)fn)((const void*)a[0].p, (const void*)a[1].p, (const void*)a[2].p, (const void*)a[3].p, (const void*)a[4].p, (const void*)a[5].p, (const void*)a[6].p, (const void*)a[7].p, (const void*)a[8].p, (const void*)a[9].p, (long long)a[10].i, (long long)a[11].i, (long long)a[12].i, (const void*)a[13].p, (const void*)a[14].p, (float)a[15].f, (const void*)a[16].p, (const void*)a[17].p, (float)a[18].f, (const void*)a[19].p, (const void*)a[20].p); }
static int call_codetr_ffn_oproj_relu_ln2_bf16(void* fn, const Arg* a) { typedef int (*F)(const void*, const void*, const void*, const void*, const void*, const void*, const void*, const void*, const void*, const void*, long long, long long, long long, const void*, const void*, float, const void*, const void*, float, const void*, const void*); return ((F)fn)((const void*)a[0].p, (const void*)a[1].p, (const void*)a[2].p, (const void*)a[3].p, (const void*)a[4].p, (const void*)a[5].p, (const void*)a[6].p, (const void*)a[7].p, (const void*)a[8].p, (const void*)a[9].p, (long long)a[10].i, (long long)a[11].i, (long long)a[12].i, (const void*)a[13].p, (const void*)a[14].p, (float)a[15].f, (const void*)a[16].p, (const void*)a[17].p, (float)a[18].f, (const void*)a[19].p, (const void*)a[20].p); }
static int call_codetr_ffn_fp8(void* fn, const Arg* a) { typedef int (*F)(const void*, const void*, const void*, const void*, const void*, const void*, const void*, const void*, const void*, long long, long long, long long, float, float, const void*, const void*, float, const void*, const void*, float, const void*, const void*); return ((F)fn)((const void*)a[0].p, (const void*)a[1].p, (const void*)a[2].p, (const void*)a[3].p, (const void*)a[4].p, (const void*)a[5].p, (const void*)a[6].p, (const void*)a[7].p, (const void*)a[8].p, (long long)a[9].i, (long long)a[10].i, (long long)a[11].i, (float)a[12].f, (float)a[13].f, (const void*)a[14].p, (const void*)a[15].p, (float)a[16].f, (const void*)a[17].p, (const void*)a[18].p, (float)a[19].f, (const void*)a[20].p, (const void*)a[21].p); }
static int call_codetr_window_attention_f16(void* fn, const Arg* a) { typedef int (*F)(const void*, const void*, const void*, const void*, const void*, long long, long long, long long, int, int, int, int); return ((F)fn)((const void*)a[0].p, (const void*)a[1].p, (const void*)a[2].p, (const void*)a[3].p, (const void*)a[4].p, (long long)a[5].i, (long long)a[6].i, (long long)a[7].i, (int)a[8].i, (int)a[9].i, (int)a[10].i, (int)a[11].i); }
static int call_codetr_window_attention_bf16(void* fn, const Arg* a) { typedef int (*F)(const void*, const void*, const void*, const void*, const void*, long long, long long, long long, int, int, int, int); return ((F)fn)((const void*)a[0].p, (const void*)a[1].p, (const void*)a[2].p, (const void*)a[3].p, (const void*)a[4].p, (long long)a[5].i, (long long)a[6].i, (long long)a[7].i, (int)a[8].i, (int)a[9].i, (int)a[10].i, (int)a[11].i); }
static int call_codetr_window_attention_ex(void* fn, const Arg* a) { typedef int (*F)(const void*, const void*, const void*, const void*, const void*, const void*, float, long long, long long, long long, int, int, int, int, int, int, int); return ((F)fn)((const void*)a[0].p, (const void*)a[1].p, (const void*)a[2].p, (const void*)a[3].p, (const void*)a[4].p, (const void*)a[5].p, (float)a[6].f, (long long)a[7].i, (long long)a[8].i, (long long)a[9].i, (int)a[10].i, (int)a[11].i, (int)a[12].i, (int)a[13].i, (int)a[14].i, (int)a[15].i, (int)a[16].i); }
static int call_codetr_window_attention_fp8out_f16(void* fn, const Arg* a) { typedef int (*F)(const void*, const void*, const void*, const void*, const void*, float, long long, long long, long long, int, int, int, int); return ((F)fn)((const void*)a[0].p, (const void*)a[1].p, (const void*)a[2].p, (const void*)a[3].p, (const void*)a[4].p, (float)a[5].f, (long long)a[6].i, (long long)a[7].i, (long long)a[8].i, (int)a[9].i, (int)a[10].i, (int)a[11].i, (int)a[12].i); }
static const Entry kEntries[] = {
  {"codetr_msda_forward_f16", 15, call_codetr_msda_forward_f16},
  {"codetr_msda_forward_bf16", 15, call_codetr_msda_forward_bf16},
  {"codetr_msda_forward_f32", 15, call_codetr_msda_forward_f32},
  {"codetr_msda_forward_f64", 15, call_codetr_msda_forward_f64},
  {"codetr_msda_backward_f16", 18, call_codetr_msda_backward_f16},
  {"codetr_msda_backward_f32", 18, call_codetr_msda_backward_f32},
  {"codetr_msda_backward_f64", 18, call_codetr_msda_backward_f64},
  {"codetr_msda_fused_forward_f16", 19, call_codetr_msda_fused_forward_f16},
  {"codetr_msda_fused_forward_bf16", 19, call_codetr_msda_fused_forward_bf16},
  {"codetr_msda_fused_forward_ref32_f16", 19, call_codetr_msda_fused_forward_ref32_f16},
  {"codetr_msda_fused_forward_ref32_bf16", 19, call_codetr_msda_fused_forward_ref32_bf16},
  {"codetr_msda_encoder_forward_packed_f16", 18, call_codetr_msda_encoder_forward_packed_f16},
  {"codetr_msda_encoder_forward_packed_bf16", 18, call_codetr_msda_encoder_forward_packed_bf16},
  {"codetr_linear_bf16_f16out", 11, call_codetr_linear_bf16_f16out},
  {"codetr_encoder_projections_f16", 14, call_codetr_encoder_projections_f16},
  {"codetr_encoder_projections_bf16", 14, call_codetr_encoder_projections_bf16},
  {"codetr_encoder_projections_posgen_f16", 32, call_codetr_encoder_projections_posgen_f16},
  {"codetr_encoder_projections_posgen_bf16", 32, call_codetr_encoder_projections_posgen_bf16},
  {"codetr_linear_fp8mx", 13, call_codetr_linear_fp8mx},
  {"codetr_cast_fp8mx_f16", 6, call_codetr_cast_fp8mx_f16},
  {"codetr_layernorm_fp8mx_f16", 9, call_codetr_layernorm_fp8mx_f16},
  {"codetr_window_attention_fp8mx_f16", 13, call_codetr_window_attention_fp8mx_f16},
  {"codetr_mha_attention_f16", 14, call_codetr_mha_attention_f16},
  {"codetr_mha_attention_bf16", 14, call_codetr_mha_attention_bf16},
  {"codetr_linear_ln_f16", 12, call_codetr_linear_ln_f16},
  {"codetr_linear_ln_bf16", 12, call_codetr_linear_ln_bf16},
  {"codetr_linear_xadd_f16", 9, call_codetr_linear_xadd_f16},
  {"codetr_linear_xadd_bf16", 9, call_codetr_linear_xadd_bf16},
  {"codetr_im2col_tokens_b16", 10, call_codetr_im2col_tokens_b16},
  {"codetr_conv_tokens_f16", 15, call_codetr_conv_tokens_f16},
  {"codetr_conv_tokens_bf16", 15, call_codetr_conv_tokens_bf16},
  {"codetr_conv_im2col_nchw_b16", 11, call_codetr_conv_im2col_nchw_b16},
  {"codetr_maxpool_tokens_b16", 11, call_codetr_maxpool_tokens_b16},
  {"codetr_topk_chunked_f16", 10, call_codetr_topk_chunked_f16},
  {"codetr_topk_chunked_bf16", 10, call_codetr_topk_chunked_bf16},
  {"codetr_topk_f16", 7, call_codetr_topk_f16},
  {"codetr_topk_bf16", 7, call_codetr_topk_bf16},
  {"codetr_patch_im2col_b16", 9, call_codetr_patch_im2col_b16},
  {"codetr_add_f16", 6, call_codetr_add_f16},
  {"codetr_add_bf16", 6, call_codetr_add_bf16},
  {"codetr_sigmoid_f16", 4, call_codetr_sigmoid_f16},
  {"codetr_sigmoid_bf16", 4, call_codetr_sigmoid_bf16},
  {"codetr_gather_rows_b16", 8, call_codetr_gather_rows_b16},
  {"codetr_decode_boxes_f16", 11, call_codetr_decode_boxes_f16},
  {"codetr_decode_boxes_bf16", 11, call_codetr_decode_boxes_bf16},
  {"codetr_valid_ratios_f16", 7, call_codetr_valid_ratios_f16},
  {"codetr_valid_ratios_bf16", 7, call_codetr_valid_ratios_bf16},
  {"codetr_linear_fp8", 14, call_codetr_linear_fp8},
  {"codetr_cast_fp8_f16", 5, call_codetr_cast_fp8_f16},
  {"codetr_layernorm_fp8_f16", 9, call_codetr_layernorm_fp8_f16},
  {"codetr_linear_f16", 13, call_codetr_linear_f16},
  {"codetr_linear_bf16", 13, call_codetr_linear_bf16},
  {"codetr_query_sine_embed_f16", 14, call_codetr_query_sine_embed_f16},
  {"codetr_query_sine_embed_bf16", 14, call_codetr_query_sine_embed_bf16},
  {"codetr_encoder_geometry_f16", 10, call_codetr_encoder_geometry_f16},
  {"codetr_encoder_geometry_bf16", 10, call_codetr_encoder_geometry_bf16},
  {"codetr_row_max_f16", 5, call_codetr_row_max_f16},
  {"codetr_row_max_bf16", 5, call_codetr_row_max_bf16},
  {"codetr_preprocess_u8_f16", 13, call_codetr_preprocess_u8_f16},
  {"codetr_preprocess_u8_f32", 13, call_codetr_preprocess_u8_f32},
  {"codetr_batched_nms_f32", 6, call_codetr_batched_nms_f32},
  {"codetr_preprocess_batch_u8_f16", 13, call_codetr_preprocess_batch_u8_f16},
  {"codetr_preprocess_batch_u8_bf16", 13, call_codetr_preprocess_batch_u8_bf16},
  {"codetr_preprocess_batch_u8_f32", 13, call_codetr_preprocess_batch_u8_f32},
  {"codetr_postprocess_detections_f16", 15, call_codetr_postprocess_detections_f16},
  {"codetr_postprocess_detections_bf16", 15, call_codetr_postprocess_detections_bf16},
  {"codetr_postprocess_detections_f32", 15, call_codetr_postprocess_detections_f32},
  {"codetr_postprocess_softnms_f16", 18, call_codetr_postprocess_softnms_f16},
  {"codetr_postprocess_softnms_bf16", 18, call_codetr_postprocess_softnms_bf16},
  {"codetr_postprocess_softnms_f32", 18, call_codetr_postprocess_softnms_f32},
  {"codetr_preprocess_views_u8_f16", 13, call_codetr_preprocess_views_u8_f16},
  {"codetr_preprocess_views_u8_bf16", 13, call_codetr_preprocess_views_u8_bf16},
  {"codetr_preprocess_views_u8_f32", 13, call_codetr_preprocess_views_u8_f32},
  {"codetr_tta_merge_f16", 19, call_codetr_tta_merge_f16},
  {"codetr_tta_merge_bf16", 19, call_codetr_tta_merge_bf16},
  {"codetr_tta_merge_f32", 19, call_codetr_tta_merge_f32},
  {"codetr_patch_merge_layernorm_f16", 10, call_codetr_patch_merge_layernorm_f16},
  {"codetr_patch_merge_layernorm_bf16", 10, call_codetr_patch_merge_layernorm_bf16},
  {"codetr_mask_pyramid", 12, call_codetr_mask_pyramid},
  {"codetr_linear_splitk_f16", 14, call_codetr_linear_splitk_f16},
  {"codetr_linear_splitk_bf16", 14, call_codetr_linear_splitk_bf16},
  {"codetr_linear_sk_f16", 13, call_codetr_linear_sk_f16},
  {"codetr_msda_op4_forward_f16", 14, call_codetr_msda_op4_forward_f16},
  {"codetr_msda_op4_forward_bf16", 14, call_codetr_msda_op4_forward_bf16},
  {"codetr_swin_mlp_f16", 12, call_codetr_swin_mlp_f16},
  {"codetr_swin_mlp_bf16", 12, call_codetr_swin_mlp_bf16},
  {"codetr_linear_pp_f16", 11, call_codetr_linear_pp_f16},
  {"codetr_linear_pp_bf16", 11, call_codetr_linear_pp_bf16},
  {"codetr_linear_sk_bf16", 13, call_codetr_linear_sk_bf16},
  {"codetr_decoder_layer_f16", 26, call_codetr_decoder_layer_f16},
  {"codetr_decoder_layer_bf16", 26, call_codetr_decoder_layer_bf16},
  {"codetr_layernorm_f16", 8, call_codetr_layernorm_f16},
  {"codetr_layernorm_bf16", 8, call_codetr_layernorm_bf16},
  {"codetr_groupnorm_tokens_f16", 12, call_codetr_groupnorm_tokens_f16},
  {"codetr_groupnorm_tokens_bf16", 12, call_codetr_groupnorm_tokens_bf16},
  {"codetr_sine_pos_tokens_f16", 15, call_codetr_sine_pos_tokens_f16},
  {"codetr_sine_pos_tokens_bf16", 15, call_codetr_sine_pos_tokens_bf16},
  {"codetr_ffn_relu_f16", 10, call_codetr_ffn_relu_f16},
  {"codetr_ffn_relu_ln_f16", 15, call_codetr_ffn_relu_ln_f16},
  {"codetr_ffn_relu_ln2_f16", 18, call_codetr_ffn_relu_ln2_f16},
  {"codetr_ffn_relu_ln2_bf16", 18, call_codetr_ffn_relu_ln2_bf16},
  {"codetr_ffn_pack_w2_f16", 5, call_codetr_ffn_pack_w2_f16},
  {"codetr_ffn_oproj_relu_ln2_f16", 21, call_codetr_ffn_oproj_relu_ln2_f16},
  {"codetr_ffn_oproj_relu_ln2_bf16", 21, call_codetr_ffn_oproj_relu_ln2_bf16},
  {"codetr_ffn_fp8", 22, call_codetr_ffn_fp8},
  {"codetr_window_attention_f16", 12, call_codetr_window_attention_f16},
  {"codetr_window_attention_bf16", 12, call_codetr_window_attention_bf16},
  {"codetr_window_attention_ex", 17, call_codetr_window_attention_ex},
  {"codetr_window_attention_fp8out_f16", 13, call_codetr_window_attention_fp8out_f16},
};
```

Measured before the change: 101.4.

## Fuse encoder output projection, LayerNorm, class head and row max into one kernel

Adds an encoder_score kernel that computes the two-stage scoring path (enc_output linear, LayerNorm, class-branch linear, row max) in one launch without writing the full normalized memory or class logits to global memory. After top-k, the same kernel runs again on only the selected rows to produce their normalized features, replacing a gather from the full out_mem tensor. This cuts several launches and large intermediate tensors, at the cost of recomputing the projection and LayerNorm for the selected rows.

Result: no change. 101.7, median of 6 (+0.4%).

```diff
diff --git a/co-detr-tensorrt_amd/codetr/_cabi.py b/co-detr-tensorrt_amd/codetr/_cabi.py
--- a/co-detr-tensorrt_amd/codetr/_cabi.py
+++ b/co-detr-tensorrt_amd/codetr/_cabi.py
@@ -91,6 +91,8 @@
     "codetr_encoder_geometry_bf16": (_i32, [_vp, _vp, _vp, _i64, _i32, _vp, _vp, _vp, _vp, _vp]),
     "codetr_row_max_f16": (_i32, [_vp, _vp, _vp, _i64, _i64]),
     "codetr_row_max_bf16": (_i32, [_vp, _vp, _vp, _i64, _i64]),
+    "codetr_encoder_score_f16": (_i32, [_vp] * 8 + [ctypes.c_float] + [_vp] * 4 + [_i64] * 5),
+    "codetr_encoder_score_bf16": (_i32, [_vp] * 8 + [ctypes.c_float] + [_vp] * 4 + [_i64] * 5),
     "codetr_preprocess_u8_f16": (_i32, [_vp, _vp, _i64, _i64, _i64, _i64, _i64, _i64, _vp, _vp, _vp, _vp, _vp]),
     "codetr_preprocess_u8_f32": (_i32, [_vp, _vp, _i64, _i64, _i64, _i64, _i64, _i64, _vp, _vp, _vp, _vp, _vp]),
     "codetr_batched_nms_f32": (_i32, [_vp, _vp, _vp, _i64, ctypes.c_float, _vp]),
@@ -182,7 +184,7 @@
 
 CALLS = {"encoder_projections_posgen": 0, "msda": 0, "msda_fused": 0, "linear": 0, "layernorm": 0, "window_attention": 0, "groupnorm_tokens": 0,
          "sine_pos_tokens": 0, "ffn_fused": 0, "ffn_oproj_fused": 0, "linear_splitk": 0, "linear_sk": 0, "mask_pyramid": 0,
-         "query_sine_embed": 0, "encoder_geometry": 0, "row_max": 0, "preprocess": 0, "batched_nms": 0,
+         "query_sine_embed": 0, "encoder_geometry": 0, "row_max": 0, "encoder_score": 0, "preprocess": 0, "batched_nms": 0,
          "preprocess_batch": 0, "postprocess_detections": 0, "postprocess_softnms": 0,
          "preprocess_views": 0, "tta_merge": 0,
          "msda_backward": 0, "patch_merge_layernorm": 0, "msda_encoder": 0, "msda_encoder_packed": 0, "patch_im2col": 0, "mha_attention": 0, "topk": 0,
@@ -469,6 +471,28 @@
     rc = fn(current_stream_ptr(x2d.device), x2d.data_ptr(), out.data_ptr(), rows, C)
     check(rc, "codetr_row_max_f16")
     return out
+
+
+def encoder_score_supported(memory, num_classes) -> bool:
+    return (memory.dtype in (torch.float16, torch.bfloat16) and memory.dim() == 3 and memory.shape[-1] == 256
+            and 0 < num_classes <= 128)
+
+
+def encoder_score(memory, row_state, index, w_enc, b_enc, gamma, beta, eps, w_cls, b_cls, want_score, want_rows):
+    B, S, C = memory.shape
+    Nq = 0 if index is None else index.shape[1]
+    R = S if index is None else Nq
+    nc = w_cls.shape[0]
+    score = torch.empty((B, R), dtype=memory.dtype, device=memory.device) if want_score else None
+    rows = torch.empty((B, R, C), dtype=memory.dtype, device=memory.device) if want_rows else None
+    fn = load().codetr_encoder_score_bf16 if memory.dtype == torch.bfloat16 else load().codetr_encoder_score_f16
+    rc = fn(current_stream_ptr(memory.device), memory.data_ptr(), None if row_state is None else row_state.data_ptr(),
+            None if index is None else index.data_ptr(), w_enc.data_ptr(), b_enc.data_ptr(), gamma.data_ptr(),
+            beta.data_ptr(), float(eps), w_cls.data_ptr(), b_cls.data_ptr(), None if score is None else score.data_ptr(),
+            None if rows is None else rows.data_ptr(), B, S, Nq, C, nc)
+    check(rc, "codetr_encoder_score_f16")
+    CALLS["encoder_score"] += 1
+    return score, rows
 
 
 def preprocess_u8(src, resized_hw, pad_hw, mean, std, pad_value, dtype, with_mask=True):
diff --git a/co-detr-tensorrt_amd/codetr/_kernel_names.py b/co-detr-tensorrt_amd/codetr/_kernel_names.py
--- a/co-detr-tensorrt_amd/codetr/_kernel_names.py
+++ b/co-detr-tensorrt_amd/codetr/_kernel_names.py
@@ -8,6 +8,7 @@
     "decode_boxes_kernel",
     "decoder_layer_kernel",
     "encoder_geometry_kernel",
+    "encoder_score_kernel",
     "ffn_fp8_kernel",
     "ffn_fused_kernel",
     "gather_rows_kernel",
diff --git a/co-detr-tensorrt_amd/codetr/hip_ops.py b/co-detr-tensorrt_amd/codetr/hip_ops.py
--- a/co-detr-tensorrt_amd/codetr/hip_ops.py
+++ b/co-detr-tensorrt_amd/codetr/hip_ops.py
@@ -12,6 +12,7 @@
           "mask_pyramid(level masks + running valid counts + valid ratios)",
           "query_sine_embed(f16: sigmoid x valid ratios + sine embedding of the decoder reference boxes)",
           "encoder_geometry(f16: reference points, proposals, keep/drop state)", "row_max(f16)",
+          "encoder_score(f16/bf16: enc_output + LayerNorm + class branch + row max of the two-stage scoring, one launch)",
           "preprocess_image(u8 -> f16/f32, cv2-exact resize + pad + normalise + mask)", "batched_nms(f32)",
           "preprocess_batch(u8 -> f16/bf16/f32, <= 32 images of any size per launch, stacked + padded)",
           "postprocess_detections(f16/bf16/f32: threshold + sort + per-class NMS + rescale, one workgroup per image)",
@@ -412,6 +413,32 @@
         return _cabi.row_max(x.view(-1, x.shape[-1])).view(x.shape[:-1])
 
 
+ENC_SCORE = True
+
+
+def encoder_score_supported(memory, row_state, enc_output, enc_norm, cls_head):
+    if not ENC_SCORE or torch.is_grad_enabled() or not memory.is_cuda or not memory.is_contiguous():
+        return False
+    ps = (enc_output.weight, enc_output.bias, enc_norm.weight, enc_norm.bias, cls_head.weight, cls_head.bias)
+    if any(p is None for p in ps) or not _cabi.encoder_score_supported(memory, cls_head.weight.shape[0]):
+        return False
+    C = memory.shape[-1]
+    return (tuple(enc_output.weight.shape) == (C, C) and tuple(enc_norm.weight.shape) == (C,)
+            and cls_head.weight.shape[1] == C and memory.data_ptr() % 16 == 0
+            and (row_state is None or (row_state.dtype == torch.uint8 and row_state.is_contiguous()
+                                       and row_state.shape == memory.shape[:2]))
+            and all(p.dtype == memory.dtype and p.is_cuda and p.is_contiguous() and p.data_ptr() % 16 == 0 for p in ps))
+
+
+def encoder_score(memory, row_state, enc_output, enc_norm, cls_head, index=None, want_score=True, want_rows=False):
+    _gpu(memory, "encoder_score")
+    if index is not None:
+        index = index if (index.dtype == torch.int64 and index.is_contiguous()) else index.to(torch.int64).contiguous()
+    with torch.cuda.device(memory.device):
+        return _cabi.encoder_score(memory, row_state, index, enc_output.weight, enc_output.bias, enc_norm.weight,
+                                   enc_norm.bias, enc_norm.eps, cls_head.weight, cls_head.bias, want_score, want_rows)
+
+
 def preprocess_image(src_u8, resized_hw, pad_hw, mean, std, pad_value=(0, 0, 0), dtype=torch.float16):
     _gpu(src_u8, "preprocess_image")
     if src_u8.dtype != torch.uint8 or src_u8.dim() != 3 or src_u8.shape[2] != 3:
@@ -875,7 +902,7 @@
 
 _SWITCH_DEFAULTS = {"ENC_POSGEN": True, "WINDOW_BIAS_LANE": True, "LINEAR_PP": True, "SWIN_MLP": True, "SWIN_MLP_MIN_ROWS": 32768, "LN_GEMM": True, "XADD": True, "XADD_MIN_ROWS": 0, "MERGE_LN": True, "MSDA_ENCODER": True,
                     "MSDA_FP32_REF": True, "FP8_MIN_TILES": 96,
-                    "R50_NATIVE": True, "R50_CONV_IM2COL": False}
+                    "R50_NATIVE": True, "R50_CONV_IM2COL": False, "ENC_SCORE": True}
 
 
 def nondefault_switches():
diff --git a/co-detr-tensorrt_amd/codetr/transformer.py b/co-detr-tensorrt_amd/codetr/transformer.py
--- a/co-detr-tensorrt_amd/codetr/transformer.py
+++ b/co-detr-tensorrt_amd/codetr/transformer.py
@@ -482,22 +482,29 @@
         memory = self.encoder.forward_bf(feat, pos, mask, reference_points=ref_by_level, spatial_shapes=spatial_shapes,
                                          level_start_index=level_start_index)
         B = memory.shape[0]
-        if native_geom:
-            out_mem = hip_ops.linear(memory, self.enc_output.weight, self.enc_output.bias, row_mask=row_state)
-        else:
-            proposals = make_encoder_output_proposals_export(reference_points, mlvl_masks)
-            proposals, out_mem = apply_mask_to_proposal_and_memory(proposals, memory, mask)
-            out_mem = hip_ops.linear(out_mem, self.enc_output.weight, self.enc_output.bias)
-        out_mem = hip_ops.layer_norm(out_mem, self.enc_output_norm.weight, self.enc_output_norm.bias,
-                                     self.enc_output_norm.eps)
         last = self.decoder.num_layers
         cls_head = cls_branches[last]
-        enc_cls = hip_ops.linear(out_mem, cls_head.weight, cls_head.bias)
-        if forced_topk_indices is None:
-            topk = hip_ops.topk(hip_ops.row_max(enc_cls), self.two_stage_num_proposals, want_values=False)[1]
-        else:
-            topk = forced_topk_indices
-        sel = hip_ops.gather_rows(out_mem, topk)
+        if (native_geom and capture is None and forced_topk_indices is None
+                and hip_ops.encoder_score_supported(memory, row_state, self.enc_output, self.enc_output_norm, cls_head)):
+            score = hip_ops.encoder_score(memory, row_state, self.enc_output, self.enc_output_norm, cls_head)[0]
+            topk = hip_ops.topk(score, self.two_stage_num_proposals, want_values=False)[1]
+            sel = hip_ops.encoder_score(memory, row_state, self.enc_output, self.enc_output_norm, cls_head, index=topk,
+                                        want_score=False, want_rows=True)[1]
+        else:
+            if native_geom:
+                out_mem = hip_ops.linear(memory, self.enc_output.weight, self.enc_output.bias, row_mask=row_state)
+            else:
+                proposals = make_encoder_output_proposals_export(reference_points, mlvl_masks)
+                proposals, out_mem = apply_mask_to_proposal_and_memory(proposals, memory, mask)
+                out_mem = hip_ops.linear(out_mem, self.enc_output.weight, self.enc_output.bias)
+            out_mem = hip_ops.layer_norm(out_mem, self.enc_output_norm.weight, self.enc_output_norm.bias,
+                                         self.enc_output_norm.eps)
+            enc_cls = hip_ops.linear(out_mem, cls_head.weight, cls_head.bias)
+            if forced_topk_indices is None:
+                topk = hip_ops.topk(hip_ops.row_max(enc_cls), self.two_stage_num_proposals, want_values=False)[1]
+            else:
+                topk = forced_topk_indices
+            sel = hip_ops.gather_rows(out_mem, topk)
         topk_coords = run_mlp(reg_branches[last], sel, residual=hip_ops.gather_rows(proposals, topk))
         qw = self.query_embed.weight
         if B == 1 or not qw.is_cuda or torch.is_grad_enabled():
diff --git a/co-detr-tensorrt_amd/csrc/encoder_score.hip b/co-detr-tensorrt_amd/csrc/encoder_score.hip
--- /dev/null
+++ b/co-detr-tensorrt_amd/csrc/encoder_score.hip
@@ -0,0 +1,264 @@
+#include <hip/hip_runtime.h>
+#include <stdint.h>
+
+#include "codetr_hip.h"
+#include "device_prims.h"
+
+namespace {
+
+constexpr int kC = 256;
+constexpr int kRowsPerWave = 32;
+constexpr int kRowsPerBlock = 128;
+constexpr int kTileBytes = kRowsPerWave * kC * 2;
+constexpr int kChunkCols = 16;
+constexpr int kChunkBytes = kChunkCols * kC * 2;
+constexpr int kMaxClasses = 128;
+
+__device__ __forceinline__ float group_sum32(float v) {
+#pragma unroll
+  for (int o = 16; o > 0; o >>= 1) v += __shfl_xor(v, o, 64);
+  return v;
+}
+
+__device__ __forceinline__ void stage_chunk(const unsigned short* __restrict__ W, int rows, int n0, unsigned char* buf,
+                                            int tid) {
+  const int wave = tid >> 6;
+#pragma unroll
+  for (int q = 0; q < 2; ++q) {
+    const int u = q * 256 + tid;
+    const int r = u >> 5, pos = u & 31;
+    int n = n0 + r;
+    n = n < rows ? n : rows - 1;
+    lds_dma16_auto(W + (size_t)n * kC + ((pos ^ r) << 3), buf + (q * 256 + wave * 64) * 16);
+  }
+}
+
+template <class T>
+__global__ __launch_bounds__(256, 2) void encoder_score_kernel(
+    const unsigned short* __restrict__ X, const unsigned char* __restrict__ row_state, const int64_t* __restrict__ index,
+    const unsigned short* __restrict__ Wenc, const unsigned short* __restrict__ benc,
+    const unsigned short* __restrict__ gamma, const unsigned short* __restrict__ beta, float eps,
+    const unsigned short* __restrict__ Wcls, const unsigned short* __restrict__ bcls, int num_classes,
+    unsigned short* __restrict__ score, unsigned short* __restrict__ norm_out, int64_t M, int64_t S, int64_t Nq) {
+  __shared__ __attribute__((aligned(16))) unsigned char lds[4 * kTileBytes + 2 * kChunkBytes];
+  const int tid = threadIdx.x, lane = tid & 63, wave = tid >> 6;
+  const int frow = lane & 15, g = lane >> 4;
+  unsigned char* tile = lds + wave * kTileBytes;
+  unsigned char* ring = lds + 4 * kTileBytes;
+  const int64_t m0 = (int64_t)blockIdx.x * kRowsPerBlock + wave * kRowsPerWave;
+  const int cls_chunks = score ? (num_classes + kChunkCols - 1) / kChunkCols : 0;
+  const int chunks = kC / kChunkCols + cls_chunks;
+  auto issue = [&](int c) {
+    unsigned char* buf = ring + (c & 1) * kChunkBytes;
+    if (c < kC / kChunkCols) stage_chunk(Wenc, kC, c * kChunkCols, buf, tid);
+    else stage_chunk(Wcls, num_classes, (c - kC / kChunkCols) * kChunkCols, buf, tid);
+  };
+  issue(0);
+
+  typename T::frag xb[8][2];
+  unsigned char st[2];
+#pragma unroll
+  for (int j = 0; j < 2; ++j) {
+    int64_t m = m0 + j * 16 + frow;
+    m = m < M ? m : M - 1;
+    int64_t src = m;
+    if (index) {
+      int64_t i = index[m];
+      i = i < 0 ? 0 : (i < S ? i : S - 1);
+      src = (m / Nq) * S + i;
+    }
+    st[j] = row_state ? row_state[src] : (unsigned char)0;
+    const unsigned short* xr = X + src * kC + g * 8;
+#pragma unroll
+    for (int ks = 0; ks < 8; ++ks) {
+      s16x8 v = {0, 0, 0, 0, 0, 0, 0, 0};
+      if (st[j] != 2) v = *reinterpret_cast<const s16x8*>(xr + ks * 32);
+      xb[ks][j] = __builtin_bit_cast(typename T::frag, v);
+    }
+  }
+
+  s16x4 bcur = *reinterpret_cast<const s16x4*>(benc + 4 * g);
+#pragma unroll 1
+  for (int c = 0; c < kC / kChunkCols; ++c) {
+    wait_vmcnt<0>();
+    __builtin_amdgcn_s_barrier();
+    if (c + 1 < chunks) issue(c + 1);
+    const int cn = c + 1 < kC / kChunkCols ? c + 1 : c;
+    const s16x4 bnext = *reinterpret_cast<const s16x4*>(benc + cn * kChunkCols + 4 * g);
+    const unsigned char* buf = ring + (c & 1) * kChunkBytes;
+    f32x4 acc[2];
+#pragma unroll
+    for (int r = 0; r < 4; ++r) acc[0][r] = T::to_f32((unsigned short)bcur[r]);
+    acc[1] = acc[0];
+#pragma unroll
+    for (int ks = 0; ks < 8; ++ks) {
+      const typename T::frag a =
+          *reinterpret_cast<const typename T::frag*>(buf + frow * (kC * 2) + (((ks * 4 + g) ^ frow) << 4));
+      acc[0] = T::mfma(a, xb[ks][0], acc[0]);
+      acc[1] = T::mfma(a, xb[ks][1], acc[1]);
+    }
+#pragma unroll
+    for (int j = 0; j < 2; ++j) {
+      const float v[4] = {acc[j][0], acc[j][1], acc[j][2], acc[j][3]};
+      s16x4 o = T::pack4(v);
+      if (st[j] == 1) o = s16x4{0, 0, 0, 0};
+      const int row = j * 16 + frow;
+      *reinterpret_cast<s16x4*>(tile + row * (kC * 2) + (((c * 2 + (g >> 1)) ^ row) << 4) + (g & 1) * 8) = o;
+    }
+    bcur = bnext;
+  }
+  __builtin_amdgcn_wave_barrier();
+
+  {
+    const int sub = lane & 31, half = lane >> 5;
+    const s16x8 gw = *reinterpret_cast<const s16x8*>(gamma + sub * 8);
+    const s16x8 gb = *reinterpret_cast<const s16x8*>(beta + sub * 8);
+    const float inv_c = 1.0f / (float)kC;
+#pragma unroll 1
+    for (int p0 = 0; p0 < 16; p0 += 8) {
+      s16x8 v[8];
+      float mean[8], rstd[8];
+#pragma unroll
+      for (int p = 0; p < 8; ++p) {
+        const int row = (p0 + p) * 2 + half;
+        v[p] = *reinterpret_cast<const s16x8*>(tile + row * (kC * 2) + ((sub ^ row) << 4));
+        float s = 0.f;
+#pragma unroll
+        for (int e = 0; e < 8; ++e) s += T::to_f32((unsigned short)v[p][e]);
+        mean[p] = s;
+      }
+#pragma unroll
+      for (int p = 0; p < 8; ++p) mean[p] = group_sum32(mean[p]) * inv_c;
+#pragma unroll
+      for (int p = 0; p < 8; ++p) {
+        float q = 0.f;
+#pragma unroll
+        for (int e = 0; e < 8; ++e) {
+          const float d = T::to_f32((unsigned short)v[p][e]) - mean[p];
+          q = fmaf(d, d, q);
+        }
+        rstd[p] = q;
+      }
+#pragma unroll
+      for (int p = 0; p < 8; ++p) rstd[p] = rsqrtf(group_sum32(rstd[p]) * inv_c + eps);
+#pragma unroll
+      for (int p = 0; p < 8; ++p) {
+        const int row = (p0 + p) * 2 + half;
+        s16x8 o;
+#pragma unroll
+        for (int e = 0; e < 8; ++e)
+          o[e] = (short)T::from_f32(fmaf((T::to_f32((unsigned short)v[p][e]) - mean[p]) * rstd[p],
+                                         T::to_f32((unsigned short)gw[e]), T::to_f32((unsigned short)gb[e])));
+        *reinterpret_cast<s16x8*>(tile + row * (kC * 2) + ((sub ^ row) << 4)) = o;
+        if (norm_out && m0 + row < M) *reinterpret_cast<s16x8*>(norm_out + (m0 + row) * kC + sub * 8) = o;
+      }
+    }
+  }
+  if (!score) return;
+  __builtin_amdgcn_wave_barrier();
+
+  typename T::frag hb[8][2];
+#pragma unroll
+  for (int j = 0; j < 2; ++j)
+#pragma unroll
+    for (int ks = 0; ks < 8; ++ks) {
+      const int row = j * 16 + frow;
+      hb[ks][j] = *reinterpret_cast<const typename T::frag*>(tile + row * (kC * 2) + (((ks * 4 + g) ^ row) << 4));
+    }
+  float best[2] = {-__builtin_inff(), -__builtin_inff()};
+  bool nan[2] = {false, false};
+#pragma unroll 1
+  for (int c = kC / kChunkCols; c < chunks; ++c) {
+    wait_vmcnt<0>();
+    __builtin_amdgcn_s_barrier();
+    if (c + 1 < chunks) issue(c + 1);
+    const unsigned char* buf = ring + (c & 1) * kChunkBytes;
+    const int n = (c - kC / kChunkCols) * kChunkCols + 4 * g;
+    f32x4 acc[2];
+#pragma unroll
+    for (int r = 0; r < 4; ++r) acc[0][r] = n + r < num_classes ? T::to_f32(bcls[n + r]) : 0.f;
+    acc[1] = acc[0];
+#pragma unroll
+    for (int ks = 0; ks < 8; ++ks) {
+      const typename T::frag a =
+          *reinterpret_cast<const typename T::frag*>(buf + frow * (kC * 2) + (((ks * 4 + g) ^ frow) << 4));
+      acc[0] = T::mfma(a, hb[ks][0], acc[0]);
+      acc[1] = T::mfma(a, hb[ks][1], acc[1]);
+    }
+#pragma unroll
+    for (int j = 0; j < 2; ++j) {
+      const float v[4] = {acc[j][0], acc[j][1], acc[j][2], acc[j][3]};
+      const s16x4 o = T::pack4(v);
+#pragma unroll
+      for (int r = 0; r < 4; ++r) {
+        const float f = T::to_f32((unsigned short)o[r]);
+        if (n + r < num_classes) {
+          nan[j] = nan[j] || f != f;
+          best[j] = f > best[j] ? f : best[j];
+        }
+      }
+    }
+  }
+#pragma unroll
+  for (int j = 0; j < 2; ++j) {
+#pragma unroll
+    for (int o = 16; o <= 32; o <<= 1) {
+      const float b2 = __shfl_xor(best[j], o, 64);
+      const int n2 = __shfl_xor((int)nan[j], o, 64);
+      best[j] = b2 > best[j] ? b2 : best[j];
+      nan[j] = nan[j] || n2;
+    }
+    const int64_t m = m0 + j * 16 + frow;
+    if (g == 0 && m < M) score[m] = T::from_f32(nan[j] ? __builtin_nanf("") : best[j]);
+  }
+}
+
+template <class T>
+int launch(void* stream, const void* memory, const void* row_state, const void* index, const void* w_enc, const void* b_enc,
+           const void* ln_gamma, const void* ln_beta, float ln_eps, const void* w_cls, const void* b_cls, void* score,
+           void* norm, int64_t B, int64_t S, int64_t Nq, int64_t C, int64_t num_classes) {
+  if (!memory || !w_enc || !b_enc || !ln_gamma || !ln_beta || B <= 0 || S <= 0 || C <= 0) return CODETR_E_BADARG;
+  if (index ? (Nq <= 0 || !norm) : !score) return CODETR_E_BADARG;
+  if (score && (!w_cls || !b_cls || num_classes <= 0)) return CODETR_E_BADARG;
+  if (C != kC || (score && num_classes > kMaxClasses)) return CODETR_E_UNSUPPORTED;
+  const uintptr_t align = reinterpret_cast<uintptr_t>(memory) | reinterpret_cast<uintptr_t>(w_enc) |
+                          reinterpret_cast<uintptr_t>(b_enc) | reinterpret_cast<uintptr_t>(ln_gamma) |
+                          reinterpret_cast<uintptr_t>(ln_beta) | reinterpret_cast<uintptr_t>(w_cls) |
+                          reinterpret_cast<uintptr_t>(norm) | reinterpret_cast<uintptr_t>(index);
+  if (align & 15) return CODETR_E_BADARG;
+  const int64_t M = B * (index ? Nq : S);
+  if (B * S > 0x7fffffffLL * 16 || (M + kRowsPerBlock - 1) / kRowsPerBlock > 0x7fffffffLL) return CODETR_E_TOO_LARGE;
+  hipLaunchKernelGGL(encoder_score_kernel<T>, dim3((unsigned)((M + kRowsPerBlock - 1) / kRowsPerBlock)), dim3(256), 0,
+                     static_cast<hipStream_t>(stream), static_cast<const unsigned short*>(memory),
+                     static_cast<const unsigned char*>(row_state), static_cast<const int64_t*>(index),
+                     static_cast<const unsigned short*>(w_enc), static_cast<const unsigned short*>(b_enc),
+                     static_cast<const unsigned short*>(ln_gamma), static_cast<const unsigned short*>(ln_beta), ln_eps,
+                     static_cast<const unsigned short*>(w_cls), static_cast<const unsigned short*>(b_cls),
+                     (int)num_classes, static_cast<unsigned short*>(score), static_cast<unsigned short*>(norm), M, S, Nq);
+  const hipError_t err = hipGetLastError();
+  return err == hipSuccess ? 0 : (int)err;
+}
+
+}
+
+extern "C" {
+
+int codetr_encoder_score_f16(void* stream, const void* memory_dev, const void* row_state_dev, const void* index_dev,
+                             const void* w_enc_dev, const void* b_enc_dev, const void* ln_gamma_dev,
+                             const void* ln_beta_dev, float ln_eps, const void* w_cls_dev, const void* b_cls_dev,
+                             void* score_dev, void* norm_dev, int64_t B, int64_t S, int64_t Nq, int64_t C,
+                             int64_t num_classes) {
+  return launch<HalfT>(stream, memory_dev, row_state_dev, index_dev, w_enc_dev, b_enc_dev, ln_gamma_dev, ln_beta_dev, ln_eps,
+                       w_cls_dev, b_cls_dev, score_dev, norm_dev, B, S, Nq, C, num_classes);
+}
+
+int codetr_encoder_score_bf16(void* stream, const void* memory_dev, const void* row_state_dev, const void* index_dev,
+                              const void* w_enc_dev, const void* b_enc_dev, const void* ln_gamma_dev,
+                              const void* ln_beta_dev, float ln_eps, const void* w_cls_dev, const void* b_cls_dev,
+                              void* score_dev, void* norm_dev, int64_t B, int64_t S, int64_t Nq, int64_t C,
+                              int64_t num_classes) {
+  return launch<BFloatT>(stream, memory_dev, row_state_dev, index_dev, w_enc_dev, b_enc_dev, ln_gamma_dev, ln_beta_dev,
+                         ln_eps, w_cls_dev, b_cls_dev, score_dev, norm_dev, B, S, Nq, C, num_classes);
+}
+
+}
diff --git a/include/codetr_hip.h b/include/codetr_hip.h
--- a/include/codetr_hip.h
+++ b/include/codetr_hip.h
@@ -246,6 +246,17 @@
 
 int codetr_row_max_f16(void *stream, const void *x_dev, void *out_dev, int64_t rows, int64_t C);
 int codetr_row_max_bf16(void *stream, const void *x_dev, void *out_dev, int64_t rows, int64_t C);
+
+int codetr_encoder_score_f16(void *stream, const void *memory_dev, const void *row_state_dev, const void *index_dev,
+                             const void *w_enc_dev, const void *b_enc_dev, const void *ln_gamma_dev,
+                             const void *ln_beta_dev, float ln_eps, const void *w_cls_dev, const void *b_cls_dev,
+                             void *score_dev, void *norm_dev, int64_t B, int64_t S, int64_t Nq, int64_t C,
+                             int64_t num_classes);
+int codetr_encoder_score_bf16(void *stream, const void *memory_dev, const void *row_state_dev, const void *index_dev,
+                              const void *w_enc_dev, const void *b_enc_dev, const void *ln_gamma_dev,
+                              const void *ln_beta_dev, float ln_eps, const void *w_cls_dev, const void *b_cls_dev,
+                              void *score_dev, void *norm_dev, int64_t B, int64_t S, int64_t Nq, int64_t C,
+                              int64_t num_classes);
 
 int codetr_preprocess_u8_f16(void *stream, const void *src_dev, int64_t H_src, int64_t W_src, int64_t H_resized,
                              int64_t W_resized, int64_t H_pad, int64_t W_pad, const float *mean_host,
diff --git a/runner/dispatch_gen.inc b/runner/dispatch_gen.inc
--- a/runner/dispatch_gen.inc
+++ b/runner/dispatch_gen.inc
@@ -57,6 +57,8 @@
 static int call_codetr_encoder_geometry_bf16(void* fn, const Arg* a) { typedef int (*F)(const void*, const void*, const void*, long long, int, const void*, const void*, const void*, const void*, const void*); return ((F)fn)((const void*)a[0].p, (const void*)a[1].p, (const void*)a[2].p, (long long)a[3].i, (int)a[4].i, (const void*)a[5].p, (const void*)a[6].p, (const void*)a[7].p, (const void*)a[8].p, (const void*)a[9].p); }
 static int call_codetr_row_max_f16(void* fn, const Arg* a) { typedef int (*F)(const void*, const void*, const void*, long long, long long); return ((F)fn)((const void*)a[0].p, (const void*)a[1].p, (const void*)a[2].p, (long long)a[3].i, (long long)a[4].i); }
 static int call_codetr_row_max_bf16(void* fn, const Arg* a) { typedef int (*F)(const void*, const void*, const void*, long long, long long); return ((F)fn)((const void*)a[0].p, (const void*)a[1].p, (const void*)a[2].p, (long long)a[3].i, (long long)a[4].i); }
+static int call_codetr_encoder_score_f16(void* fn, const Arg* a) { typedef int (*F)(const void*, const void*, const void*, const void*, const void*, const void*, const void*, const void*, float, const void*, const void*, const void*, const void*, long long, long long, long long, long long, long long); return ((F)fn)((const void*)a[0].p, (const void*)a[1].p, (const void*)a[2].p, (const void*)a[3].p, (const void*)a[4].p, (const void*)a[5].p, (const void*)a[6].p, (const void*)a[7].p, (float)a[8].f, (const void*)a[9].p, (const void*)a[10].p, (const void*)a[11].p, (const void*)a[12].p, (long long)a[13].i, (long long)a[14].i, (long long)a[15].i, (long long)a[16].i, (long long)a[17].i); }
+static int call_codetr_encoder_score_bf16(void* fn, const Arg* a) { typedef int (*F)(const void*, const void*, const void*, const void*, const void*, const void*, const void*, const void*, float, const void*, const void*, const void*, const void*, long long, long long, long long, long long, long long); return ((F)fn)((const void*)a[0].p, (const void*)a[1].p, (const void*)a[2].p, (const void*)a[3].p, (const void*)a[4].p, (const void*)a[5].p, (const void*)a[6].p, (const void*)a[7].p, (float)a[8].f, (const void*)a[9].p, (const void*)a[10].p, (const void*)a[11].p, (const void*)a[12].p, (long long)a[13].i, (long long)a[14].i, (long long)a[15].i, (long long)a[16].i, (long long)a[17].i); }
 static int call_codetr_preprocess_u8_f16(void* fn, const Arg* a) { typedef int (*F)(const void*, const void*, long long, long long, long long, long long, long long, long long, const void*, const void*, const void*, const void*, const void*); return ((F)fn)((const void*)a[0].p, (const void*)a[1].p, (long long)a[2].i, (long long)a[3].i, (long long)a[4].i, (long long)a[5].i, (long long)a[6].i, (long long)a[7].i, (const void*)a[8].p, (const void*)a[9].p, (const void*)a[10].p, (const void*)a[11].p, (const void*)a[12].p); }
 static int call_codetr_preprocess_u8_f32(void* fn, const Arg* a) { typedef int (*F)(const void*, const void*, long long, long long, long long, long long, long long, long long, const void*, const void*, const void*, const void*, const void*); return ((F)fn)((const void*)a[0].p, (const void*)a[1].p, (long long)a[2].i, (long long)a[3].i, (long long)a[4].i, (long long)a[5].i, (long long)a[6].i, (long long)a[7].i, (const void*)a[8].p, (const void*)a[9].p, (const void*)a[10].p, (const void*)a[11].p, (const void*)a[12].p); }
 static int call_codetr_batched_nms_f32(void* fn, const Arg* a) { typedef int (*F)(const void*, const void*, const void*, long long, float, const void*); return ((F)fn)((const void*)a[0].p, (const void*)a[1].p, (const void*)a[2].p, (long long)a[3].i, (float)a[4].f, (const void*)a[5].p); }
@@ -167,6 +169,8 @@
   {"codetr_encoder_geometry_bf16", 10, call_codetr_encoder_geometry_bf16},
   {"codetr_row_max_f16", 5, call_codetr_row_max_f16},
   {"codetr_row_max_bf16", 5, call_codetr_row_max_bf16},
+  {"codetr_encoder_score_f16", 18, call_codetr_encoder_score_f16},
+  {"codetr_encoder_score_bf16", 18, call_codetr_encoder_score_bf16},
   {"codetr_preprocess_u8_f16", 13, call_codetr_preprocess_u8_f16},
   {"codetr_preprocess_u8_f32", 13, call_codetr_preprocess_u8_f32},
   {"codetr_batched_nms_f32", 6, call_codetr_batched_nms_f32},
```
